# thepochynsons/MCRay-Tracing

Hardware: AMD Instinct MI355X
Metric: rays/sec (Monte-Carlo sample paths traced + accumulated into whole B-mode frames: PSF, envelope, scan conversion) (higher is better)
Workload: dtype f32; 1 GPU; 1M random triangles (8 meshes, PCG64 12345): 128x1024 rays/GPU, depth 10, 465 rows; scan_lines_total=128, triangles=1000000, parallelism=scanline-shard x1, frames_in_flight=128, last_pass_gather_and_post_exposed=False, gather=none (one GPU), slowest_repeat=0, overlap_gather_psf_with_next_trace=True, bvh_builder=sah, warmup_steps_run=5304

## Files before the change

### include/mcrt.h

```cpp
#ifndef MCRT_H
#define MCRT_H
#include <stdint.h>
#include <stddef.h>

#ifdef __cplusplus
extern "C" {
#endif

#define MCRT_VERSION 109

typedef enum {
    MCRT_OK = 0,
    MCRT_ERR_INVALID = -1,
    MCRT_ERR_HIP = -2,
    MCRT_ERR_NOMEM = -3,
    MCRT_ERR_NO_DEVICE = -4,
    MCRT_ERR_LIMIT = -5
} mcrt_status;

typedef struct mcrt_ctx mcrt_ctx;

typedef struct {
    uint32_t n_elements;
    uint32_t n_samples;
// ... 158 lines not shown
                                    uint8_t *out_dev , const mcrt_compound_opts *o );
int mcrt_compound_weights(uint32_t n_elements, uint32_t n_rows, double radius_mm, double total_angle_rad, uint32_t max_travel_us,
                          uint32_t speed_of_sound, uint32_t out_rows, uint32_t out_cols, float steer_rad, float view_weight, float feather_lines,
                          float *w );

typedef struct { uint32_t n_planes;
                 float    step_rad;
                 float    pivot_mm;
} mcrt_sweep;
typedef struct { double origin_mm[3], du_mm[3], dv_mm[3], dw_mm[3];
                 uint32_t nu, nv, nw, _pad;
} mcrt_volume_grid;
int mcrt_transducer_swept(uint32_t n_elements, double radius_cm, double separation_mm, const float position[3], const float angles_deg[3],
                          float tilt_rad, float pivot_mm, float *pos, float *dir);
int mcrt_volume_maps(uint32_t n_elements, uint32_t n_rows, double radius_mm, double total_angle_rad, uint32_t max_travel_us, uint32_t speed_of_sound,
                     const mcrt_sweep *sweep, const mcrt_volume_grid *grid, float *map_plane, float *map_row, float *map_col);
int mcrt_volume_frames(mcrt_ctx *ctx, const float *rf_dev , uint32_t n_frames, uint32_t n_elements, uint32_t n_rows,
                       double radius_mm, double total_angle_rad, const mcrt_sweep *sweep, const mcrt_volume_grid *grid,
                       float *out_dev );
int mcrt_bmode_volume_frames(mcrt_ctx *ctx, const float *rf_dev , uint32_t n_frames, uint32_t n_elements, uint32_t n_rows,
                             const mcrt_bmode_params *p, const mcrt_sweep *sweep, const mcrt_volume_grid *grid,
                             const float *tgc_db , float *peak_dev ,
                             uint8_t *out_dev );

enum { MCRT_RENDER_MIP = 0, MCRT_RENDER_MEAN = 1, MCRT_RENDER_SURFACE = 2 };
typedef struct { float origin[3], di[3], dj[3], ds[3];
                 uint32_t nx, ny, n_steps, _pad;
} mcrt_render_view;
typedef struct { uint32_t mode;
                 float lo, hi;
                 float threshold;
                 float ramp;
                 float opacity;
                 float depth_cue;
                 float t_cut;
} mcrt_render_opts;
int mcrt_default_render_opts(mcrt_render_opts *o, int in_u8);
int mcrt_render_view_for_grid(const mcrt_volume_grid *g, const double dir_mm[3], const double up_mm[3], double pixel_mm, double step_mm,
                              uint32_t nx, uint32_t ny, mcrt_render_view *out);
int mcrt_render_frames(mcrt_ctx *ctx, const void *vol_dev, int in_u8, uint32_t n_frames, uint32_t nu, uint32_t nv, uint32_t nw,
                       const mcrt_render_view *view, const mcrt_render_opts *o ,
                       float *out_dev , uint8_t *out8_dev , float *depth_dev );

typedef struct { uint32_t n_iter;
                 float q0;
                 float rho;
                 float lambda;
} mcrt_speckle_opts;
int mcrt_default_speckle_opts(mcrt_speckle_opts *o);
int mcrt_speckle_tables(const mcrt_speckle_opts *o, float *q0sq , float *kq , float *lam4 );
int mcrt_speckle_frames(mcrt_ctx *ctx, const float *in_dev, uint32_t n_frames, uint32_t height, uint32_t width,
                        const mcrt_speckle_opts *o , float *out_dev);

enum { MCRT_RECON_MEAN = 0, MCRT_RECON_MAX = 1 };
typedef struct { uint32_t mode;
                 float    value_max;
                 uint32_t fill_radius;
                 uint32_t fill_min;
                 float    empty;
} mcrt_recon_opts;
int mcrt_default_recon_opts(mcrt_recon_opts *o);
int mcrt_recon_transform(const mcrt_volume_grid *grid_world_mm, double unit_mm, float A[9], float b[3]);
int mcrt_recon_frames(mcrt_ctx *ctx, const float *stack_dev , uint32_t n_frames, uint32_t n_elements, uint32_t n_rows,
                      const float *pos , const float *dir , double row_mm, double unit_mm,
                      const mcrt_volume_grid *grid , const mcrt_recon_opts *o ,
                      float *out_dev , uint32_t *count_dev , uint32_t *stats_dev );

enum { MCRT_LABEL_TRACED = 0, MCRT_LABEL_GEOMETRIC = 1 };
#define MCRT_LABEL_NONE 255u
#define MCRT_LABEL_MAX_CROSSINGS 64u
typedef struct { uint32_t rule;
                 float    start_offset;
} mcrt_label_opts;
int mcrt_default_label_opts(mcrt_label_opts *o);
int mcrt_label_frames(mcrt_ctx *ctx, uint32_t n_frames, uint32_t e_begin, uint32_t e_end,
                      const float *pos , const float *dir ,
                      const mcrt_label_opts *o ,
                      uint8_t *tissue_dev , int32_t *interface_dev ,
                      uint32_t *crossings_dev );
int mcrt_label_scan_convert_frames(mcrt_ctx *ctx, const uint8_t *tissue_dev , uint32_t n_frames, uint32_t n_elements, uint32_t n_rows,
                                   double radius_mm, double total_angle_rad, uint8_t *out_dev , uint32_t out_rows, uint32_t out_cols);
int mcrt_label_volume_frames(mcrt_ctx *ctx, const uint8_t *tissue_dev , uint32_t n_frames, uint32_t n_elements, uint32_t n_rows,
                             double radius_mm, double total_angle_rad, const mcrt_sweep *sweep, const mcrt_volume_grid *grid,
                             uint8_t *out_dev );

typedef struct { uint32_t n_labels;
                 uint32_t fill_radius;
                 uint32_t fill_min;
} mcrt_recon_label_opts;
int mcrt_default_recon_label_opts(mcrt_recon_label_opts *o, uint32_t n_labels);
int mcrt_recon_label_frames(mcrt_ctx *ctx, const uint8_t *stack_dev , uint32_t n_frames, uint32_t n_elements, uint32_t n_rows,
                            const float *pos , const float *dir , double row_mm, double unit_mm,
                            const mcrt_volume_grid *grid , const mcrt_recon_label_opts *o,
                            uint8_t *out_dev , uint32_t *count_dev , uint32_t *votes_dev ,
                            uint32_t *stats_dev );
int mcrt_render_label_frames(mcrt_ctx *ctx, const uint8_t *label_dev , uint32_t n_frames, uint32_t nu, uint32_t nv, uint32_t nw,
                             const mcrt_render_view *view, const float *depth_dev , uint8_t *out_dev );

int mcrt_export_rf(mcrt_ctx *ctx, const float *rf_dev, uint32_t n_elements, uint32_t n_rows, float *host_rows_by_cols);

int mcrt_import_rf(mcrt_ctx *ctx, const float *host_rows_by_cols, uint32_t n_elements, uint32_t n_rows, float *rf_dev);

typedef struct mcrt_group mcrt_group;
int mcrt_group_create(const int *devices, uint32_t n_devices, mcrt_group **out);
int mcrt_group_destroy(mcrt_group *grp);
int mcrt_group_size(const mcrt_group *grp);
mcrt_ctx *mcrt_group_root(mcrt_group *grp);
mcrt_ctx *mcrt_group_member(mcrt_group *grp, uint32_t rank);
int mcrt_group_shard(uint32_t rank, uint32_t n_ranks, uint32_t n_elements, uint32_t *e_begin, uint32_t *e_end);
int mcrt_group_set_params(mcrt_group *grp, const mcrt_params *p);
int mcrt_group_set_bvh_builder(mcrt_group *grp, int builder);
int mcrt_group_upload_scene(mcrt_group *grp, const float *tri_xyz_host, const uint32_t *tri_mesh, uint32_t n_tri, const mcrt_mesh *meshes, uint32_t n_mesh,
                            const float *materials, uint32_t n_mat, uint32_t start_mat, const float spacing[3]);
int mcrt_group_update_triangles(mcrt_group *grp, const float *tri_xyz_host, uint32_t n_tri);
int mcrt_group_last_scene_seconds(mcrt_group *grp, double *build_s, double *upload_s);
int mcrt_group_refit_triangles(mcrt_group *grp, const float *tri_xyz_host, uint32_t n_tri);
int mcrt_group_upload_texture(mcrt_group *grp, const float *voxels, uint32_t n);
int mcrt_group_set_transducer(mcrt_group *grp, const float *pos, const float *dir, uint32_t n_elements);
int mcrt_group_trace_frames(mcrt_group *grp, uint32_t frame_id, uint32_t n_frames, float *rf_dev);
int mcrt_group_trace_frames_poses(mcrt_group *grp, uint32_t frame_id, uint32_t n_frames, const float *pos, const float *dir, float *rf_dev);
int mcrt_group_synchronize(mcrt_group *grp);
int mcrt_group_last_pass_ms(mcrt_group *grp, float *trace_ms, float *copy_ms);

int mcrt_alloc(mcrt_ctx *ctx, size_t bytes, void **dev);
int mcrt_free(mcrt_ctx *ctx, void *dev);
int mcrt_memcpy_d2h(mcrt_ctx *ctx, void *host, const void *dev, size_t bytes);
int mcrt_memcpy_h2d(mcrt_ctx *ctx, void *dev, const void *host, size_t bytes);

int mcrt_enable_stats(mcrt_ctx *ctx, int enable);
int mcrt_get_stats(mcrt_ctx *ctx, mcrt_stats *out, int reset);
int mcrt_enable_timing(mcrt_ctx *ctx, int enable);
int mcrt_get_kernel_time(mcrt_ctx *ctx, double *avg_ms, uint32_t *n, int reset);
int mcrt_get_kernel_times(mcrt_ctx *ctx, double avg_ms[3], uint32_t n[3], int reset);

int mcrt_build_bvh(const float *tri_xyz, const uint32_t *tri_mesh, uint32_t n_tri, mcrt_bvh *out);
void mcrt_free_bvh(mcrt_bvh *bvh);
int mcrt_get_bvh(mcrt_ctx *ctx, mcrt_bvh *out );
int mcrt_build_bvh4(const mcrt_bvh *bvh2, mcrt_bvh4 *out);
void mcrt_free_bvh4(mcrt_bvh4 *bvh4);
int mcrt_get_bvh4(mcrt_ctx *ctx, mcrt_bvh4 *out );
int mcrt_row_thresholds(double row_dt_us, uint32_t n_rows, double *thr);
int mcrt_generate_texture(float *voxels, uint32_t n);
int mcrt_psf_kernels(float freq, float var_x, float var_y, uint32_t res_um, float *axial, uint32_t n_ax, float *lateral, uint32_t n_lat);
int mcrt_transducer_elements(uint32_t n_elements, double radius_cm, double separation_mm,
                             const float position[3], const float angles_deg[3], float *pos, float *dir);

int mcrt_debug_math(mcrt_ctx *ctx, int op, const double *x, const double *y, double *out, uint32_t n);
int mcrt_debug_philox(mcrt_ctx *ctx, const uint32_t ctr[4], const uint32_t key[2], uint32_t out[4]);
int mcrt_debug_stamps(mcrt_ctx *ctx, uint64_t out[200], int reset);
int mcrt_debug_tail_histograms(mcrt_ctx *ctx, uint64_t out[2560], int reset);
int mcrt_debug_fast_paths(mcrt_ctx *ctx, uint32_t out[4]);
int mcrt_debug_beam(mcrt_ctx *ctx, uint32_t out[6]);
int mcrt_debug_beam_bounce(mcrt_ctx *ctx, uint32_t b, uint32_t out[8]);
int mcrt_debug_set_error(mcrt_ctx *ctx, uint32_t bits);

#ifdef __cplusplus
}
#endif
#endif
```

### mcray-tracing_amd/__init__.py

```python
from ._lib import load_library, build_library, McrtError, Params, MeshRec, BvhNode, Stats, BmodeParams, Focus, Compound, Sweep, VolumeGrid, CompoundOpts, LabelOpts, RenderView, RenderOpts, SpeckleOpts, ReconOpts, ReconLabelOpts, SEGMENT_DTYPE
from .api import Context, Group, shard_range, Simulator, bmode_params, Transducer, Psf, host_build_bvh, host_build_bvh4, host_row_thresholds, host_texture, host_psf, host_psf_focus, focus_struct, row_pitch_mm, host_transducer, host_scan_maps, host_elevation_axis, host_elevation_planes, host_psf_elevation, host_transducer_steered, host_compound_maps, host_transducer_swept, host_volume_maps, sweep_struct, sweep_tilts, volume_grid, cplane_grid, sagittal_grid, compound_struct, compound_opts_struct, host_compound_weights, label_opts_struct, render_view, render_opts_struct, RENDER_MODES, speckle_opts_struct, host_speckle_tables, recon_opts_struct, recon_label_opts_struct, host_recon_transform, RECON_MODES, LABEL_RULES, LABEL_NONE, LABEL_MAX_CROSSINGS, LABEL_CAPPED
from . import synth, scene_io


def __getattr__(name):
    if name == "dist":
        import importlib
        return importlib.import_module("mcray_tracing_amd.dist")
    raise AttributeError(name)

__all__ = ["load_library", "build_library", "McrtError", "Params", "BmodeParams", "bmode_params", "Context", "Group", "shard_range", "Simulator", "Transducer", "Psf",
           "synth", "scene_io", "host_build_bvh", "host_texture", "host_psf", "host_psf_focus", "host_transducer"]
```

### mcray-tracing_amd/_lib.py

```python
import ctypes as C
import os
import subprocess
import numpy as np

_HERE = os.path.dirname(os.path.abspath(__file__))
_SO = os.environ.get("MCRT_LIB") or os.path.join(_HERE, "libmcrt_hip.so")
_LIB = None


class McrtError(RuntimeError):
    def __init__(self, code, msg):
        super().__init__(f"mcrt error {code}: {msg}")
        self.code = code


class Params(C.Structure):
    _fields_ = [("n_elements", C.c_uint32), ("n_samples", C.c_uint32), ("max_depth", C.c_uint32), ("n_rows", C.c_uint32),
                ("frequency", C.c_float), ("intensity_epsilon", C.c_float), ("initial_intensity", C.c_float),
                ("ray_start_offset", C.c_float), ("speed_of_sound", C.c_uint32), ("depth_cm", C.c_double),
                ("seed", C.c_uint32), ("sanitize_tir", C.c_uint32), ("tex_n", C.c_uint32), ("tex_res", C.c_float)]


class MeshRec(C.Structure):
    _fields_ = [("mat_inside", C.c_uint32), ("mat_outside", C.c_uint32), ("vascular", C.c_uint32), ("_pad", C.c_uint32)]


class BvhNode(C.Structure):
    _fields_ = [("lo0", C.c_float * 3), ("c0", C.c_int32), ("hi0", C.c_float * 3), ("c1", C.c_int32),
                ("lo1", C.c_float * 3), ("pad0", C.c_uint32), ("hi1", C.c_float * 3), ("pad1", C.c_uint32)]


class Bvh(C.Structure):
    _fields_ = [("n_nodes", C.c_uint32), ("n_tri", C.c_uint32), ("max_depth", C.c_uint32), ("pad_abs", C.c_float),
                ("nodes", C.c_void_p), ("tri", C.c_void_p)]


class Bvh4(C.Structure):
    _fields_ = [("n_nodes", C.c_uint32), ("max_stack", C.c_uint32), ("nodes", C.c_void_p)]


class Stats(C.Structure):
    _fields_ = [(n, C.c_uint64) for n in ("queries", "nodes_visited", "tris_tested", "segments", "rf_steps", "hits")]

    def as_dict(self):
        return {n: int(getattr(self, n)) for n, _ in self._fields_}


class BmodeParams(C.Structure):
    _fields_ = [("mode", C.c_uint32), ("dynamic_range_db", C.c_float), ("gain_db", C.c_float), ("ref", C.c_float), ("persistence", C.c_float),
                ("reset_state", C.c_uint32), ("out_rows", C.c_uint32), ("out_cols", C.c_uint32), ("radius_mm", C.c_double), ("total_angle_rad", C.c_double)]


class Focus(C.Structure):
    _fields_ = [("n_focus", C.c_uint32), ("focus_mm", C.c_float * 8), ("focal_range_mm", C.c_float)]


class Compound(C.Structure):
    _fields_ = [("n_views", C.c_uint32), ("steer_rad", C.c_float * 16)]


class CompoundOpts(C.Structure):
    _fields_ = [("mode", C.c_uint32), ("feather_lines", C.c_float), ("view_weight", C.c_float * 16)]


class Sweep(C.Structure):
    _fields_ = [("n_planes", C.c_uint32), ("step_rad", C.c_float), ("pivot_mm", C.c_float)]


class VolumeGrid(C.Structure):
    _fields_ = [("origin_mm", C.c_double * 3), ("du_mm", C.c_double * 3), ("dv_mm", C.c_double * 3), ("dw_mm", C.c_double * 3),
                ("nu", C.c_uint32), ("nv", C.c_uint32), ("nw", C.c_uint32), ("_pad", C.c_uint32)]


class LabelOpts(C.Structure):
    _fields_ = [("rule", C.c_uint32), ("start_offset", C.c_float)]


class RenderView(C.Structure):
    _fields_ = [("origin", C.c_float * 3), ("di", C.c_float * 3), ("dj", C.c_float * 3), ("ds", C.c_float * 3),
                ("nx", C.c_uint32), ("ny", C.c_uint32), ("n_steps", C.c_uint32), ("_pad", C.c_uint32)]


class RenderOpts(C.Structure):
    _fields_ = [("mode", C.c_uint32), ("lo", C.c_float), ("hi", C.c_float), ("threshold", C.c_float), ("ramp", C.c_float), ("opacity", C.c_float),
                ("depth_cue", C.c_float), ("t_cut", C.c_float)]


class SpeckleOpts(C.Structure):
    _fields_ = [("n_iter", C.c_uint32), ("q0", C.c_float), ("rho", C.c_float), ("lambda_", C.c_float)]


class ReconOpts(C.Structure):
    _fields_ = [("mode", C.c_uint32), ("value_max", C.c_float), ("fill_radius", C.c_uint32), ("fill_min", C.c_uint32), ("empty", C.c_float)]


class ReconLabelOpts(C.Structure):
    _fields_ = [("n_labels", C.c_uint32), ("fill_radius", C.c_uint32), ("fill_min", C.c_uint32)]


NODE_DTYPE = np.dtype([("lo0", "<f4", 3), ("c0", "<i4"), ("hi0", "<f4", 3), ("c1", "<i4"),
                       ("lo1", "<f4", 3), ("pad0", "<u4"), ("hi1", "<f4", 3), ("pad1", "<u4")])
SEGMENT_DTYPE = np.dtype([("from", "<f4", 3), ("to", "<f4", 3), ("dir", "<f4", 3),
                          ("reflected_intensity", "<f4"), ("initial_intensity", "<f4"), ("attenuation", "<f4"),
                          ("distance_traveled", "<f8"), ("media", "<i4"), ("tri", "<i4")])
assert NODE_DTYPE.itemsize == 64 and SEGMENT_DTYPE.itemsize == 64 and C.sizeof(BvhNode) == 64 and C.sizeof(BmodeParams) == 48 and C.sizeof(Focus) == 40 and C.sizeof(Compound) == 68 and C.sizeof(CompoundOpts) == 72
assert C.sizeof(Sweep) == 12 and C.sizeof(VolumeGrid) == 112 and C.sizeof(LabelOpts) == 8 and C.sizeof(RenderView) == 64 and C.sizeof(RenderOpts) == 32 and C.sizeof(SpeckleOpts) == 16 and C.sizeof(ReconOpts) == 20
assert C.sizeof(ReconLabelOpts) == 12

SYMBOLS = ["mcrt_last_error", "mcrt_version", "mcrt_device_count", "mcrt_create", "mcrt_destroy", "mcrt_set_stream",
           "mcrt_synchronize", "mcrt_default_params", "mcrt_set_params", "mcrt_get_params", "mcrt_import_rf", "mcrt_set_bvh_builder", "mcrt_upload_scene", "mcrt_update_triangles", "mcrt_refit_triangles", "mcrt_upload_texture",
           "mcrt_set_transducer", "mcrt_trace_frame", "mcrt_trace_frames", "mcrt_trace_frames_poses", "mcrt_envelope_frames", "mcrt_scan_convert_frames", "mcrt_trace_frame_debug", "mcrt_cast_rays", "mcrt_convolve", "mcrt_convolve_frames", "mcrt_convolve_frames_depth",
           "mcrt_envelope", "mcrt_scan_convert", "mcrt_default_bmode", "mcrt_bmode_frames", "mcrt_export_rf", "mcrt_alloc", "mcrt_free", "mcrt_memcpy_d2h",
           "mcrt_memcpy_h2d", "mcrt_enable_stats", "mcrt_get_stats", "mcrt_enable_timing", "mcrt_get_kernel_time", "mcrt_get_kernel_times",
           "mcrt_build_bvh", "mcrt_free_bvh", "mcrt_get_bvh", "mcrt_build_bvh4", "mcrt_free_bvh4", "mcrt_get_bvh4", "mcrt_row_thresholds", "mcrt_generate_texture", "mcrt_psf_kernels", "mcrt_psf_focus_kernels",
           "mcrt_transducer_elements", "mcrt_transducer_elevation_axis", "mcrt_elevation_planes", "mcrt_psf_elevation_kernels", "mcrt_elevation_frames", "mcrt_debug_math", "mcrt_debug_philox", "mcrt_debug_stamps", "mcrt_debug_tail_histograms", "mcrt_debug_set_error", "mcrt_debug_fast_paths", "mcrt_debug_beam", "mcrt_debug_beam_bounce", "mcrt_scan_maps",
           "mcrt_group_create", "mcrt_group_destroy", "mcrt_group_size", "mcrt_group_root", "mcrt_group_member", "mcrt_group_shard", "mcrt_group_set_params",
           "mcrt_group_set_bvh_builder", "mcrt_group_upload_scene", "mcrt_group_update_triangles", "mcrt_group_refit_triangles", "mcrt_group_upload_texture",
           "mcrt_group_set_transducer", "mcrt_group_trace_frames", "mcrt_group_trace_frames_poses", "mcrt_group_synchronize", "mcrt_group_last_pass_ms", "mcrt_group_last_scene_seconds",
           "mcrt_transducer_steered", "mcrt_compound_maps", "mcrt_compound_frames", "mcrt_bmode_compound_frames",
           "mcrt_default_compound_opts", "mcrt_compound_weights", "mcrt_compound_frames_opts", "mcrt_bmode_compound_frames_opts",
           "mcrt_transducer_swept", "mcrt_volume_maps", "mcrt_volume_frames", "mcrt_bmode_volume_frames",
           "mcrt_default_label_opts", "mcrt_label_frames", "mcrt_label_scan_convert_frames", "mcrt_label_volume_frames",
           "mcrt_default_render_opts", "mcrt_render_view_for_grid", "mcrt_render_frames",
           "mcrt_default_speckle_opts", "mcrt_speckle_tables", "mcrt_speckle_frames",
           "mcrt_default_recon_opts", "mcrt_recon_transform", "mcrt_recon_frames",
           "mcrt_default_recon_label_opts", "mcrt_recon_label_frames", "mcrt_render_label_frames"]


def build_library(force=False):
    srcs = [os.path.join(_HERE, "csrc", f) for f in os.listdir(os.path.join(_HERE, "csrc"))]
    srcs.append(os.path.join(_HERE, "..", "include", "mcrt.h"))
    stale = (not os.path.exists(_SO)) or any(os.path.getmtime(s) > os.path.getmtime(_SO) for s in srcs)
    if force or stale:
        subprocess.check_call(["make", "-C", _HERE, "libmcrt_hip.so"] + (["-B"] if force else []))
    return _SO


def load_library():
    global _LIB
    if _LIB is not None:
        return _LIB
    if not os.path.exists(_SO):
        raise McrtError(-4, f"{_SO} is missing: run __graft_entry__.build() (make -C mcray-tracing_amd); there is no CPU fallback")
    L = C.CDLL(_SO)
    L.mcrt_last_error.restype = C.c_char_p
    vp, u32, i32 = C.c_void_p, C.c_uint32, C.c_int
    sig = {
        "mcrt_create": [i32, C.POINTER(vp)], "mcrt_destroy": [vp], "mcrt_set_stream": [vp, vp], "mcrt_synchronize": [vp],
        "mcrt_default_params": [C.POINTER(Params)], "mcrt_set_params": [vp, C.POINTER(Params)], "mcrt_get_params": [vp, C.POINTER(Params)], "mcrt_import_rf": [vp, vp, u32, u32, vp],
        "mcrt_upload_scene": [vp, vp, vp, u32, vp, u32, vp, u32, u32, vp],
        "mcrt_upload_texture": [vp, vp, u32], "mcrt_set_transducer": [vp, vp, vp, u32],
        "mcrt_trace_frame": [vp, u32, u32, u32, vp], "mcrt_trace_frames": [vp, u32, u32, u32, u32, vp], "mcrt_trace_frame_debug": [vp, u32, u32, u32, vp, vp, vp, vp],
        "mcrt_cast_rays": [vp, u32, u32, u32, vp, vp, vp],
        "mcrt_convolve": [vp, vp, u32, u32, vp, u32, vp, u32], "mcrt_envelope": [vp, vp, u32, u32],
        "mcrt_scan_convert": [vp, vp, u32, u32, C.c_double, C.c_double, vp, u32, u32],
        "mcrt_convolve_frames": [vp, vp, u32, u32, u32, vp, u32, vp, u32], "mcrt_convolve_frames_depth": [vp, vp, u32, u32, u32, vp, u32, vp, u32],
        "mcrt_trace_frames_poses": [vp, u32, u32, u32, u32, vp, vp, vp], "mcrt_envelope_frames": [vp, vp, u32, u32, u32],
        "mcrt_scan_convert_frames": [vp, vp, u32, u32, u32, C.c_double, C.c_double, vp, u32, u32],
        "mcrt_default_bmode": [C.POINTER(BmodeParams)], "mcrt_bmode_frames": [vp, vp, u32, u32, u32, C.POINTER(BmodeParams), vp, vp, vp, vp],
        "mcrt_set_bvh_builder": [vp, i32], "mcrt_update_triangles": [vp, vp, u32], "mcrt_refit_triangles": [vp, vp, u32],
        "mcrt_export_rf": [vp, vp, u32, u32, vp], "mcrt_alloc": [vp, C.c_size_t, C.POINTER(vp)], "mcrt_free": [vp, vp],
        "mcrt_memcpy_d2h": [vp, vp, vp, C.c_size_t], "mcrt_memcpy_h2d": [vp, vp, vp, C.c_size_t],
        "mcrt_enable_stats": [vp, i32], "mcrt_get_stats": [vp, C.POINTER(Stats), i32],
        "mcrt_enable_timing": [vp, i32], "mcrt_get_kernel_time": [vp, C.POINTER(C.c_double), C.POINTER(u32), i32], "mcrt_get_kernel_times": [vp, vp, vp, i32],
        "mcrt_build_bvh": [vp, vp, u32, C.POINTER(Bvh)], "mcrt_free_bvh": [C.POINTER(Bvh)], "mcrt_get_bvh": [vp, C.POINTER(Bvh)],
        "mcrt_build_bvh4": [C.POINTER(Bvh), C.POINTER(Bvh4)], "mcrt_free_bvh4": [C.POINTER(Bvh4)], "mcrt_get_bvh4": [vp, C.POINTER(Bvh4)],
        "mcrt_row_thresholds": [C.c_double, u32, vp],
        "mcrt_generate_texture": [vp, u32], "mcrt_psf_kernels": [C.c_float, C.c_float, C.c_float, u32, vp, u32, vp, u32],
        "mcrt_psf_focus_kernels": [C.c_float, u32, C.POINTER(Focus), u32, C.c_double, vp, u32],
        "mcrt_transducer_elements": [u32, C.c_double, C.c_double, vp, vp, vp, vp],
        "mcrt_transducer_elevation_axis": [vp, vp], "mcrt_elevation_planes": [vp, vp, u32, vp, u32, u32, vp, vp, vp],
        "mcrt_psf_elevation_kernels": [C.c_float, u32, C.POINTER(Focus), u32, C.c_double, i32, vp, u32],
        "mcrt_elevation_frames": [vp, vp, u32, u32, u32, u32, vp, vp],
        "mcrt_transducer_steered": [u32, C.c_double, C.c_double, vp, vp, C.c_float, vp, vp],
        "mcrt_compound_maps": [u32, u32, C.c_double, C.c_double, u32, u32, u32, u32, C.c_float, vp, vp],
        "mcrt_compound_frames": [vp, vp, u32, u32, u32, C.c_double, C.c_double, C.POINTER(Compound), vp, u32, u32],
        "mcrt_bmode_compound_frames": [vp, vp, u32, u32, u32, C.POINTER(BmodeParams), C.POINTER(Compound), vp, vp, vp, vp],
        "mcrt_default_compound_opts": [C.POINTER(CompoundOpts)],
        "mcrt_compound_weights": [u32, u32, C.c_double, C.c_double, u32, u32, u32, u32, C.c_float, C.c_float, C.c_float, vp],
        "mcrt_compound_frames_opts": [vp, vp, u32, u32, u32, C.c_double, C.c_double, C.POINTER(Compound), vp, u32, u32, C.POINTER(CompoundOpts)],
        "mcrt_bmode_compound_frames_opts": [vp, vp, u32, u32, u32, C.POINTER(BmodeParams), C.POINTER(Compound), vp, vp, vp, vp, C.POINTER(CompoundOpts)],
        "mcrt_transducer_swept": [u32, C.c_double, C.c_double, vp, vp, C.c_float, C.c_float, vp, vp],
        "mcrt_volume_maps": [u32, u32, C.c_double, C.c_double, u32, u32, C.POINTER(Sweep), C.POINTER(VolumeGrid), vp, vp, vp],
        "mcrt_volume_frames": [vp, vp, u32, u32, u32, C.c_double, C.c_double, C.POINTER(Sweep), C.POINTER(VolumeGrid), vp],
        "mcrt_bmode_volume_frames": [vp, vp, u32, u32, u32, C.POINTER(BmodeParams), C.POINTER(Sweep), C.POINTER(VolumeGrid), vp, vp, vp],
        "mcrt_default_label_opts": [C.POINTER(LabelOpts)],
        "mcrt_label_frames": [vp, u32, u32, u32, vp, vp, C.POINTER(LabelOpts), vp, vp, vp],
        "mcrt_label_scan_convert_frames": [vp, vp, u32, u32, u32, C.c_double, C.c_double, vp, u32, u32],
        "mcrt_label_volume_frames": [vp, vp, u32, u32, u32, C.c_double, C.c_double, C.POINTER(Sweep), C.POINTER(VolumeGrid), vp],
        "mcrt_default_render_opts": [C.POINTER(RenderOpts), i32],
        "mcrt_render_view_for_grid": [C.POINTER(VolumeGrid), vp, vp, C.c_double, C.c_double, u32, u32, C.POINTER(RenderView)],
        "mcrt_render_frames": [vp, vp, i32, u32, u32, u32, u32, C.POINTER(RenderView), C.POINTER(RenderOpts), vp, vp, vp],
        "mcrt_default_speckle_opts": [C.POINTER(SpeckleOpts)],
        "mcrt_speckle_tables": [C.POINTER(SpeckleOpts), vp, vp, vp],
        "mcrt_speckle_frames": [vp, vp, u32, u32, u32, C.POINTER(SpeckleOpts), vp],
        "mcrt_default_recon_opts": [C.POINTER(ReconOpts)],
        "mcrt_recon_transform": [C.POINTER(VolumeGrid), C.c_double, vp, vp],
        "mcrt_recon_frames": [vp, vp, u32, u32, u32, vp, vp, C.c_double, C.c_double, C.POINTER(VolumeGrid), C.POINTER(ReconOpts), vp, vp, vp],
        "mcrt_default_recon_label_opts": [C.POINTER(ReconLabelOpts), u32],
        "mcrt_recon_label_frames": [vp, vp, u32, u32, u32, vp, vp, C.c_double, C.c_double, C.POINTER(VolumeGrid), C.POINTER(ReconLabelOpts), vp, vp, vp, vp],
        "mcrt_render_label_frames": [vp, vp, u32, u32, u32, u32, C.POINTER(RenderView), vp, vp],
        "mcrt_debug_math": [vp, i32, vp, vp, vp, u32], "mcrt_debug_philox": [vp, vp, vp, vp], "mcrt_debug_stamps": [vp, vp, i32], "mcrt_debug_tail_histograms": [vp, vp, i32], "mcrt_debug_set_error": [vp, u32], "mcrt_debug_fast_paths": [vp, vp], "mcrt_debug_beam": [vp, vp], "mcrt_debug_beam_bounce": [vp, u32, vp],
        "mcrt_scan_maps": [u32, u32, C.c_double, C.c_double, u32, u32, u32, u32, vp, vp],
        "mcrt_group_create": [vp, u32, C.POINTER(vp)], "mcrt_group_destroy": [vp], "mcrt_group_size": [vp], "mcrt_group_root": [vp], "mcrt_group_member": [vp, u32],
        "mcrt_group_shard": [u32, u32, u32, C.POINTER(u32), C.POINTER(u32)], "mcrt_group_set_params": [vp, C.POINTER(Params)], "mcrt_group_set_bvh_builder": [vp, i32],
        "mcrt_group_upload_scene": [vp, vp, vp, u32, vp, u32, vp, u32, u32, vp], "mcrt_group_update_triangles": [vp, vp, u32], "mcrt_group_refit_triangles": [vp, vp, u32],
        "mcrt_group_upload_texture": [vp, vp, u32], "mcrt_group_set_transducer": [vp, vp, vp, u32], "mcrt_group_trace_frames": [vp, u32, u32, vp],
        "mcrt_group_trace_frames_poses": [vp, u32, u32, vp, vp, vp], "mcrt_group_synchronize": [vp], "mcrt_group_last_pass_ms": [vp, vp, vp],
        "mcrt_group_last_scene_seconds": [vp, C.POINTER(C.c_double), C.POINTER(C.c_double)],
    }
    for name, args in sig.items():
        if name in ("mcrt_debug_beam", "mcrt_debug_beam_bounce") and not hasattr(L, name):
            continue
        f = getattr(L, name)
        f.argtypes = args
        f.restype = None if name in ("mcrt_free_bvh", "mcrt_free_bvh4") else vp if name in ("mcrt_group_root", "mcrt_group_member") else C.c_int
    _LIB = L
    return L


def check(rc):
    if rc != 0:
        raise McrtError(rc, load_library().mcrt_last_error().decode())


def ptr(a):
    if a is None:
        return None
    if isinstance(a, int):
        return C.c_void_p(a)
    if isinstance(a, np.ndarray):
        return a.ctypes.data_as(C.c_void_p)
    if hasattr(a, "data_ptr"):
        return C.c_void_p(a.data_ptr())
    raise TypeError(type(a))
```

### mcray-tracing_amd/api.py

```python
import contextlib
import ctypes as C
import math
import numpy as np

from . import _lib
from ._lib import Params, MeshRec, Stats, Bvh, Bvh4, BmodeParams, Focus, Compound, Sweep, VolumeGrid, CompoundOpts, LabelOpts, RenderView, RenderOpts, SpeckleOpts, ReconOpts, ReconLabelOpts, NODE_DTYPE, SEGMENT_DTYPE, check, ptr, load_library

DEFAULT_ANGLE = 1.0471975511965976


def host_build_bvh(tri, tri_mesh):
    L = load_library()
    tri = np.ascontiguousarray(tri, np.float32).reshape(-1, 9)
    tm = np.ascontiguousarray(tri_mesh, np.uint32)
    b = Bvh()
    check(L.mcrt_build_bvh(ptr(tri), ptr(tm), tri.shape[0], C.byref(b)))
    try:
        nodes = np.frombuffer(C.string_at(b.nodes, 64 * b.n_nodes), dtype=NODE_DTYPE).copy()
        btri = np.frombuffer(C.string_at(b.tri, 48 * b.n_tri), dtype=np.float32).reshape(-1, 12).copy()
        depth = int(b.max_depth)
    finally:
        L.mcrt_free_bvh(C.byref(b))
    return nodes, btri, depth


def host_build_bvh4(tri, tri_mesh):
    L = load_library()
    tri = np.ascontiguousarray(tri, np.float32).reshape(-1, 9)
    tm = np.ascontiguousarray(tri_mesh, np.uint32)
    b = Bvh(); b4 = Bvh4()
    check(L.mcrt_build_bvh(ptr(tri), ptr(tm), tri.shape[0], C.byref(b)))
    try:
        check(L.mcrt_build_bvh4(C.byref(b), C.byref(b4)))
        nodes = np.frombuffer(C.string_at(b.nodes, 64 * b.n_nodes), dtype=NODE_DTYPE).copy()
        btri = np.frombuffer(C.string_at(b.tri, 48 * b.n_tri), dtype=np.float32).reshape(-1, 12).copy()
        n4 = np.frombuffer(C.string_at(b4.nodes, 128 * b4.n_nodes), dtype=np.uint8).reshape(-1, 128).copy()
        ms = int(b4.max_stack)
    finally:
        L.mcrt_free_bvh(C.byref(b)); L.mcrt_free_bvh4(C.byref(b4))
    return nodes, btri, n4, ms


def host_row_thresholds(row_dt_us, n_rows):
    thr = np.zeros(n_rows + 1, np.float64)
    check(load_library().mcrt_row_thresholds(row_dt_us, n_rows, ptr(thr)))
    return thr


def host_texture(n=256):
    out = np.empty((n, n, n, 2), np.float32)
    check(load_library().mcrt_generate_texture(ptr(out), n))
    return out


def host_psf(freq=4.5, var_x=0.05, var_y=0.2, res_um=145, n_ax=7, n_lat=13):
    ax = np.zeros(n_ax, np.float32); lat = np.zeros(n_lat, np.float32)
    check(load_library().mcrt_psf_kernels(freq, var_x, var_y, res_um, ptr(ax), n_ax, ptr(lat), n_lat))
    return ax, lat


def focus_struct(focus_mm=(), focal_range_mm=20.0):
    f = Focus()
    fm = [float(x) for x in (focus_mm or ())]
    f.n_focus = len(fm)
    for i, x in enumerate(fm[:8]):
        f.focus_mm[i] = x
    f.focal_range_mm = focal_range_mm
    return f


def host_psf_focus(var_y, res_um, n_rows, row_mm, focus_mm, focal_range_mm=20.0, n_lat=13):
    out = np.zeros((n_rows, n_lat), np.float32)
    f = focus_struct(focus_mm, focal_range_mm)
    check(load_library().mcrt_psf_focus_kernels(var_y, res_um, C.byref(f), n_rows, row_mm, ptr(out), n_lat))
    return out


def row_pitch_mm(frequency):
    res_f = np.float32(np.float32(1.45) / np.float32(frequency))
    return int(np.float32(res_f * np.float32(1000.0))) / 1000.0


def _element_tables(fn, n_elements, radius_cm, sep_mm, position, angles_deg, *how):
    pos = np.zeros((n_elements, 3), np.float32); d = np.zeros((n_elements, 3), np.float32)
    p = np.asarray(position, np.float32); a = np.asarray(angles_deg, np.float32)
    check(getattr(load_library(), fn)(n_elements, radius_cm, sep_mm, ptr(p), ptr(a), *how, ptr(pos), ptr(d)))
    return pos, d


def host_transducer(n_elements, radius_cm, sep_mm, position, angles_deg):
    return _element_tables("mcrt_transducer_elements", n_elements, radius_cm, sep_mm, position, angles_deg)


def host_elevation_axis(angles_deg):
    a = np.asarray(angles_deg, np.float32); out = np.zeros(3, np.float32)
    check(load_library().mcrt_transducer_elevation_axis(ptr(a), ptr(out)))
    return out


def host_elevation_planes(pos, dirs, axis, n_planes, pitch_um):
    pos = np.ascontiguousarray(pos, np.float32).reshape(-1, 3); dirs = np.ascontiguousarray(dirs, np.float32).reshape(-1, 3)
    axis = np.ascontiguousarray(axis, np.float32)
    E, K = pos.shape[0], max(int(n_planes), 0)
    po = np.zeros((K, E, 3), np.float32); do = np.zeros((K, E, 3), np.float32); z = np.zeros(K, np.float32)
    check(load_library().mcrt_elevation_planes(ptr(pos), ptr(dirs), E, ptr(axis), n_planes, pitch_um, ptr(po), ptr(do), ptr(z)))
    return po, do, z


def host_psf_elevation(var_z, pitch_um, n_rows, row_mm, focus_mm=(), focal_range_mm=20.0, n_planes=7, normalize=True):
    out = np.zeros((n_rows, max(int(n_planes), 0)), np.float32)
    f = focus_struct(focus_mm, focal_range_mm)
    check(load_library().mcrt_psf_elevation_kernels(var_z, pitch_um, C.byref(f), n_rows, row_mm, 1 if normalize else 0, ptr(out), n_planes))
    return out


def host_scan_maps(n_elements, n_rows, radius_mm=30.0, total_angle=DEFAULT_ANGLE, max_travel_us=100, speed_of_sound=1500, out_rows=400, out_cols=500):
    return _sector_maps("mcrt_scan_maps", n_elements, n_rows, radius_mm, total_angle, max_travel_us, speed_of_sound, out_rows, out_cols)


def _sector_maps(fn, n_elements, n_rows, radius_mm, total_angle, max_travel_us, speed_of_sound, out_rows, out_cols, *steer):
    mr = np.zeros((out_rows, out_cols), np.float32); mc = np.zeros((out_rows, out_cols), np.float32)
    check(getattr(load_library(), fn)(n_elements, n_rows, radius_mm, total_angle, max_travel_us, speed_of_sound, out_rows, out_cols, *steer, ptr(mr), ptr(mc)))
    return mr, mc


def host_transducer_steered(n_elements, radius_cm, sep_mm, position, angles_deg, steer_rad):
    return _element_tables("mcrt_transducer_steered", n_elements, radius_cm, sep_mm, position, angles_deg, steer_rad)


def host_compound_maps(n_elements, n_rows, steer_rad, radius_mm=30.0, total_angle=DEFAULT_ANGLE, max_travel_us=100, speed_of_sound=1500, out_rows=400,
                       out_cols=500):
    return _sector_maps("mcrt_compound_maps", n_elements, n_rows, radius_mm, total_angle, max_travel_us, speed_of_sound, out_rows, out_cols, steer_rad)


def compound_struct(steer_rad):
    st = [float(x) for x in steer_rad]
    cp = Compound()
    cp.n_views = len(st)
    for i, x in enumerate(st[:16]):
        cp.steer_rad[i] = x
    return cp


COMPOUND_MODES = {"mean": 0, "max": 1, "median": 2}


def compound_opts_struct(mode="mean", view_weights=None, feather_lines=0.0):
    o = CompoundOpts()
    check(load_library().mcrt_default_compound_opts(C.byref(o)))
    o.mode = COMPOUND_MODES[mode] if isinstance(mode, str) else int(mode)
    o.feather_lines = float(feather_lines)
    if view_weights is not None:
        w = [float(x) for x in view_weights]
        if len(w) > 16:
            raise ValueError("at most 16 view weights, got %d" % len(w))
        for i, x in enumerate(w):
            o.view_weight[i] = x
    return o


def _compound_defaults(mode, view_weights, feather_lines):
    return mode in ("mean", 0) and view_weights is None and feather_lines == 0.0


def host_compound_weights(n_elements, n_rows, steer_rad, view_weight=1.0, feather_lines=0.0, radius_mm=30.0, total_angle=DEFAULT_ANGLE,
                          max_travel_us=100, speed_of_sound=1500, out_rows=400, out_cols=500):
    w = np.zeros((out_rows, out_cols), np.float32)
    check(load_library().mcrt_compound_weights(n_elements, n_rows, radius_mm, total_angle, max_travel_us, speed_of_sound, out_rows, out_cols, steer_rad,
                                               view_weight, feather_lines, ptr(w)))
    return w


def host_transducer_swept(n_elements, radius_cm, sep_mm, position, angles_deg, tilt_rad, pivot_mm=0.0):
    return _element_tables("mcrt_transducer_swept", n_elements, radius_cm, sep_mm, position, angles_deg, tilt_rad, pivot_mm)


def sweep_struct(n_planes, step_rad, pivot_mm=0.0):
    sw = Sweep()
    sw.n_planes, sw.step_rad, sw.pivot_mm = int(n_planes), float(step_rad), float(pivot_mm)
    return sw


def _as_sweep(sweep):
    return sweep if isinstance(sweep, Sweep) else sweep_struct(*sweep)


def sweep_tilts(n_planes, step_rad):
    step = float(np.float32(step_rad))
    return np.array([(k - (n_planes - 1) / 2.0) * step for k in range(n_planes)], np.float32)


def volume_grid(origin_mm, du, dv, dw, nu, nv, nw=1):
    g = VolumeGrid()
    for dst, src in ((g.origin_mm, origin_mm), (g.du_mm, du), (g.dv_mm, dv), (g.dw_mm, dw)):
        for i in range(3):
            dst[i] = float(src[i])
    g.nu, g.nv, g.nw, g._pad = int(nu), int(nv), int(nw), 0
    return g


def cplane_grid(depth_mm, nu, nv, pitch_mm, x0_mm=None, z0_mm=None):
    x0 = -(nu - 1) * pitch_mm / 2.0 if x0_mm is None else x0_mm
    z0 = -(nv - 1) * pitch_mm / 2.0 if z0_mm is None else z0_mm
    return volume_grid((x0, depth_mm, z0), (pitch_mm, 0, 0), (0, 0, pitch_mm), (0, 0, 0), nu, nv, 1)


def sagittal_grid(x_mm, nu, nv, pitch_mm, y0_mm, z0_mm=None):
    z0 = -(nu - 1) * pitch_mm / 2.0 if z0_mm is None else z0_mm
    return volume_grid((x_mm, y0_mm, z0), (0, 0, pitch_mm), (0, pitch_mm, 0), (0, 0, 0), nu, nv, 1)


def host_volume_maps(n_elements, n_rows, sweep, grid, radius_mm=30.0, total_angle=DEFAULT_ANGLE, max_travel_us=100, speed_of_sound=1500):
    sw = _as_sweep(sweep)
    shape = (grid.nw, grid.nv, grid.nu)
    mz = np.zeros(shape, np.float32); mr = np.zeros(shape, np.float32); mc = np.zeros(shape, np.float32)
    check(load_library().mcrt_volume_maps(n_elements, n_rows, radius_mm, total_angle, max_travel_us, speed_of_sound, C.byref(sw), C.byref(grid), ptr(mz), ptr(mr), ptr(mc)))
    return mz, mr, mc


BMODE_MODES = {"db": 0, "ref_log": 1}


RENDER_MODES = {"mip": 0, "mean": 1, "surface": 2}


def render_view(grid, direction, up=(0, 0, 1), pixel_mm=0.25, step_mm=0.25, nx=500, ny=400):
    v = RenderView()
    d = (C.c_double * 3)(*[float(x) for x in direction]); u = (C.c_double * 3)(*[float(x) for x in up])
    check(load_library().mcrt_render_view_for_grid(C.byref(grid), d, u, float(pixel_mm), float(step_mm), int(nx), int(ny), C.byref(v)))
    return v


def render_opts_struct(in_u8=False, mode=None, lo=None, hi=None, threshold=None, ramp=None, opacity=None, depth_cue=None, t_cut=None):
    o = RenderOpts()
    check(load_library().mcrt_default_render_opts(C.byref(o), 1 if in_u8 else 0))
    if mode is not None:
        o.mode = RENDER_MODES[mode] if isinstance(mode, str) else int(mode)
    for name, val in (("lo", lo), ("hi", hi), ("threshold", threshold), ("ramp", ramp), ("opacity", opacity), ("depth_cue", depth_cue), ("t_cut", t_cut)):
        if val is not None:
            setattr(o, name, float(val))
    return o


def speckle_opts_struct(n_iter=None, q0=None, rho=None, lambda_=None, **kw):
    o = SpeckleOpts()
    check(load_library().mcrt_default_speckle_opts(C.byref(o)))
    for k in ("lambda", "lam"):
        if k in kw:
            lambda_ = kw.pop(k)
    if kw:
        raise TypeError("unknown speckle options: %s" % ", ".join(sorted(kw)))
    if n_iter is not None:
        o.n_iter = int(n_iter)
    for name, val in (("q0", q0), ("rho", rho), ("lambda_", lambda_)):
        if val is not None:
            setattr(o, name, float(val))
    return o


def host_speckle_tables(opts=None, **kw):
    o = opts if opts is not None else speckle_opts_struct(**kw)
    n = min(int(o.n_iter), 256)
    q0sq = np.zeros(n, np.float32); kq = np.zeros(n, np.float32); lam4 = np.zeros(1, np.float32)
    check(load_library().mcrt_speckle_tables(C.byref(o), ptr(q0sq), ptr(kq), ptr(lam4)))
    return q0sq, kq, np.float32(lam4[0])


RECON_MODES = {"mean": 0, "max": 1}
# ... 93 lines not shown
        if positions.shape != angles_deg.shape:
            raise ValueError("poses takes one position and one set of angles per frame")
        tabs = [host_transducer(self.n_elements, self.radius_cm, self.separation_mm, p, a) for p, a in zip(positions, angles_deg)]
        return np.stack([t[0] for t in tabs]), np.stack([t[1] for t in tabs])


class Psf:

    def __init__(self, freq=4.5, var_x=0.05, var_y=0.2, var_z=0.1, axial_size=7, lateral_size=13, resolution_um=145, focus_mm=None, focal_range_mm=20.0,
                 elevation_size=7, elevation_pitch_um=None, elevation_focus_mm=None, elevation_normalize=True):
        self.axial_kernel, self.lateral_kernel = host_psf(freq, var_x, var_y, resolution_um, axial_size, lateral_size)
        self.var_y, self.resolution_um = var_y, resolution_um
        self.focus_mm = tuple(float(x) for x in focus_mm) if focus_mm is not None else ()
        self.focal_range_mm = focal_range_mm
        self._rows = {}
        self.var_z, self.elevation_size = var_z, elevation_size
        self.elevation_pitch_um = resolution_um if elevation_pitch_um is None else elevation_pitch_um
        self.elevation_focus_mm = tuple(float(x) for x in elevation_focus_mm) if elevation_focus_mm is not None else ()
        self.elevation_normalize = bool(elevation_normalize)
        self.elevation_kernel = (host_psf_elevation(var_z, self.elevation_pitch_um, 1, 1.0, (), focal_range_mm, elevation_size, False)[0]
                                 if var_z > 0 and math.isfinite(var_z) else np.zeros(elevation_size, np.float32))
        self._elev_rows = {}

    def elevation_rows(self, n_rows, row_mm):
        key = (n_rows, row_mm)
        if key not in self._elev_rows:
            self._elev_rows[key] = host_psf_elevation(self.var_z, self.elevation_pitch_um, n_rows, row_mm, self.elevation_focus_mm, self.focal_range_mm,
                                                      self.elevation_size, self.elevation_normalize)
        return self._elev_rows[key]

    @property
    def has_focus(self):
        return len(self.focus_mm) > 0

    def lateral_rows(self, n_rows, row_mm):
        key = (n_rows, row_mm)
        if key not in self._rows:
            self._rows[key] = host_psf_focus(self.var_y, self.resolution_um, n_rows, row_mm, self.focus_mm, self.focal_range_mm, self.lateral_kernel.size)
        return self._rows[key]


def _scene_tables(sd):
    meshes = (MeshRec * len(sd.meshes))(*[MeshRec(a, b, c, 0) for a, b, c in sd.meshes])
    return meshes, len(sd.meshes), np.asarray(sd.spacing, np.float32)


def _tri9(tri):
    if isinstance(tri, np.ndarray):
        tri = np.ascontiguousarray(tri, np.float32).reshape(-1, 9)
        return tri, tri.shape[0]
    return tri, tri.numel() // 9


def _tgc_rows(tgc_db, n_rows):
    if tgc_db is None:
        return None
    tgc = np.ascontiguousarray(tgc_db, np.float32)
    if tgc.shape != (n_rows,):
        raise ValueError("tgc_db needs one value per RF row: %d, got shape %s" % (n_rows, tgc.shape))
    return tgc


def _pose_tables(what, pos, dirs, n_frames, n_elements):
    if isinstance(pos, np.ndarray):
        pos = np.ascontiguousarray(pos, np.float32); dirs = np.ascontiguousarray(dirs, np.float32)
    if n_frames is None:
        if not hasattr(pos, "shape"):
            raise ValueError("%s: n_frames is required with raw device pointers for pos / dirs" % what)
        n_frames = pos.shape[0]
        assert tuple(pos.shape) == (n_frames, n_elements, 3) and tuple(dirs.shape) == tuple(pos.shape)
    return pos, dirs, n_frames


class _SceneCalls:

    def _call(self, name, *args):
        check(getattr(self.L, self.PREFIX + name)(self.h, *args))

    def _assign_params(self, kw):
        for k, v in kw.items():
            if not hasattr(self.params, k):
                raise AttributeError(k)
            setattr(self.params, k, v)

    def set_bvh_builder(self, builder):
        self._call("set_bvh_builder", {"sah": 0, "lbvh": 1}[builder] if isinstance(builder, str) else int(builder))

    def upload_scene(self, sd):
        meshes, n_mesh, sp = _scene_tables(sd)
        self._call("upload_scene", ptr(sd.tri), ptr(sd.tri_mesh), sd.n_tri, C.cast(meshes, C.c_void_p), n_mesh, ptr(sd.materials), sd.materials.shape[0], sd.start_mat, ptr(sp))

    def upload_texture(self, vox=None, n=256):
        if vox is not None:
            vox = np.ascontiguousarray(vox, np.float32)
        self._call("upload_texture", ptr(vox), n)

    def set_transducer(self, pos, d):
        pos = np.ascontiguousarray(pos, np.float32); d = np.ascontiguousarray(d, np.float32)
        self._call("set_transducer", ptr(pos), ptr(d), pos.shape[0])


class Context(_SceneCalls):
    PREFIX = "mcrt_"

    def __init__(self, device=0, _borrowed=None):
        self.L = load_library()
        self.owned = _borrowed is None
        if self.owned:
            h = C.c_void_p()
            check(self.L.mcrt_create(device, C.byref(h)))
        else:
            h = C.c_void_p(_borrowed)
        self.h = h
        self.params = Params()
        check(self.L.mcrt_default_params(C.byref(self.params)))

    def close(self):
        if getattr(self, "h", None):
            if self.owned:
                self.L.mcrt_destroy(self.h)
            self.h = None

    def __del__(self):
        try:
            self.close()
        except Exception:
            pass

    def set_params(self, **kw):
        self._assign_params(kw)
        check(self.L.mcrt_set_params(self.h, C.byref(self.params)))

    def set_stream(self, stream_ptr):
        check(self.L.mcrt_set_stream(self.h, C.c_void_p(stream_ptr) if stream_ptr else None))

    def synchronize(self):
        check(self.L.mcrt_synchronize(self.h))

    def debug_fast_paths(self):
        out = (C.c_uint32 * 4)()
        check(self.L.mcrt_debug_fast_paths(self.h, out))
        return bool(out[0]), bool(out[1]), int(out[2])

    def debug_beam(self):
        out = (C.c_uint32 * 6)()
        if hasattr(self.L, "mcrt_debug_beam"):
            check(self.L.mcrt_debug_beam(self.h, out))
        return bool(out[0]), int(out[1]), int(out[2]), int(out[3]), int(out[4]), int(out[5])

    def debug_beam_bounce(self, b):
        out = (C.c_uint32 * 8)()
        if hasattr(self.L, "mcrt_debug_beam_bounce"):
            check(self.L.mcrt_debug_beam_bounce(self.h, int(b), out))
        return (bool(out[0]),) + tuple(int(v) for v in out[1:])

    def debug_set_error(self, bits):
        check(self.L.mcrt_debug_set_error(self.h, int(bits)))

    def update_triangles(self, tri):
        tri, n = _tri9(tri)
        check(self.L.mcrt_update_triangles(self.h, ptr(tri), n))

    def refit_triangles(self, tri):
        tri, n = _tri9(tri)
        check(self.L.mcrt_refit_triangles(self.h, ptr(tri), n))

    def get_bvh(self):
        b = Bvh()
        check(self.L.mcrt_get_bvh(self.h, C.byref(b)))
        nodes = np.frombuffer(C.string_at(b.nodes, 64 * b.n_nodes), dtype=NODE_DTYPE).copy() if b.n_nodes else np.zeros(0, NODE_DTYPE)
        btri = np.frombuffer(C.string_at(b.tri, 48 * b.n_tri), dtype=np.float32).reshape(-1, 12).copy()
        return nodes, btri, int(b.max_depth)

    def get_bvh4(self):
        b = Bvh4()
        check(self.L.mcrt_get_bvh4(self.h, C.byref(b)))
        return np.frombuffer(C.string_at(b.nodes, 128 * b.n_nodes), dtype=np.uint8).reshape(-1, 128).copy(), int(b.max_stack)

    def alloc(self, nbytes):
        p = C.c_void_p()
        check(self.L.mcrt_alloc(self.h, nbytes, C.byref(p)))
        return p.value

    def free(self, dev):
        check(self.L.mcrt_free(self.h, C.c_void_p(dev)))

    @contextlib.contextmanager
    def temp(self, nbytes):
        p = self.alloc(nbytes)
        try:
            yield p
        finally:
            self.free(p)

    def d2h(self, dev, shape, dtype=np.float32):
        out = np.empty(shape, dtype)
        check(self.L.mcrt_memcpy_d2h(self.h, ptr(out), ptr(dev), out.nbytes))
        return out

    def h2d(self, dev, arr):
        arr = np.ascontiguousarray(arr)
        check(self.L.mcrt_memcpy_h2d(self.h, ptr(dev), ptr(arr), arr.nbytes))

    def trace_frame(self, frame_id, rf_dev, e_begin=0, e_end=None):
        e_end = self.params.n_elements if e_end is None else e_end
        check(self.L.mcrt_trace_frame(self.h, frame_id, e_begin, e_end, ptr(rf_dev)))

    def trace_frames(self, frame_id, n_frames, rf_dev, e_begin=0, e_end=None):
        e_end = self.params.n_elements if e_end is None else e_end
        check(self.L.mcrt_trace_frames(self.h, frame_id, n_frames, e_begin, e_end, ptr(rf_dev)))

    def trace_frames_poses(self, frame_id, pos, dirs, rf_dev, e_begin=0, e_end=None, n_frames=None):
        e_end = self.params.n_elements if e_end is None else e_end
        pos, dirs, n_frames = _pose_tables("trace_frames_poses", pos, dirs, n_frames, self.params.n_elements)
        check(self.L.mcrt_trace_frames_poses(self.h, frame_id, n_frames, e_begin, e_end, ptr(pos), ptr(dirs), ptr(rf_dev)))

    def trace_frame_debug(self, frame_id, rf_dev, e_begin=0, e_end=None, want_hits=True, want_segs=False):
        e_end = self.params.n_elements if e_end is None else e_end
        ne, S, B = e_end - e_begin, self.params.n_samples, self.params.max_depth
        hits = np.full((ne, S, B), -3, np.int32) if want_hits else None
        segs = np.zeros((ne, S, B), SEGMENT_DTYPE) if want_segs else None
        cnt = np.zeros((ne, S), np.uint32) if want_segs else None
        check(self.L.mcrt_trace_frame_debug(self.h, frame_id, e_begin, e_end, ptr(rf_dev), ptr(hits), ptr(segs), ptr(cnt)))
        return hits, segs, cnt

    def cast_rays(self, frame_id, e_begin=0, e_end=None, want_hits=True):
        e_end = self.params.n_elements if e_end is None else e_end
        ne, S, B = e_end - e_begin, self.params.n_samples, self.params.max_depth
        segs = np.zeros((ne, S, B), SEGMENT_DTYPE); cnt = np.zeros((ne, S), np.uint32)
        hits = np.full((ne, S, B), -3, np.int32) if want_hits else None
        check(self.L.mcrt_cast_rays(self.h, frame_id, e_begin, e_end, ptr(segs), ptr(cnt), ptr(hits)))
        return segs, cnt, hits

    def convolve_frames(self, rf_dev, n_frames, n_elements, n_rows, axial, lateral):
        ax = np.ascontiguousarray(axial, np.float32); lat = np.ascontiguousarray(lateral, np.float32)
        check(self.L.mcrt_convolve_frames(self.h, ptr(rf_dev), n_frames, n_elements, n_rows, ptr(ax), ax.size, ptr(lat), lat.size))

    def convolve_frames_depth(self, rf_dev, n_frames, n_elements, n_rows, axial, lat_rows):
        ax = np.ascontiguousarray(axial, np.float32); lat = np.ascontiguousarray(lat_rows, np.float32)
        if lat.ndim != 2 or lat.shape[0] != n_rows:
            raise ValueError("lat_rows needs one row of taps per RF row: (%d, n_lat), got shape %s" % (n_rows, lat.shape))
        check(self.L.mcrt_convolve_frames_depth(self.h, ptr(rf_dev), n_frames, n_elements, n_rows, ptr(ax), ax.size, ptr(lat), lat.shape[1]))

    def elevation_frames(self, planes_dev, n_frames, n_planes, n_elements, n_rows, w_rows, rf_dev):
        w = np.ascontiguousarray(w_rows, np.float32)
        if w.shape != (n_rows, n_planes):
            raise ValueError("w_rows needs one row of weights per RF row: (%d, %d), got shape %s" % (n_rows, n_planes, w.shape))
        check(self.L.mcrt_elevation_frames(self.h, ptr(planes_dev), n_frames, n_planes, n_elements, n_rows, ptr(w), ptr(rf_dev)))

    def convolve(self, rf_dev, n_elements, n_rows, axial, lateral):
        ax =np.ascontiguousarray(axial, np.float32); lat = np.ascontiguousarray(lateral, np.float32)
        check(self.L.mcrt_convolve(self.h, ptr(rf_dev), n_elements, n_rows, ptr(ax), ax.size, ptr(lat), lat.size))

    def envelope(self, rf_dev, n_elements, n_rows):
        check(self.L.mcrt_envelope(self.h, ptr(rf_dev), n_elements, n_rows))

    def envelope_frames(self, rf_dev, n_frames, n_elements, n_rows):
        check(self.L.mcrt_envelope_frames(self.h, ptr(rf_dev), n_frames, n_elements, n_rows))

    def scan_convert_frames(self, rf_dev, n_frames, n_elements, n_rows, out_dev, radius_mm=30.0, total_angle=DEFAULT_ANGLE, out_rows=400, out_cols=500):
        check(self.L.mcrt_scan_convert_frames(self.h, ptr(rf_dev), n_frames, n_elements, n_rows, radius_mm, total_angle, ptr(out_dev), out_rows, out_cols))

    def scan_convert(self, rf_dev, n_elements, n_rows, out_dev, radius_mm=30.0, total_angle=DEFAULT_ANGLE, out_rows=400, out_cols=500):
        check(self.L.mcrt_scan_convert(self.h, ptr(rf_dev), n_elements, n_rows, radius_mm, total_angle, ptr(out_dev), out_rows, out_cols))

    def bmode_frames(self, rf_dev, n_frames, n_elements, n_rows, out_dev, *, mode="db", dynamic_range_db=60.0, gain_db=0.0, ref=None, tgc_db=None,
                     persistence=0.0, state_dev=None, reset_state=True, peak_dev=None, radius_mm=30.0, total_angle=DEFAULT_ANGLE,
                     out_rows=400, out_cols=500):
        p = bmode_params(mode=mode, dynamic_range_db=dynamic_range_db, gain_db=gain_db, ref=ref, persistence=persistence, reset_state=reset_state,
                         radius_mm=radius_mm, total_angle=total_angle, out_rows=out_rows, out_cols=out_cols)
        tgc = _tgc_rows(tgc_db, n_rows)
        check(self.L.mcrt_bmode_frames(self.h, ptr(rf_dev), n_frames, n_elements, n_rows, C.byref(p), ptr(tgc), ptr(state_dev), ptr(peak_dev), ptr(out_dev)))

    def compound_frames(self, rf_dev, n_frames, n_elements, n_rows, steer_rad, out_dev, radius_mm=30.0, total_angle=DEFAULT_ANGLE, out_rows=400, out_cols=500,
                        mode="mean", view_weights=None, feather_lines=0.0):
        cp = compound_struct(steer_rad)
        if _compound_defaults(mode, view_weights, feather_lines):
            check(self.L.mcrt_compound_frames(self.h, ptr(rf_dev), n_frames, n_elements, n_rows, radius_mm, total_angle, C.byref(cp), ptr(out_dev), out_rows, out_cols))
            return
        o = compound_opts_struct(mode, view_weights, feather_lines)
        check(self.L.mcrt_compound_frames_opts(self.h, ptr(rf_dev), n_frames, n_elements, n_rows, radius_mm, total_angle, C.byref(cp), ptr(out_dev), out_rows, out_cols,
                                               C.byref(o)))

    def bmode_compound_frames(self, rf_dev, n_frames, n_elements, n_rows, steer_rad, out_dev, *, mode="db", dynamic_range_db=60.0, gain_db=0.0, ref=None,
                              tgc_db=None, persistence=0.0, state_dev=None, reset_state=True, peak_dev=None, radius_mm=30.0,
                              total_angle=DEFAULT_ANGLE, out_rows=400, out_cols=500, compound_mode="mean", view_weights=None, feather_lines=0.0):
        p = bmode_params(mode=mode, dynamic_range_db=dynamic_range_db, gain_db=gain_db, ref=ref, persistence=persistence, reset_state=reset_state,
                         radius_mm=radius_mm, total_angle=total_angle, out_rows=out_rows, out_cols=out_cols)
        cp = compound_struct(steer_rad)
        tgc = _tgc_rows(tgc_db, n_rows)
        if _compound_defaults(compound_mode, view_weights, feather_lines):
            check(self.L.mcrt_bmode_compound_frames(self.h, ptr(rf_dev), n_frames, n_elements, n_rows, C.byref(p), C.byref(cp), ptr(tgc), ptr(state_dev),
                                                    ptr(peak_dev), ptr(out_dev)))
            return
        o = compound_opts_struct(compound_mode, view_weights, feather_lines)
        check(self.L.mcrt_bmode_compound_frames_opts(self.h, ptr(rf_dev), n_frames, n_elements, n_rows, C.byref(p), C.byref(cp), ptr(tgc), ptr(state_dev),
                                                     ptr(peak_dev), ptr(out_dev), C.byref(o)))

    def volume_frames(self, rf_dev, n_frames, n_elements, n_rows, sweep, grid, out_dev, radius_mm=30.0, total_angle=DEFAULT_ANGLE):
        sw = _as_sweep(sweep)
        check(self.L.mcrt_volume_frames(self.h, ptr(rf_dev), n_frames, n_elements, n_rows, radius_mm, total_angle, C.byref(sw), C.byref(grid), ptr(out_dev)))

    def bmode_volume_frames(self, rf_dev, n_frames, n_elements, n_rows, sweep, grid, out_dev, *, mode="db", dynamic_range_db=60.0, gain_db=0.0, ref=None,
                            tgc_db=None, persistence=0.0, peak_dev=None, radius_mm=30.0, total_angle=DEFAULT_ANGLE):
        p = bmode_params(mode=mode, dynamic_range_db=dynamic_range_db, gain_db=gain_db, ref=ref, persistence=persistence, radius_mm=radius_mm,
                         total_angle=total_angle, out_rows=0, out_cols=0)
# ... 398 lines not shown
```

### mcray-tracing_amd/csrc/mcrt_api.cpp

```cpp
#include "mcrt_ctx.h"
#include "mcrt_kernels.h"
#include "mcrt_lbvh.h"

#include <hip/hip_runtime.h>
#include <cmath>
#include <cstdlib>
#include <cstring>
#include <vector>
#include <algorithm>
#include <memory>
#include <utility>

using mcrt::set_error;

static Consts derive_consts(const mcrt_params &p)
{
    Consts c;
    c.axial_res_f = 1.45f / p.frequency;
    c.axial_res_mm = (double)c.axial_res_f;
    c.axial_res_um = (uint32_t)(c.axial_res_f * 1000.0f);
    c.time_step_us = (c.axial_res_mm * 1000.0) / (double)p.speed_of_sound;
    c.row_dt_us = (double)c.axial_res_um / (double)p.speed_of_sound;
    c.max_travel_us = (p.depth_cm / (double)p.speed_of_sound) * 10000.0;
    c.max_rows = (uint32_t)((p.speed_of_sound * (uint32_t)c.max_travel_us) / c.axial_res_um);
    return c;
}

static Knobs read_knobs()
{
    using mcrt::tuning_env;
    Knobs k;
    if (const char *e = tuning_env("MCRT_KSPLIT_LIMIT")) { long v = atol(e); if (v >= 0 && v <= MCRT_KSPLIT_MAX) k.ksplit_limit = (uint32_t)v; }
    if (const char *e = tuning_env("MCRT_TRACE_BLOCKS")) { int v = atoi(e); if (v >= 1) k.trace_blocks = (uint32_t)v; }
    if (const char *e = tuning_env("MCRT_TRACE_BLOCKS_WIDE")) { int v = atoi(e); if (v >= 1) k.trace_blocks_wide = (uint32_t)v; }
    if (const char *e = tuning_env("MCRT_WIDE_MAX_TREE_MB")) { long long v = atoll(e); if (v >= 0 && v <= 0xffffffffll) k.wide_max_tree_mb = (uint32_t)v; }
    if (const char *e = tuning_env("MCRT_WIDE_FROM")) { long long v = atoll(e); if (v >= 1 && v <= 0xffffffffll) k.wide_from = (uint32_t)v; }
    if (const char *e = tuning_env("MCRT_GROUPS")) { int v = atoi(e); if (v >= 1 && v <= 16) k.groups = (uint32_t)v; }
    if (const char *e = tuning_env("MCRT_PACKET_BOUNCES")) { long v = strtol(e, nullptr, 0); if (v >= 0) k.packet_mask = (uint32_t)v; }
    if (const char *e = tuning_env("MCRT_PATH_GROUPS")) { int v = atoi(e); if (v >= 1 && v <= 16) k.path_groups = (uint32_t)v; }
    if (const char *e = tuning_env("MCRT_PATH_MAX")) { long long v = atoll(e); if (v >= 0 && v <= 0xffffffffll) k.path_max = (uint32_t)v; }
    if (const char *e = tuning_env("MCRT_PACKET_FROM")) { long long v = atoll(e); if (v >= 0 && v <= 0xffffffffll) k.packet_from = (uint32_t)v; }
    if (const char *e = tuning_env("MCRT_MARCH_STREAMS")) { int v = atoi(e); if (v >= 1 && v <= MCRT_SIDE_STREAMS) k.march_streams = (uint32_t)v; }
    if (const char *e = tuning_env("MCRT_MARCH_BLOCKS")) { int v = atoi(e); if (v >= 1) k.march_blocks = (uint32_t)v; }
    k.no_overlap = tuning_env("MCRT_NO_OVERLAP") != nullptr; k.no_priority = tuning_env("MCRT_NO_PRIORITY") != nullptr;
    k.no_fast_div = tuning_env("MCRT_NO_FAST_DIV") != nullptr; k.no_lean = tuning_env("MCRT_NO_LEAN") != nullptr;
    k.test_hooks = tuning_env("MCRT_TEST_HOOKS") != nullptr;
    if (const char *e = tuning_env("MCRT_RETIRE_LATE")) k.retire_late = atoi(e) != 0;
    if (const char *e = tuning_env("MCRT_FOLD_B0")) k.fold_b0 = atoi(e) != 0;
    if (const char *e = tuning_env("MCRT_BEAM_B1")) { int v = atoi(e); if (v >= 0 && v <= 2) k.beam_b1 = (uint32_t)v; }
    if (const char *e = tuning_env("MCRT_BEAM_FROM")) { long long v = atoll(e); if (v >= 0 && v <= 0xffffffffll) k.beam_from = (uint32_t)v; }
    if (const char *e = tuning_env("MCRT_BEAM_LAST")) { int v = atoi(e); if (v >= 1 && v < MCRT_MAX_BOUNCES) k.beam_last = (uint32_t)v; }
    if (const char *e = tuning_env("MCRT_BEAM_DEEP_FROM")) { long long v = atoll(e); if (v >= 0 && v <= 0xffffffffll) k.beam_deep_from = (uint32_t)v; }
    if (const char *e = tuning_env("MCRT_BEAM_GROUPS")) { long long v = atoll(e); if (v >= 1 && v <= (1 << 20)) k.beam_groups = (uint32_t)v; }
    if (const char *e = tuning_env("MCRT_BEAM_CAP")) { int v = atoi(e); if (v >= 1 && v <= (int)MCRT_BEAM_CAP_MAX) k.beam_cap = (uint32_t)v; }
    if (const char *e = tuning_env("MCRT_BEAM_NEAR")) { int v = atoi(e); if (v >= 1) k.beam_near = (uint32_t)v; }
    if (const char *e = tuning_env("MCRT_RENDER_ROW_TILE")) k.render_row_tile = atoi(e) != 0;
    if (const char *e = tuning_env("MCRT_SPECKLE_FUSE")) { int v = atoi(e); if (v == 2 || v == 4) k.speckle_fuse = (uint32_t)v; }
    return k;
}

static int prepare_tables(mcrt_ctx *c)
{
    if (c->tab.thr_rows != c->p.n_rows || c->tab.thr_dt != c->c.row_dt_us || !c->tab.d_row_thr) {
        std::vector<double> thr((size_t)c->p.n_rows + 1);
        MCRT_TRY(mcrt_row_thresholds(c->c.row_dt_us, c->p.n_rows, thr.data()));
        HIP_TRY(hipStreamSynchronize(c->stream));
        c->tab.thr_rows = 0;
        HIP_TRY(c->tab.d_row_thr.alloc(thr.size()));
        HIP_TRY(hipMemcpy(c->tab.d_row_thr, thr.data(), thr.size() * 8, hipMemcpyHostToDevice));
        c->tab.thr_rows = c->p.n_rows; c->tab.thr_dt = c->c.row_dt_us; c->tab.thr_end = thr.back();
    }
    if (c->tab.verified_res != c->p.tex_res) {
        Buf<unsigned long long> d_bad; unsigned long long bad = 1;
        HIP_TRY(d_bad.alloc(1));
        HIP_TRY(hipMemsetAsync(d_bad, 0, 8, c->stream));
        HIP_TRY(mcrt::launch_verify_div(c->p.tex_res, 1.0f / c->p.tex_res, d_bad, c->stream));
        HIP_TRY(hipStreamSynchronize(c->stream));
        HIP_TRY(hipMemcpy(&bad, d_bad, 8, hipMemcpyDeviceToHost));
        c->tab.fast_div = (bad == 0) && !c->knobs.no_fast_div;
        c->tab.fast_div_all = c->tab.fast_div && c->p.tex_res > 1e-16f && !c->knobs.no_lean;
        c->tab.verified_res = c->p.tex_res;
    }
    if (c->scene.have && (!c->tab.mtab_valid || c->tab.mtab_key[0] != c->c.axial_res_f || c->tab.mtab_key[1] != c->p.frequency)) {
        c->tab.mtab_valid = false;
        if (c->tab.d_mtab.cap < c->scene.n_mat) {
            HIP_TRY(hipStreamSynchronize(c->stream));
            HIP_TRY(c->tab.d_mtab.alloc(c->scene.n_mat));
        }
        HIP_TRY(mcrt::launch_material_table(c->scene.d_mats, c->scene.n_mat, c->c.axial_res_f, c->p.frequency, c->tab.d_mtab, c->stream));
        c->tab.mtab_key[0] = c->c.axial_res_f; c->tab.mtab_key[1] = c->p.frequency; c->tab.mtab_valid = true;
    }
    return MCRT_OK;
}

extern "C" int mcrt_version(void) { return MCRT_VERSION; }
extern "C" int mcrt_device_count(void)
{
    int n = 0;
    if (hipGetDeviceCount(&n) != hipSuccess) return 0;
    return n;
}

extern "C" int mcrt_default_params(mcrt_params *p)
{
    if (!p) return set_error(MCRT_ERR_INVALID, "null params");
    memset(p, 0, sizeof *p);
    p->n_elements = 512; p->n_samples = 5; p->max_depth = 10; p->n_rows = 465;
    p->frequency = 4.5f; p->intensity_epsilon = 1e-10f; p->initial_intensity = 1.0f; p->ray_start_offset = 0.1f;
    p->speed_of_sound = 1500; p->depth_cm = 15.0; p->seed = 0x5EED; p->sanitize_tir = 0; p->tex_n = 256; p->tex_res = 0.145f;
    return MCRT_OK;
}

extern "C" int mcrt_create(int device, mcrt_ctx **out)
{
    if (!out) return set_error(MCRT_ERR_INVALID, "null out pointer");
    *out = nullptr;
    int n = 0;
    if (hipGetDeviceCount(&n) != hipSuccess || n <= 0)
        return set_error(MCRT_ERR_NO_DEVICE, "no HIP device visible: libmcrt_hip has no CPU fallback");
    if (device < 0 || device >= n) return set_error(MCRT_ERR_INVALID, "device %d out of range (0..%d)", device, n - 1);
    HIP_TRY(hipSetDevice(device));
    hipDeviceProp_t prop;
    HIP_TRY(hipGetDeviceProperties(&prop, device));
    if (!strstr(prop.gcnArchName, "gfx950"))
        return set_error(MCRT_ERR_NO_DEVICE, "device %d is %s; this library carries gfx950 (MI355X) code only", device, prop.gcnArchName);
    std::unique_ptr<mcrt_ctx> c(new (std::nothrow) mcrt_ctx());
    if (!c) return set_error(MCRT_ERR_NOMEM, "out of host memory");
    c->device = device;
    c->knobs = read_knobs();
    if (prop.multiProcessorCount > 0) c->n_cu = (uint32_t)prop.multiProcessorCount;
    HIP_TRY(hipStreamCreateWithFlags(&c->own_stream.h, hipStreamNonBlocking));
    c->stream = c->own_stream;
    HIP_TRY(ensure_event(c->ev_start));
    c->work.reserve(16);
    mcrt_default_params(&c->p);
    c->c = derive_consts(c->p);
    HIP_TRY(c->ins.d_stats.alloc(MCRT_STATS_WORDS));
    HIP_TRY(hipMemsetAsync(c->ins.d_stats, 0, MCRT_STATS_WORDS * sizeof(unsigned long long), c->stream));
    HIP_TRY(c->d_error.alloc(1));
    HIP_TRY(hipMemsetAsync(c->d_error, 0, 4, c->stream));
    HIP_TRY(hipStreamSynchronize(c->stream));
    MCRT_TRY(prepare_tables(c.get()));
    *out = c.release();
    return MCRT_OK;
}

static int refresh_soa(mcrt_ctx *c)
{
    c->scene.walked_stale = true;
    if (c->scene.bvh4.n_nodes == 0) { c->scene.d_nodes_walk.reset(); return MCRT_OK; }
    if (c->scene.d_nodes_walk.cap != 4 * (size_t)c->scene.bvh4.n_nodes) {
        HIP_TRY(hipStreamSynchronize(c->stream));
        HIP_TRY(c->scene.d_nodes_walk.alloc(4 * (size_t)c->scene.bvh4.n_nodes));
    }
    HIP_TRY(mcrt::launch_nodes_walk(c->scene.d_nodes, c->scene.bvh4.n_nodes, c->scene.d_nodes_walk, c->stream));
    if (c->scene.d_tris_id.cap != MCRT_TRI_PIECES * (size_t)c->scene.bvh.n_tri) {
        HIP_TRY(hipStreamSynchronize(c->stream));
        HIP_TRY(c->scene.d_tris_id.alloc(MCRT_TRI_PIECES * (size_t)c->scene.bvh.n_tri));
    }
    HIP_TRY(mcrt::launch_tris_by_id((const float4 *)c->scene.d_tris, c->scene.bvh.n_tri, c->scene.d_tris_id, c->stream));
    HIP_TRY(ensure_event(c->scene.ev_update));
    HIP_TRY(hipEventRecord(c->scene.ev_update, c->stream));
    c->scene.update_stream = c->stream; c->scene.update_pending = true;
    return MCRT_OK;
}

extern "C" int mcrt_destroy(mcrt_ctx *c)
{
    if (!c) return MCRT_OK;
    hipSetDevice(c->device);
    hipDeviceSynchronize();
    delete c;
    return MCRT_OK;
}

namespace mcrt { hipStream_t ctx_stream(mcrt_ctx *c) { return c->stream; } }
extern "C" int mcrt_set_stream(mcrt_ctx *c, void *s) { CTX_TRY(c); c->stream = s ? (hipStream_t)s : c->own_stream; return MCRT_OK; }
int mcrt::check_device_error(mcrt_ctx *c)
{
    uint32_t e = 0;
    HIP_TRY(hipMemcpy(&e, c->d_error, 4, hipMemcpyDeviceToHost));
    if (e) { HIP_TRY(hipMemsetAsync(c->d_error, 0, 4, c->stream)); HIP_TRY(hipStreamSynchronize(c->stream)); return set_error(MCRT_ERR_LIMIT, "device error flag 0x%x:%s%s", e, (e & 1u) ? " BVH traversal stack overflow" : "", (e & 2u) ? " kernel watchdog expired (a persistent kernel ran for more than its time limit and was abandoned)" : ""); }
    return MCRT_OK;
}
extern "C" int mcrt_synchronize(mcrt_ctx *c) { CTX_TRY(c); HIP_TRY(hipStreamSynchronize(c->stream)); return mcrt::check_device_error(c); }

extern "C" int mcrt_set_params(mcrt_ctx *c, const mcrt_params *p)
{
    CTX_TRY(c);
    if (!p) return set_error(MCRT_ERR_INVALID, "null params");
    if (p->n_elements == 0 || p->n_samples == 0) return set_error(MCRT_ERR_INVALID, "n_elements and n_samples must be positive");
    if (p->max_depth == 0 || p->max_depth > MCRT_MAX_BOUNCES) return set_error(MCRT_ERR_LIMIT, "max_depth must be 1..%d", MCRT_MAX_BOUNCES);
    if (p->n_rows == 0 || p->n_rows > MCRT_MAX_ROWS) return set_error(MCRT_ERR_LIMIT, "n_rows must be 1..%d", MCRT_MAX_ROWS);
    if (!(p->frequency > 0.f) || p->speed_of_sound == 0 || !(p->depth_cm > 0.0)) return set_error(MCRT_ERR_INVALID, "frequency, speed_of_sound and depth must be positive");
    if (p->tex_n == 0 || !(p->tex_res > 0.f)) return set_error(MCRT_ERR_INVALID, "texture size/resolution must be positive");
    Consts k = derive_consts(*p);
    if (k.axial_res_um == 0) return set_error(MCRT_ERR_INVALID, "axial resolution rounds to 0 um at %g MHz", (double)p->frequency);
    c->p = *p; c->c = k;
    return prepare_tables(c);
}

extern "C" int mcrt_get_params(mcrt_ctx *c, mcrt_params *out)
{
    if (!c || !out) return set_error(MCRT_ERR_INVALID, "null argument");
    *out = c->p;
    return MCRT_OK;
}

// ... 204 lines not shown
extern "C" int mcrt_get_bvh4(mcrt_ctx *c, mcrt_bvh4 *out)
{
    if (!c || !out) return set_error(MCRT_ERR_INVALID, "null argument");
    if (!c->scene.have) return set_error(MCRT_ERR_INVALID, "no scene uploaded");
    HIP_TRY(hipSetDevice(c->device));
    if (c->scene.d_nodes_walk) {
        if (c->scene.walked_stale || !c->scene.walked_nodes) {
            const size_t bytes = sizeof(mcrt_bvh4_node) * (size_t)c->scene.bvh4.n_nodes;
            Buf<float4> d_tmp;
            HIP_TRY(d_tmp.alloc(bytes / 16));
            hipError_t e = mcrt::launch_nodes_walk_decode(c->scene.d_nodes_walk, c->scene.bvh4.n_nodes, d_tmp, c->stream);
            if (e == hipSuccess) e = hipStreamSynchronize(c->stream);
            free(c->scene.walked_nodes);
            c->scene.walked_nodes = (mcrt_bvh4_node *)malloc(bytes);
            if (e == hipSuccess && c->scene.walked_nodes) e = hipMemcpy(c->scene.walked_nodes, d_tmp, bytes, hipMemcpyDeviceToHost);
            d_tmp.reset();
            if (!c->scene.walked_nodes) return set_error(MCRT_ERR_NOMEM, "out of memory");
            if (e != hipSuccess) return set_error(MCRT_ERR_HIP, "mcrt_get_bvh4: %s", hipGetErrorString(e));
            c->scene.walked_stale = false;
        }
        out->n_nodes = c->scene.bvh4.n_nodes; out->max_stack = c->scene.bvh4.max_stack; out->nodes = c->scene.walked_nodes;
        return MCRT_OK;
    }
    MCRT_TRY(download_bvh(c));
    *out = c->scene.bvh4;
    return MCRT_OK;
}

extern "C" int mcrt_upload_texture(mcrt_ctx *c, const float *vox, uint32_t n)
{
    CTX_TRY(c);
    if (n == 0) return set_error(MCRT_ERR_INVALID, "texture size 0");
    const size_t total = (size_t)n * n * n;
    std::vector<float> gen;
    bool finite = true;
    if (!vox) {
        gen.resize(total * 2);
        MCRT_TRY(mcrt_generate_texture(gen.data(), n));
        vox = gen.data();
    } else {
        for (size_t i = 0; i < total * 2; i++) if (!std::isfinite(vox[i])) { finite = false; break; }
    }
    HIP_TRY(hipStreamSynchronize(c->stream));
    c->tex_n = 0;
    HIP_TRY(c->d_tex.alloc(total));
    HIP_TRY(hipMemcpy(c->d_tex, vox, total * 8, hipMemcpyHostToDevice));
    c->tex_n = n; c->tex_finite = finite;
    return MCRT_OK;
}

extern "C" int mcrt_set_transducer(mcrt_ctx *c, const float *pos, const float *dir, uint32_t n)
{
    CTX_TRY(c);
    if (!pos || !dir || n == 0) return set_error(MCRT_ERR_INVALID, "mcrt_set_transducer: bad arguments");
    if (n != c->n_el) {
        HIP_TRY(hipStreamSynchronize(c->stream));
        c->n_el = 0;
        HIP_TRY(c->d_pos.alloc(3 * (size_t)n));
        HIP_TRY(c->d_dir.alloc(3 * (size_t)n));
        c->n_el = n;
    }
    HIP_TRY(hipMemcpyAsync(c->d_pos, pos, 12 * (size_t)n, hipMemcpyHostToDevice, c->stream));
    HIP_TRY(hipMemcpyAsync(c->d_dir, dir, 12 * (size_t)n, hipMemcpyHostToDevice, c->stream));
    HIP_TRY(hipStreamSynchronize(c->stream));
    return MCRT_OK;
}

extern "C" int mcrt_alloc(mcrt_ctx *c, size_t bytes, void **dev)
{
    CTX_TRY(c);
    if (!dev) return set_error(MCRT_ERR_INVALID, "null out pointer");
    HIP_TRY(hipMalloc(dev, bytes ? bytes : 1));
    return MCRT_OK;
}
extern "C" int mcrt_free(mcrt_ctx *c, void *dev) { CTX_TRY(c); HIP_TRY(hipStreamSynchronize(c->stream)); HIP_TRY(hipFree(dev)); return MCRT_OK; }
extern "C" int mcrt_memcpy_d2h(mcrt_ctx *c, void *host, const void *dev, size_t bytes)
{
    CTX_TRY(c);
    HIP_TRY(hipMemcpyAsync(host, dev, bytes, hipMemcpyDeviceToHost, c->stream));
    HIP_TRY(hipStreamSynchronize(c->stream));
    return MCRT_OK;
}
extern "C" int mcrt_memcpy_h2d(mcrt_ctx *c, void *dev, const void *host, size_t bytes)
{
    CTX_TRY(c);
    HIP_TRY(hipMemcpyAsync(dev, host, bytes, hipMemcpyHostToDevice, c->stream));
    HIP_TRY(hipStreamSynchronize(c->stream));
    return MCRT_OK;
}

extern "C" int mcrt_enable_stats(mcrt_ctx *c, int on) { CTX_TRY(c); c->ins.stats_on = on != 0; return MCRT_OK; }
static int read_stats(mcrt_ctx *c, size_t first, size_t n, void *out, int reset)
{
    CTX_TRY(c);
    HIP_TRY(hipStreamSynchronize(c->stream));
    HIP_TRY(hipMemcpy(out, c->ins.d_stats + first, n * 8, hipMemcpyDeviceToHost));
    if (reset) { HIP_TRY(hipMemsetAsync(c->ins.d_stats + first, 0, n * 8, c->stream)); HIP_TRY(hipStreamSynchronize(c->stream)); }
    return MCRT_OK;
}
extern "C" int mcrt_get_stats(mcrt_ctx *c, mcrt_stats *out, int reset)
{
    unsigned long long v[6];
    MCRT_TRY(read_stats(c, 0, 6, v, reset));
    if (out) { out->queries = v[0]; out->nodes_visited = v[1]; out->tris_tested = v[2]; out->segments = v[3]; out->rf_steps = v[4]; out->hits = v[5]; }
    return MCRT_OK;
}

extern "C" int mcrt_debug_stamps(mcrt_ctx *c, uint64_t out[200], int reset) { return read_stats(c, 8, 200, out, reset); }

extern "C" int mcrt_debug_tail_histograms(mcrt_ctx *c, uint64_t out[2560], int reset)
{
    CTX_TRY(c);
    if (!out) return set_error(MCRT_ERR_INVALID, "null out pointer");
    return read_stats(c, 256, 2560, out, reset);
}

extern "C" int mcrt_debug_fast_paths(mcrt_ctx *c, uint32_t out[4])
{
    CTX_TRY(c);
    if (!out) return set_error(MCRT_ERR_INVALID, "null out pointer");
    out[0] = c->tab.fast_div ? 1u : 0u; out[1] = c->ins.last_lean_bound > 0.0f ? 1u : 0u; out[2] = c->ins.last_march_rows; out[3] = 0u;
    return MCRT_OK;
}

static int debug_beam(mcrt_ctx *c, uint32_t b, uint32_t out[8])
{
    for (int k = 0; k < 8; k++) out[k] = 0u;
    if (b >= MCRT_MAX_BOUNCES || !((c->ins.last_beam_mask >> b) & 1u) || c->work.empty()) return MCRT_OK;
    const Work &w = c->work[0];
    uint32_t lc[MCRT_BEAM_COUNTERS] = {}, n = 0;
    HIP_TRY(hipStreamSynchronize(c->stream));
    HIP_TRY(hipMemcpy(lc, w.beam.lcount.p + (size_t)b * MCRT_BEAM_COUNTERS, sizeof lc, hipMemcpyDeviceToHost));
    HIP_TRY(hipMemcpy(&n, w.b.counts.p + b, 4, hipMemcpyDeviceToHost));
    const uint32_t walked = lc[c->ins.last_beam_far ? 1 : 0];
    out[0] = 1u; out[1] = n - walked; out[2] = walked; out[3] = lc[2]; out[4] = lc[3]; out[5] = lc[4]; out[6] = lc[6]; out[7] = lc[7];
    return MCRT_OK;
}
extern "C" int mcrt_debug_beam(mcrt_ctx *c, uint32_t out[6])
{
    CTX_TRY(c);
    if (!out) return set_error(MCRT_ERR_INVALID, "null out pointer");
    uint32_t o[8];
    MCRT_TRY(debug_beam(c, 1u, o));
    for (int k = 0; k < 6; k++) out[k] = o[k];
    return MCRT_OK;
}
extern "C" int mcrt_debug_beam_bounce(mcrt_ctx *c, uint32_t b, uint32_t out[8])
{
    CTX_TRY(c);
    if (!out) return set_error(MCRT_ERR_INVALID, "null out pointer");
    return debug_beam(c, b, out);
}

extern "C" int mcrt_debug_set_error(mcrt_ctx *c, uint32_t bits)
{
    CTX_TRY(c);
    if (!c->knobs.test_hooks) return set_error(MCRT_ERR_INVALID, "mcrt_debug_set_error is a test hook: create the context with MCRT_TEST_HOOKS set in the environment");
    uint32_t e = 0;
    HIP_TRY(hipStreamSynchronize(c->stream));
    HIP_TRY(hipMemcpy(&e, c->d_error, 4, hipMemcpyDeviceToHost));
    e |= bits;
    HIP_TRY(hipMemcpy(c->d_error, &e, 4, hipMemcpyHostToDevice));
    return MCRT_OK;
}

extern "C" int mcrt_enable_timing(mcrt_ctx *c, int on) { CTX_TRY(c); c->ins.timing_on = on != 0; c->ins.timing_level = on; return MCRT_OK; }
extern "C" int mcrt_get_kernel_times(mcrt_ctx *c, double avg_ms[3], uint32_t n[3], int reset)
{
    CTX_TRY(c);
    double sum[3] = { 0, 0, 0 }; uint32_t cnt[3] = { 0, 0, 0 };
    for (size_t i = 0; i < c->ins.ev_used; i++) {
        const TimedLaunch &t = c->ins.ev[i];
        float ms = 0;
        HIP_TRY(hipEventSynchronize(t.end));
        HIP_TRY(hipEventElapsedTime(&ms, t.start, t.end));
        sum[t.kind] += ms; cnt[t.kind]++;
    }
    for (int k = 0; k < 3; k++) { if (avg_ms) avg_ms[k] = cnt[k] ? sum[k] / (double)cnt[k] : 0.0; if (n) n[k] = cnt[k]; }
    if (reset) c->ins.ev_used = 0;
    return MCRT_OK;
}
extern "C" int mcrt_get_kernel_time(mcrt_ctx *c, double *avg_ms, uint32_t *n, int reset)
{
    double a[3]; uint32_t k[3];
    MCRT_TRY(mcrt_get_kernel_times(c, a, k, reset));
    if (avg_ms) *avg_ms = a[0];
    if (n) *n = k[0];
    return MCRT_OK;
}

extern "C" int mcrt_debug_math(mcrt_ctx *c, int op, const double *x, const double *y, double *out, uint32_t n)
{
    CTX_TRY(c);
    if (!x || !out || n == 0) return set_error(MCRT_ERR_INVALID, "mcrt_debug_math: bad arguments");
    Buf<double> dx, dy, dout;
    HIP_TRY(dx.alloc(n)); HIP_TRY(dout.alloc(n));
    HIP_TRY(hipMemcpy(dx, x, 8 * (size_t)n, hipMemcpyHostToDevice));
    if (y) { HIP_TRY(dy.alloc(n)); HIP_TRY(hipMemcpy(dy, y, 8 * (size_t)n, hipMemcpyHostToDevice)); }
    HIP_TRY(mcrt::launch_math_probe(op, dx, dy, dout, n, c->stream));
    HIP_TRY(hipStreamSynchronize(c->stream));
    HIP_TRY(hipMemcpy(out, dout, 8 * (size_t)n, hipMemcpyDeviceToHost));
    return MCRT_OK;
}

extern "C" int mcrt_debug_philox(mcrt_ctx *c, const uint32_t ctr[4], const uint32_t key[2], uint32_t out[4])
{
    CTX_TRY(c);
    Buf<uint32_t> d;
    HIP_TRY(d.alloc(4));
    HIP_TRY(mcrt::launch_philox_probe(ctr, key, d, c->stream));
    HIP_TRY(hipStreamSynchronize(c->stream));
    HIP_TRY(hipMemcpy(out, d, 16, hipMemcpyDeviceToHost));
    return MCRT_OK;
}
```

### mcray-tracing_amd/csrc/mcrt_beam.hip

```cpp
#include <hip/hip_fp16.h>
#include "mcrt_device.h"
#include "mcrt_walk.h"

#define BEAM_CT 256u
#define BEAM_QN 512
#define BEAM_EN 1024
#define BEAM_LN 2048

namespace mcrt {

MCRT_DEV uint32_t ford(float f) { const uint32_t b = __float_as_uint(f); return (b & 0x80000000u) ? ~b : (b | 0x80000000u); }
MCRT_DEV float funord(uint32_t u) { return __uint_as_float((u & 0x80000000u) ? (u & 0x7fffffffu) : ~u); }
MCRT_DEV float comp(f3 v, int k) { return k == 0 ? v.x : k == 1 ? v.y : v.z; }

MCRT_DEV int beam_slot(const BeamArgs &g, unsigned long long key, bool claim)
{
    uint32_t h = ((uint32_t)key ^ (uint32_t)(key >> 32) * 0x9e3779b1u) * 2654435761u;
    h ^= h >> 15;
    for (uint32_t p = 0; p < MCRT_BEAM_PROBES; p++) {
        const uint32_t s = (h + p) & (g.groups - 1u);
        unsigned long long k = claim ? __hip_atomic_load(&g.gkey[s], __ATOMIC_RELAXED, __HIP_MEMORY_SCOPE_AGENT) : g.gkey[s];
        if (k == 0ull && claim) {
            k = atomicCAS(&g.gkey[s], 0ull, key);
            if (k == 0ull) { k = key; atomicAdd(&g.lcount[7], 1u); }
        }
        if (k == key) return (int)s;
        if (k == 0ull) return -1;
    }
    return -1;
}

struct BeamRay { f3 f2, to; float u, v, cmax, dd; int dom, bid; bool neg; };
MCRT_DEV bool beam_ray(const FrameArgs &a, const BeamArgs &g, uint32_t i, bool claim, BeamRay &r)
{
    const size_t half = (size_t)(g.b & 1u) * a.ne * a.S;
    const uint32_t pid = a.queue[half + i];
    const uint32_t line = pid / a.S, scan = line - (line / a.ne_frame) * a.ne_frame;
    const float4 s0 = a.st0[half + i], s1 = a.st1[half + i];
    const Ray ry = ray_of(mk(s0.x, s0.y, s0.z), mk(s1.x, s1.y, s1.z), s0.w, a);
    r.f2 = ry.f2; r.to = ry.to;
    const f3 D = ry.to - ry.f2;
    const float ax = fabsf(D.x), ay = fabsf(D.y), az = fabsf(D.z);
    r.dom = (ax >= ay && ax >= az) ? 0 : (ay >= az ? 1 : 2);
    r.dd = comp(D, r.dom);
    const float ad = fabsf(r.dd);
    r.u = comp(D, (r.dom + 1) % 3) / ad; r.v = comp(D, (r.dom + 2) % 3) / ad;
    r.cmax = fmaxf(fmaxf(fabsf(r.f2.x), fabsf(r.f2.y)), fabsf(r.f2.z));
    r.neg = r.dd < 0.0f;
    const float sum = fabsf(r.f2.x) + fabsf(r.f2.y) + fabsf(r.f2.z) + fabsf(r.to.x) + fabsf(r.to.y) + fabsf(r.to.z);
    const bool ok = sum < 1e30f && ad > 0.0f && fabsf(r.u) <= 1.0f && fabsf(r.v) <= 1.0f;
    const uint32_t code = (uint32_t)r.dom * 2u + (r.neg ? 1u : 0u);
    if (g.groups == 0u) {
        const uint32_t hist = __float_as_int(s1.w) != (int)a.start_mat ? 1u : 0u;
        r.bid = (int)((scan * 2u + hist) * 6u + code);
    } else {
        r.bid = -1;
        if (ok) {
            const unsigned long long key = (1ull << 63) | ((unsigned long long)scan << 40) | ((unsigned long long)((uint32_t)__float_as_int(s1.w) & 0xffu) << 32)
                                           | (unsigned long long)a.from_tri[pid];
            const int slot = beam_slot(g, key, claim);
            if (slot >= 0) r.bid = slot * 6 + (int)code;
        }
    }
    return ok;
}

MCRT_DEV float wave_min(float x) { for (int o = 32; o > 0; o >>= 1) x = fminf(x, __shfl_xor(x, o, 64)); return x; }
MCRT_DEV float wave_max(float x) { for (int o = 32; o > 0; o >>= 1) x = fmaxf(x, __shfl_xor(x, o, 64)); return x; }

__global__ void __launch_bounds__(256) k_beam_clear(BeamArgs g)
{
    const uint32_t i = blockIdx.x * 256u + threadIdx.x;
    if (i < g.n_beams * MCRT_BEAM_REC) g.red[i] = (i & 8u) ? 0u : 0xffffffffu;
    if (i < g.groups) g.gkey[i] = 0ull;
    if (i < MCRT_BEAM_COUNTERS) g.lcount[i] = 0u;
    if (i <= MCRT_MAX_BOUNCES) g.l_counts[i] = 0u;
    if (i < MCRT_MAX_BOUNCES * MCRT_XCDS) g.l_cursors[(size_t)i * MCRT_CURSOR_STRIDE] = 0u;
}

__global__ void __launch_bounds__(256) k_beam_bounds(FrameArgs a, BeamArgs g)
{
    const uint32_t n = a.counts[g.b];
    const uint32_t wave = (blockIdx.x * 256u + threadIdx.x) >> 6, lane = threadIdx.x & 63u;
    const uint32_t base = (wave * g.stride + ((wave * 2654435761u) >> 16) % g.stride) * 64u;
    if (base >= n) return;
    const uint32_t i = base + lane;
    BeamRay r; r.bid = -1;
    bool live = i < n && beam_ray(a, g, i, true, r);
    if (g.groups != 0u) {
        const unsigned long long lost = __ballot(live && r.bid < 0);
        if (lost && lane == 0u) atomicAdd(&g.lcount[6], (uint32_t)__popcll(lost));
        live = live && r.bid >= 0;
    }
    unsigned long long todo = __ballot(live);
    while (todo) {
        const int cb = __builtin_amdgcn_readlane(r.bid, __ffsll((long long)todo) - 1);
        const bool mine = live && r.bid == cb;
        todo &= ~__ballot(mine);
        const float lo[5] = { r.u, r.v, r.f2.x, r.f2.y, r.f2.z }, hi[6] = { r.u, r.v, r.f2.x, r.f2.y, r.f2.z, r.cmax };
        uint32_t *w = g.red + (size_t)cb * MCRT_BEAM_REC;
#pragma unroll
        for (int k = 0; k < 5; k++) { const uint32_t m = ford(wave_min(mine ? lo[k] : INFINITY)); if ((int)lane == k && m < __hip_atomic_load(&w[k], __ATOMIC_RELAXED, __HIP_MEMORY_SCOPE_AGENT)) atomicMin(&w[k], m); }
#pragma unroll
        for (int k = 0; k < 6; k++) { const uint32_t m = ford(wave_max(mine ? hi[k] : -INFINITY)); if ((int)lane == 8 + k && m > __hip_atomic_load(&w[8 + k], __ATOMIC_RELAXED, __HIP_MEMORY_SCOPE_AGENT)) atomicMax(&w[8 + k], m); }
    }
}

struct BeamGeom { int dom; bool neg; float xref, w, m, umin, umax, vmin, vmax, alo, ahi, blo, bhi, smax; };
MCRT_DEV bool beam_box(const BeamGeom &B, f3 lo, f3 hi, float &s_begin)
{
    const float lod = comp(lo, B.dom), hid = comp(hi, B.dom);
    const float sb0 = B.neg ? B.xref - hid : lod - B.xref, sb1 = B.neg ? B.xref - lod : hid - B.xref;
    s_begin = sb0 - B.m;
    const float s0 = fmaxf(s_begin, -B.m), s1 = fminf(sb1 + B.m, B.smax);
    if (!(s0 <= s1)) return false;
    const float sa = s0 - B.w;
    const int ka = (B.dom + 1) % 3, kb = (B.dom + 2) % 3;
    {
        const float p1 = sa * B.umin, p2 = sa * B.umax, p3 = s1 * B.umin, p4 = s1 * B.umax;
        const float l = B.alo + fminf(fminf(p1, p2), fminf(p3, p4)) - B.m, h = B.ahi + fmaxf(fmaxf(p1, p2), fmaxf(p3, p4)) + B.m;
        if (!(l <= comp(hi, ka) && h >= comp(lo, ka))) return false;
    }
    {
        const float p1 = sa * B.vmin, p2 = sa * B.vmax, p3 = s1 * B.vmin, p4 = s1 * B.vmax;
        const float l = B.blo + fminf(fminf(p1, p2), fminf(p3, p4)) - B.m, h = B.bhi + fmaxf(fmaxf(p1, p2), fmaxf(p3, p4)) + B.m;
        if (!(l <= comp(hi, kb) && h >= comp(lo, kb))) return false;
    }
    return true;
}

MCRT_DEV void beam_collect(const FrameArgs &a, const BeamArgs &g, const uint32_t beam)
{
    __shared__ int q[2][BEAM_QN];
    __shared__ unsigned long long ent[BEAM_EN];
    __shared__ uint32_t leaf[BEAM_LN];
    __shared__ uint32_t nq[2], n_leaf, n_ent, overflow, list_at;
    const uint32_t lane = threadIdx.x;
    const uint32_t *w = g.red + (size_t)beam * MCRT_BEAM_REC;
    uint32_t *rec = g.rec + (size_t)beam * MCRT_BEAM_REC;
    float umin = funord(w[0]), vmin = funord(w[1]), umax = funord(w[8]), vmax = funord(w[9]);
    const bool empty = w[0] == 0xffffffffu;
    bool refused = !empty && !(umax - umin <= g.spread_cap && vmax - vmin <= g.spread_cap);
    if (!empty && lane == 0u) atomicAdd(&g.lcount[4], 1u);
    uint32_t li = beam;
    if (g.groups != 0u) {
        if (lane == 0u) list_at = (empty || refused) ? 0u : atomicAdd(&g.lcount[5], 1u);
        __syncthreads();
        li = list_at;
        if (li >= g.n_lists) refused = !empty;
    }
    if (empty || refused) {
        if (lane < MCRT_BEAM_REC) rec[lane] = lane == 0u || lane == 2u ? __float_as_uint(INFINITY) : lane == 1u || lane == 3u || lane == 13u ? __float_as_uint(-INFINITY) : 0u;
        if (refused && lane == 0u) atomicAdd(&g.lcount[3], 1u);
        return;
    }
    float cmax = funord(w[13]);
    for (int k = 0; k < 3; k++) cmax = fmaxf(cmax, fmaxf(fabsf(a.scene_lo[k]), fabsf(a.scene_hi[k])));
    cmax *= 1.0625f;
    const float m = cmax * 0x1p-18f;
    { const float pu = 0.0625f * (umax - umin) + 1e-6f, pv = 0.0625f * (vmax - vmin) + 1e-6f; umin -= pu; umax += pu; vmin -= pv; vmax += pv; }
    float flo[3], fhi[3];
    for (int k = 0; k < 3; k++) { const float l = funord(w[2 + k]), h = funord(w[10 + k]), p = 0.0625f * (h - l) + m; flo[k] = l - p; fhi[k] = h + p; }
    const uint32_t code = beam % 6u;
    BeamGeom B;
    B.dom = (int)(code >> 1); B.neg = (code & 1u) != 0u;
    const int ka = (B.dom + 1) % 3, kb = (B.dom + 2) % 3;
    B.xref = B.neg ? fhi[B.dom] : flo[B.dom]; B.w = fhi[B.dom] - flo[B.dom]; B.m = m;
    B.umin = umin; B.umax = umax; B.vmin = vmin; B.vmax = vmax; B.alo = flo[ka]; B.ahi = fhi[ka]; B.blo = flo[kb]; B.bhi = fhi[kb]; B.smax = 2.0f * cmax + m;

    if (lane == 0u) { nq[0] = 1u; nq[1] = 0u; n_leaf = 0u; n_ent = 0u; overflow = 0u; q[0][0] = 0; }
    __syncthreads();
    for (uint32_t level = 0; ; level++) {
        const uint32_t cur = level & 1u, cnt = nq[cur];
        if (cnt == 0u) break;
        if (level >= 256u) { if (lane == 0u) overflow = 1u; break; }
        for (uint32_t t = lane; t < cnt; t += BEAM_CT) {
            const uint4 *N = a.nodes_walk + 4 * (size_t)(uint32_t)q[cur][t];
            const uint4 q0 = N[0], q1 = N[1], q2 = N[2], q3 = N[3];
            const uint32_t wd[12] = { q0.x, q0.y, q0.z, q0.w, q1.x, q1.y, q1.z, q1.w, q2.x, q2.y, q2.z, q2.w };
            const int ref[4] = { (int)q3.x, (int)q3.y, (int)q3.z, (int)q3.w };
#pragma unroll
            for (int c = 0; c < 4; c++) {
                if (ref[c] == MCRT_BVH4_EMPTY) continue;
                float bx[6];
#pragma unroll
                for (int k = 0; k < 6; k++) bx[k] = __half2float(__ushort_as_half((unsigned short)((wd[2 * k + (c >> 1)] >> ((c & 1) * 16)) & 0xffffu)));
                float sb;
                if (!beam_box(B, mk(bx[0], bx[1], bx[2]), mk(bx[3], bx[4], bx[5]), sb)) continue;
                if (ref[c] >= 0) {
                    const uint32_t at = atomicAdd(&nq[cur ^ 1u], 1u);
                    if (at < BEAM_QN) q[cur ^ 1u][at] = ref[c]; else overflow = 1u;
                } else {
                    const uint32_t v = (uint32_t)~ref[c], first = v >> 3, nt = (v & 7u) + 1u;
                    const uint32_t at = atomicAdd(&n_leaf, nt);
                    if (at + nt <= BEAM_LN) { for (uint32_t k = 0; k < nt; k++) leaf[at + k] = first + k; } else overflow = 1u;
                }
            }
        }
        __syncthreads();
        if (lane == 0u) nq[cur] = 0u;
        if (nq[cur ^ 1u] > BEAM_QN) break;
        __syncthreads();
    }
    __syncthreads();
    for (uint32_t t = lane; t < (overflow ? 0u : n_leaf); t += BEAM_CT) {
        const float4 *T = a.tris + (size_t)leaf[t] * MCRT_TRI_PIECES;
        f3 plo, phi;
        float sb;
        tri_padded_bounds(xyz(T[0]), xyz(T[1]), xyz(T[2]), a.pad_abs, plo, phi);
        if (!beam_box(B, plo, phi, sb)) continue;
        const uint32_t at = atomicAdd(&n_ent, 1u);
        if (at < BEAM_EN) ent[at] = ((unsigned long long)ford(sb) << 32) | (unsigned long long)leaf[t]; else overflow = 1u;
    }
    __syncthreads();
    const bool lost = overflow != 0u;
    const uint32_t N = lost ? 0u : n_ent;
    uint32_t P = 1u; while (P < N) P <<= 1;
    for (uint32_t t = N + lane; t < P; t += BEAM_CT) ent[t] = ~0ull;
    __syncthreads();
    for (uint32_t k = 2u; k <= P; k <<= 1)
        for (uint32_t j = k >> 1; j > 0u; j >>= 1) {
            for (uint32_t t = lane; t < P; t += BEAM_CT) {
                const uint32_t l = t ^ j;
                if (l > t) {
                    const unsigned long long x = ent[t], y = ent[l];
                    if ((x > y) == ((t & k) == 0u)) { ent[t] = y; ent[l] = x; }
                }
            }
            __syncthreads();
        }
    const uint32_t keep = N < g.cap ? N : g.cap;
    for (uint32_t e = lane; e < keep; e += BEAM_CT) {
        const unsigned long long x = ent[e];
        const float4 *T = a.tris + (size_t)(uint32_t)x * MCRT_TRI_PIECES;
        const float4 t0 = T[0], t1 = T[1], t2 = T[2];
        float4 *L = (float4 *)(g.list + 4 * ((size_t)li * g.cap + e));
        L[0] = t0; L[1] = make_float4(t1.x, t1.y, t1.z, funord((uint32_t)(x >> 32))); L[2] = t2; L[3] = make_float4(0.0f, 0.0f, 0.0f, 0.0f);
    }
    const float s_end = lost ? -INFINITY : N > g.cap ? funord((uint32_t)(ent[g.cap] >> 32)) : INFINITY;
    if (lane == 0u) {
        rec[0] = __float_as_uint(umin); rec[1] = __float_as_uint(umax); rec[2] = __float_as_uint(vmin); rec[3] = __float_as_uint(vmax);
        for (int k = 0; k < 3; k++) { rec[4 + k] = __float_as_uint(flo[k]); rec[7 + k] = __float_as_uint(fhi[k]); }
        rec[10] = __float_as_uint(cmax); rec[11] = __float_as_uint(m); rec[12] = __float_as_uint(B.xref); rec[13] = __float_as_uint(s_end); rec[14] = keep; rec[15] = li;
        if (lost || N > g.cap) atomicAdd(&g.lcount[2], 1u);
    }
}

__global__ void __launch_bounds__(BEAM_CT) k_beam_collect(FrameArgs a, BeamArgs g)
{
    const uint32_t per = g.groups != 0u ? 6u : 1u;
    for (uint32_t k = 0; k < per; k++) {
        beam_collect(a, g, blockIdx.x * per + k);
        __syncthreads();
    }
}

__global__ void __launch_bounds__(256) k_beam_test(FrameArgs a, BeamArgs g, uint32_t pass)
{
    const uint32_t n = pass == 0u ? a.counts[g.b] : g.lcount[0];
    const uint32_t lane = threadIdx.x & 63u;
    const uint32_t base = (blockIdx.x * 256u + threadIdx.x) & ~63u;
    if (base >= n) return;
    const uint32_t j = base + lane;
    const bool live = j < n;
    const uint32_t ray = !live ? 0u : pass == 0u ? j : g.lq0[j];
    BeamRay r;
    bool member = beam_ray(a, g, ray, false, r) && live && r.bid >= 0;
    const uint32_t *rec = g.rec + (size_t)(member ? r.bid : 0) * MCRT_BEAM_REC;
    {
        const float4 b0 = ((const float4 *)rec)[0], b1 = ((const float4 *)rec)[1], b2 = ((const float4 *)rec)[2];
        member = member && r.u >= b0.x && r.u <= b0.y && r.v >= b0.z && r.v <= b0.w
                 && r.f2.x >= b1.x && r.f2.y >= b1.y && r.f2.z >= b1.z && r.f2.x <= b1.w && r.f2.y <= b2.x && r.f2.z <= b2.y && r.cmax <= b2.z;
    }
    const f3 f2 = r.f2, to = r.to;
    const f3 d = to - f2;
    const f3 inv = mk(rcp_dir(d.x), rcp_dir(d.y), rcp_dir(d.z));
    const f3 rc = ray_c(f2, inv);
    unsigned long long *keys = (g.b & 1u) ? a.key1 : a.key0;
    Best best; best.frac = 1.0f; best.tri = -1;
    if (pass != 0u && live) { const unsigned long long k = keys[ray]; best.frac = __uint_as_float((uint32_t)(k >> 32)); best.tri = (int)(uint32_t)k; }
    const float f2d = comp(f2, r.dom), sg = r.neg ? -1.0f : 1.0f;
    bool left = live && !member;
    unsigned long long todo = __ballot(member);
    const uint32_t first = pass == 0u ? 0u : g.near, cut = pass == 0u ? g.near : 0xffffffffu;
    while (todo) {
        const int cb = __builtin_amdgcn_readlane(r.bid, __ffsll((long long)todo) - 1);
        const bool mine = member && r.bid == cb;
        todo &= ~__ballot(mine);
        const u32x8 R = sload8(g.rec + (size_t)cb * MCRT_BEAM_REC + 8);
        const float m2 = 2.0f * __uint_as_float(R[3]), xref = __uint_as_float(R[4]);
        const uint32_t n_ent = R[6];
        float reach = best.tri >= 0 ? sg * ((f2d + best.frac * r.dd) - xref) + m2 : INFINITY;
        float limit = __uint_as_float(R[5]);
        const char *L = (const char *)(g.list + 4 * (size_t)R[7] * g.cap);
        for (uint32_t k = first; k < n_ent; k += 2u) {
            u32x8 A, A2; u32x4 C2, C22;
            const char *E = L + ((size_t)k << 6);
            asm volatile("s_load_dwordx8 %0, %4, 0x0\n\ts_load_dwordx4 %1, %4, 0x20\n\ts_load_dwordx8 %2, %4, 0x40\n\ts_load_dwordx4 %3, %4, 0x60\n\ts_waitcnt lgkmcnt(0)"
                         : "=&s"(A), "=&s"(C2), "=&s"(A2), "=&s"(C22) : "s"(E) : "memory");
            float begin = __uint_as_float(A[7]);
            if (k >= cut || !__any(mine && !(reach < begin))) { limit = begin; break; }
            int before = best.tri;
            packet_tri_test(A, C2, f2, to, inv, rc, a.pad_abs, mine, best);
            if (best.tri != before) reach = sg * ((f2d + best.frac * r.dd) - xref) + m2;
            if (k + 1u >= n_ent) break;
            begin = __uint_as_float(A2[7]);
            if (k + 1u >= cut || !__any(mine && !(reach < begin))) { limit = begin; break; }
            before = best.tri;
            packet_tri_test(A2, C22, f2, to, inv, rc, a.pad_abs, mine, best);
            if (best.tri != before) reach = sg * ((f2d + best.frac * r.dd) - xref) + m2;
        }
        left = left || (mine && !(reach < limit || limit == INFINITY));
    }
    if (live && best.tri >= 0) keys[ray] = ((unsigned long long)__float_as_uint(best.frac) << 32) | (unsigned long long)(uint32_t)best.tri;
    const unsigned long long lm = __ballot(left);
    if (lm) {
        uint32_t at = 0;
        if (lane == 0u) at = atomicAdd(&g.lcount[pass], (uint32_t)__popcll(lm));
        at = __shfl(at, 0, 64);
        if (left) (pass == 0u ? g.lq0 : g.lq1)[at + (uint32_t)__popcll(lm & ((1ull << lane) - 1ull))] = ray;
    }
}

MCRT_DEV uint32_t beam_walk_as(uint32_t b) { return (b & 1u) ? 2u : 1u; }
__global__ void __launch_bounds__(256) k_beam_gather(FrameArgs a, BeamArgs g, uint32_t which)
{
    const uint32_t n = g.lcount[which];
    const uint32_t *lq = which == 0u ? g.lq0 : g.lq1;
    const size_t np = (size_t)a.ne * a.S, in = (g.b & 1u) ? np : 0, out = np - in;
    unsigned long long *keys = (g.b & 1u) ? a.key0 : a.key1;
    if (blockIdx.x == 0u && threadIdx.x == 0u) g.l_counts[beam_walk_as(g.b)] = n;
    for (uint32_t j = blockIdx.x * 256u + threadIdx.x; j < n; j += gridDim.x * 256u) {
        const uint32_t r = lq[j];
        a.st0[out + j] = a.st0[in + r]; a.st1[out + j] = a.st1[in + r]; keys[j] = MCRT_KEY_MISS;
    }
}
__global__ void __launch_bounds__(256) k_beam_scatter(FrameArgs a, BeamArgs g, uint32_t which)
{
    const uint32_t n = g.lcount[which];
    const uint32_t *lq = which == 0u ? g.lq0 : g.lq1;
    unsigned long long *keys = (g.b & 1u) ? a.key1 : a.key0;
    const unsigned long long *walked = (g.b & 1u) ? a.key0 : a.key1;
    for (uint32_t j = blockIdx.x * 256u + threadIdx.x; j < n; j += gridDim.x * 256u) keys[lq[j]] = walked[j];
}

hipError_t launch_beam(const FrameArgs &a, const BeamArgs &g, hipStream_t st)
{
    const uint32_t np = a.ne * a.S, blocks = (np + 255u) / 256u;
    uint32_t setup = g.n_beams * MCRT_BEAM_REC;
    if (setup < MCRT_MAX_BOUNCES * MCRT_XCDS) setup = MCRT_MAX_BOUNCES * MCRT_XCDS;
    if (setup < g.groups) setup = g.groups;
    hipLaunchKernelGGL(k_beam_clear, dim3((setup + 255u) / 256u), dim3(256), 0, st, g);
    hipLaunchKernelGGL(k_beam_bounds, dim3((blocks + g.stride - 1u) / g.stride), dim3(256), 0, st, a, g);
    hipLaunchKernelGGL(k_beam_collect, dim3(g.groups != 0u ? g.groups : g.n_beams), dim3(BEAM_CT), 0, st, a, g);
    hipLaunchKernelGGL(k_beam_test, dim3(blocks), dim3(256), 0, st, a, g, 0u);
    const uint32_t which = g.near < g.cap ? 1u : 0u;
    if (which) hipLaunchKernelGGL(k_beam_test, dim3(blocks), dim3(256), 0, st, a, g, 1u);
    const uint32_t few = blocks < 2048u ? blocks : 2048u;
    hipLaunchKernelGGL(k_beam_gather, dim3(few), dim3(256), 0, st, a, g, which);
    hipError_t e = hipGetLastError();
    if (e != hipSuccess) return e;
    FrameArgs w = a;
    w.counts = g.l_counts; w.cursors = g.l_cursors; w.packet_mask = 0u;
    e = launch_trace(w, (g.b & 1u) ? 2u : 1u, false, st);
    if (e != hipSuccess) return e;
    hipLaunchKernelGGL(k_beam_scatter, dim3(few), dim3(256), 0, st, a, g, which);
    return hipGetLastError();
}

}
```

### mcray-tracing_amd/csrc/mcrt_ctx.h

```cpp
#pragma once
#include "../../include/mcrt.h"
#include "mcrt_internal.h"
#include "mcrt_hip.h"

#include <cstdlib>
#include <cstring>
#include <vector>

#define CTX_TRY(ctx) do { if (!(ctx)) return mcrt::set_error(MCRT_ERR_INVALID, "null context"); HIP_TRY(hipSetDevice((ctx)->device)); } while (0)

struct Consts {
    float axial_res_f; double axial_res_mm, time_step_us, row_dt_us, max_travel_us; uint32_t axial_res_um, max_rows;
};

struct PathBufs {
    Buf<float4> st0, st1, st2, mrec;
    Buf<unsigned long long> key0, key1;
    Buf<uint32_t> q, counts, seg_count, cursors, from_tri;
    size_t paths = 0; uint32_t depth = 0;
};
struct BeamBufs {
    Buf<uint32_t> red, rec, lcount, l_counts, l_cursors;
    Buf<uint4> list;
    Buf<unsigned long long> gkey;
    uint32_t beams = 0, lists = 0, groups = 0, cap = 0;
};
struct Work {
    Stream stream, side[MCRT_SIDE_STREAMS];
    Event ev_bounce[MCRT_MAX_BOUNCES], ev_join[MCRT_SIDE_STREAMS], ev_done;
    Buf<int> stack_ovf;
    Buf<mcrt_segment> segs;
    Buf<int32_t> hits;
    PathBufs b;
    BeamBufs beam;
};

#define MCRT_SPECKLE_FUSE_DEFAULT 2u
struct Knobs {
    uint32_t ksplit_limit = MCRT_KSPLIT_DEFAULT, trace_blocks = 0, trace_blocks_wide = 0, wide_from = 0 , wide_max_tree_mb = 128, groups = MCRT_GROUPS_DEFAULT, march_streams = MCRT_SIDE_STREAMS_DEFAULT, march_blocks = 0;
    bool no_overlap = false, no_priority = false, no_fast_div = false, no_lean = false;
    uint32_t path_groups = MCRT_PATH_GROUPS_DEFAULT;
    uint32_t path_max = MCRT_PATH_MAX_DEFAULT;
    uint32_t packet_mask = MCRT_PACKET_MASK_DEFAULT, packet_from = MCRT_PACKET_FROM;
    bool retire_late = true;
    bool fold_b0 = false;
    uint32_t beam_b1 = 1;
    uint32_t beam_from = MCRT_BEAM_FROM;
    uint32_t beam_last = MCRT_BEAM_LAST_DEFAULT;
    uint32_t beam_deep_from = MCRT_BEAM_DEEP_FROM;
    uint32_t beam_groups = 0;
    uint32_t beam_cap = MCRT_BEAM_CAP_DEFAULT, beam_near = MCRT_BEAM_NEAR_DEFAULT;
    bool render_row_tile = false;
    uint32_t speckle_fuse = MCRT_SPECKLE_FUSE_DEFAULT;
    bool test_hooks = false;
};

struct StagedTable : Staging {
    std::vector<float> on_dev; uint32_t key[2] = { 0, 0 };
    int put(const float *src, uint32_t R, uint32_t n, size_t room, hipStream_t st)
    {
        const size_t len = (size_t)n * R;
        if (key[0] == R && key[1] == n && !memcmp(src, on_dev.data(), 4 * len)) return MCRT_OK;
        float *h = nullptr;
        MCRT_TRY(begin(room, st, &h));
        on_dev.resize(room);
        for (uint32_t r = 0; r < R; r++)
            for (uint32_t k = 0; k < n; k++) h[(size_t)k * R + r] = src[(size_t)r * n + k];
        key[0] = key[1] = 0;
        MCRT_TRY(commit(len, st));
        memcpy(on_dev.data(), src, 4 * len);
        key[0] = R; key[1] = n;
        return MCRT_OK;
    }
};

struct MapCache {
    struct Key {
        std::vector<unsigned char> bytes;
        template <class T> Key &add(const T &v) { return add(&v, sizeof v); }
        Key &add(const void *p, size_t n) { bytes.insert(bytes.end(), (const unsigned char *)p, (const unsigned char *)p + n); return *this; }
    };
    struct Slot { Buf<float> d; std::vector<unsigned char> key; uint64_t used = 0; };
    std::vector<Slot> slot; uint64_t clock = 0;
    explicit MapCache(size_t slots) : slot(slots) {}
    static size_t pad(size_t n) { return (n + 255u) & ~(size_t)255u; }
    template <class Fill> int get(const Key &key, size_t n, hipStream_t st, Fill fill, const float **maps)
    {
        Slot *lru = &slot[0];
        for (Slot &s : slot) {
            if (s.used && s.key == key.bytes) { s.used = ++clock; *maps = s.d; return MCRT_OK; }
            if (s.used < lru->used) lru = &s;
        }
        std::vector<float> m(n, 0.0f);
        MCRT_TRY(fill(m));
        HIP_TRY(hipStreamSynchronize(st));
        lru->used = 0;
        HIP_TRY(lru->d.grow(n));
        HIP_TRY(hipMemcpy(lru->d, m.data(), n * 4, hipMemcpyHostToDevice));
        lru->key = key.bytes; lru->used = ++clock;
        *maps = lru->d;
        return MCRT_OK;
    }
};

struct TimedLaunch { Event start, end; int kind = 0; };

struct Scene {
    bool have = false;
    mcrt_bvh bvh{};
    mcrt_bvh4 bvh4{};
    Buf<float4> d_nodes, d_tris, d_mats;
    mcrt_bvh4_node *walked_nodes = nullptr; bool walked_stale = true;
    Buf<uint4> d_nodes_walk;
    Buf<uint4> d_meshes;
    Buf<uint32_t> d_tri_slot;
    Buf<float4> d_tris_id;
    uint32_t n_mesh = 0, n_mat = 0, start_mat = 0;
    bool start_silent = false;
    int builder = MCRT_BVH_HOST_SAH; bool host_bvh_stale = false;
    std::vector<uint32_t> tri_mesh;
    float lo[3] = { 0, 0, 0 }, hi[3] = { 0, 0, 0 };
    float spacing[3] = { 1, 1, 1 };
    Event ev_update; hipStream_t update_stream = nullptr; bool update_pending = false;
    ~Scene() { free(walked_nodes); mcrt_free_bvh(&bvh); mcrt_free_bvh4(&bvh4); }
};
struct Tables {
    Buf<double> d_row_thr; uint32_t thr_rows = 0; double thr_dt = 0.0, thr_end = 0.0;
    float verified_res = 0.0f; bool fast_div = false, fast_div_all = false;
    Buf<float4> d_mtab; float mtab_key[2] = { 0.0f, 0.0f }; bool mtab_valid = false;
};
struct Accumulators {
    Buf<long long> d_acc; Buf<uint32_t> d_flags;
    uint32_t clean_ne = 0, clean_rows = 0;
};
struct ImageStages {
    MapCache maps{ 1 }, cmaps{ 1 }, vmaps{ 4 };
    Buf<float> d_tmp;
    Buf<float> d_disp; StagedTable tgc;
    StagedTable lat_rows, elev_rows;
    Buf<unsigned long long> d_recon;
    Buf<uint32_t> d_votes;
};
struct Instrumentation {
    Buf<unsigned long long> d_stats; bool stats_on = false;
    bool timing_on = false; int timing_level = 0;
    std::vector<TimedLaunch> ev; size_t ev_used = 0;
    uint32_t last_beam_mask = 0;
    bool last_beam_far = false;
    float last_lean_bound = 0.0f; uint32_t last_march_rows = 0;
};

struct mcrt_ctx {
    int device = 0; uint32_t n_cu = 256;
    Knobs knobs;
    Stream own_stream; hipStream_t stream = nullptr;
    std::vector<Work> work;
    Event ev_start;
    mcrt_params p{};
    Consts c{};
    Buf<uint32_t> d_error;
    Scene scene;
    Buf<float2> d_tex; uint32_t tex_n = 0; bool tex_finite = false;
    Buf<float> d_pos, d_dir; uint32_t n_el = 0;
    Buf<int> label_ovf;
    Staging pose_stage[2];
    Tables tab;
    Accumulators acc;
    ImageStages img;
    Instrumentation ins;
};

namespace mcrt {
int check_device_error(mcrt_ctx *c);
int stage_poses(mcrt_ctx *c, size_t lines, const float *dev[2]);
}
```

### mcray-tracing_amd/csrc/mcrt_internal.h

```cpp
#pragma once
#include <stdint.h>

#define MCRT_BVH_MAX_DEPTH 32
#define MCRT_STACK 64
#define MCRT_KSPLIT_DEFAULT 262144
#ifndef MCRT_KSPLIT_MAX
#define MCRT_KSPLIT_MAX 1048576
#endif
#define MCRT_GROUPS_DEFAULT 1
#define MCRT_SIDE_STREAMS 4
#define MCRT_SIDE_STREAMS_DEFAULT 0
#define MCRT_SIDE_STREAMS_TWO_FROM 5242880u
#define MCRT_LBVH_LEAF 1
#define MCRT_XCDS 8
#define MCRT_CURSOR_STRIDE 64
#define MCRT_XCD_MIN_ITEMS 262144
#define MCRT_PACKET_MASK_DEFAULT 2u
#define MCRT_PACKET_FROM 262144u
#define MCRT_BEAM_FROM 2097152u
#define MCRT_BEAM_LAST_DEFAULT 2u
#define MCRT_BEAM_DEEP_FROM 6291456u
#define MCRT_BEAM_GROUPS_PER_LINE 32u
#define MCRT_BEAM_LISTS_PER_GROUP 1u
#define MCRT_BEAM_CAP_DEFAULT 512u
#define MCRT_BEAM_NEAR_DEFAULT 512u
#define MCRT_BEAM_SPREAD 0.25f
#define MCRT_BEAM_SAMPLE_FROM 4194304u
#define MCRT_BEAM_SAMPLE_STRIDE 16u
#define MCRT_PATH_MAX_DEFAULT 655360u
#define MCRT_PATH_GROUPS_DEFAULT 2u
#define MCRT_MAX_ROWS 2048
#define MCRT_MAX_BOUNCES 16
#define MCRT_STATS_WORDS (256 + 2560)

#define MCRT_TRI_PIECES 3

namespace mcrt {
int set_error(int code, const char *fmt, ...);
const char *tuning_env(const char *name);
}
#ifdef MCRT_H
namespace mcrt {
struct HostTree { const mcrt_bvh *bvh; const mcrt_bvh4 *bvh4; };
int ctx_bvh_builder(const mcrt_ctx *c);
int upload_scene_with_tree(mcrt_ctx *c, const float *tri, const uint32_t *tri_mesh, uint32_t n_tri, const mcrt_mesh *meshes, uint32_t n_mesh,
                           const float *mats, uint32_t n_mat, uint32_t start_mat, const float spacing[3], const HostTree *pre);
int update_triangles_with_tree(mcrt_ctx *c, const float *tri, uint32_t n_tri, const HostTree *pre);
int volume_check(const char *fn, const mcrt_sweep *sw, const mcrt_volume_grid *g);
}
#endif
```

### mcray-tracing_amd/csrc/mcrt_kernels.h

```cpp
#pragma once
#include <hip/hip_runtime.h>
#include <stdint.h>
#include "../../include/mcrt.h"
#include "mcrt_internal.h"

namespace mcrt {

struct FrameArgs {
    const uint4 *nodes_walk;
    int *stack_ovf;
    const float4 *tris;
    const float4 *tris_id;
    const uint4 *meshes;
    const float4 *mats;
    const float2 *tex;
    const float *el_pos;
    const float *el_dir;
    const double *row_thr;
    float4 *st0, *st1, *st2;
    uint32_t *queue;
    unsigned long long *key0, *key1;
    uint32_t *from_tri;
    const uint32_t *tri_slot;
    uint32_t *counts;
    uint32_t *cursors;
    mcrt_segment *segs;
    int32_t *hits;
    float4 *mrec;
    const float4 *mtab;
    uint32_t *seg_count;
    long long *acc;
    uint32_t *flags;
    unsigned long long *stats;
    uint32_t *error_flag;
    unsigned long long *stamps;
    uint32_t n_nodes, S, B, R, e_begin, ne, ne_frame, pose_stride, acc_stride, acc_off, trace_blocks, trace_blocks_wide, wide_from, packet_mask, march_blocks, ksplit_limit, frame, seed, start_mat, tex_n, tex_mask, sanitize, tex_finite, fast_div, want_segs, tex_shift, march_rows, n_mat, n_mesh;
    float scene_lo[3], scene_hi[3];
    float freq, eps, I0, offs, sx, sy, sz, tex_res, axial_res_f, pad_abs, tex_rcp, lean_bound;
    double axial_res_mm, time_step, row_dt, max_travel, sos_d, inv_row_dt;
    double thr_end;
    uint32_t retire_late;
    uint32_t beam_mask;
    uint32_t fold_b0;
};

#define MCRT_BEAM_SLOTS 12u
#define MCRT_BEAM_REC 16u
#define MCRT_BEAM_CAP_MAX 1024u
#define MCRT_BEAM_PROBES 4u
#define MCRT_BEAM_COUNTERS 8u
struct BeamArgs {
    uint32_t *red;
    uint32_t *rec;
    uint4 *list;
    unsigned long long *gkey;
    uint32_t *lq0, *lq1;
    uint32_t *lcount;
    uint32_t *l_counts, *l_cursors;
    uint32_t b;
    uint32_t groups;
    uint32_t n_beams, n_lists, cap, near, stride;
    float spread_cap;
};

constexpr uint32_t MCRT_ALL_BOUNCES = 0xffffffffu;

struct ConvTaps { float ax[16]; float lat[32]; uint32_t n_ax, n_lat; };

struct PixelPass { uint32_t n, n_pad, F, frames_per_chunk, vec; };

struct BmodeArgs {
    const float *grey;
    const float *map_col, *map_row;
    float *state;
    uint8_t *out;
    float alpha;
    uint32_t E, R, reset;
    PixelPass pass;
};

struct CompoundArgs {
    const float *src;
    const float *maps;
    float *state;
    void *out;
    float alpha;
    uint32_t E, R;
    PixelPass pass;
    uint32_t N, reset;
    uint32_t mode;
    float feather;
    float weight[16];
};
enum { COMPOUND_PLAIN = 0, COMPOUND_WEIGHTED = 1, COMPOUND_MAX = 2, COMPOUND_MEDIAN = 3 };

struct VolumeArgs {
    const float *src;
    const float *maps;
    void *out;
    uint32_t E, R, K;
    PixelPass pass;
};

struct ViewArgs { float origin[3], di[3], dj[3], ds[3]; uint32_t nx, ny, n_steps, F, nu, nv, nw; };

struct RenderArgs {
    const void *vol;
    float *out;
    uint8_t *out8;
    float *depth;
    ViewArgs view;
    uint32_t mode;
    uint32_t row_tile;
    float lo, inv_range, threshold, inv_ramp, opacity, depth_cue, t_cut, inv_steps;
};

#ifndef SRAD_TH
#define SRAD_TH 16
#endif
#ifndef SRAD_TW
#define SRAD_TW 64
#endif
#define SRAD_FUSE_MAX 4
struct SpeckleArgs {
    const float *src;
    float *dst;
    uint32_t H, W;
    uint32_t n;
    uint32_t first;
    uint32_t tx, ty;
    float lam4;
    float q0sq[SRAD_FUSE_MAX], kq[SRAD_FUSE_MAX];
};

#define RECON_TU 32
#define RECON_TV 8
#define RECON_TW 8
#define RECON_MAX_FILL 3
#define RECON_MAX_TILES (1u << 24)
struct ReconBlock {
    const float *pos, *dir;
    uint32_t *stats;
    uint32_t R, n_samples;
    uint32_t nu, nv, nw, fill_radius, fill_min;
    uint32_t tu, tv;
    float A[9], b[3], row_u;
};
struct ReconArgs {
    const float *stack;
    ReconBlock blk;
    unsigned long long *sum;
    uint32_t *count;
    float *out;
    uint32_t *count_out;
    uint32_t mode;
    float value_max, empty;
    double qscale;
};

struct LabelArgs {
    uint8_t *tissue;
    int32_t *interface;
    uint32_t *crossings;
    uint32_t rule;
    float Ls;
};

struct LabelGatherArgs {
    const uint8_t *src;
    const float *map_plane, *map_col, *map_row;
    uint8_t *out;
    uint32_t E, R, K;
    PixelPass pass;
};

struct ReconLabelArgs {
    const uint8_t *stack;
    ReconBlock blk;
    uint32_t *votes;
    uint8_t *out;
    uint32_t *count_out, *votes_out;
    uint32_t n_vox, n_labels;
};

struct RenderLabelArgs {
    const uint8_t *labels;
    const float *depth;
    uint8_t *out;
    ViewArgs view;
};

hipError_t launch_init(const FrameArgs &a, hipStream_t st);
hipError_t launch_trace(const FrameArgs &a, uint32_t b, bool stats, hipStream_t st);
hipError_t launch_beam(const FrameArgs &a, const BeamArgs &g, hipStream_t st);
hipError_t launch_nodes_walk(const float4 *nodes, uint32_t n_nodes, uint4 *out, hipStream_t st);
hipError_t launch_nodes_walk_decode(const uint4 *walk, uint32_t n_nodes, float4 *out, hipStream_t st);
uint32_t lane_stack_entries();
uint32_t lane_wide_from();
hipError_t launch_shade(const FrameArgs &a, uint32_t b, bool stats, hipStream_t st);
uint32_t path_blocks(size_t np);
hipError_t launch_path(const FrameArgs &a, hipStream_t st);
hipError_t launch_march(const FrameArgs &a, uint32_t b, bool stats, hipStream_t st);
hipError_t launch_finalize(long long *acc, uint32_t *flags, float *rf, uint32_t ne, uint32_t R, const uint32_t *error_flag, hipStream_t st);
hipError_t launch_convolve(float *img, float *tmp, uint32_t n_img, uint32_t E, uint32_t R, const ConvTaps &taps, hipStream_t st);
hipError_t launch_convolve_depth(float *img, float *tmp, uint32_t n_img, uint32_t E, uint32_t R, const ConvTaps &taps, const float *lat, hipStream_t st);
hipError_t launch_elevation(const float *planes, float *rf, uint32_t F, uint32_t K, uint32_t E, uint32_t R, const float *w, hipStream_t st);
hipError_t launch_envelope(float *img, uint32_t E, uint32_t R, hipStream_t st);
hipError_t launch_remap(const float *img, uint32_t n_img, uint32_t E, uint32_t R, const float *map_col, const float *map_row, float *out, uint32_t n, hipStream_t st);
hipError_t launch_bmode_peak(const float *rf, uint32_t F, uint32_t E, uint32_t R, const float *tgc, float *peak, hipStream_t st);
hipError_t launch_bmode_grey(const float *rf, uint32_t F, uint32_t E, uint32_t R, const float *tgc, const float *peak , float ref,
                             float *peak_out , uint32_t mode, float gain, float dr, float *grey, hipStream_t st);
hipError_t launch_bmode(const BmodeArgs &a, hipStream_t st);
hipError_t launch_compound(const CompoundArgs &a, bool out8, hipStream_t st);
hipError_t launch_volume(const VolumeArgs &a, bool out8, hipStream_t st);
hipError_t launch_render(const RenderArgs &a, bool in8, hipStream_t st);
// ... 21 lines not shown
```

### mcray-tracing_amd/csrc/mcrt_trace.cpp

```cpp
#include "mcrt_ctx.h"
#include "mcrt_kernels.h"

#include <hip/hip_runtime.h>
#include <cmath>
#include <cstring>
#include <vector>
#include <algorithm>
#include <utility>

using mcrt::set_error;

static int get_work(mcrt_ctx *c, size_t g, Work **out)
{
    while (c->work.size() <= g) {
        Work w;
        for (Event &e : w.ev_join) HIP_TRY(ensure_event(e));
        for (Event &e : w.ev_bounce) HIP_TRY(ensure_event(e));
        HIP_TRY(ensure_event(w.ev_done));
        c->work.push_back(std::move(w));
    }
    *out = &c->work[g];
    return MCRT_OK;
}

// ... 12 lines not shown
        HIP_TRY(hipStreamCreateWithPriority(&w.side[i].h, hipStreamNonBlocking, prio_low));
    }
    *out = w.side[i];
    return MCRT_OK;
}

static int ensure_acc(mcrt_ctx *c, uint32_t ne)
{
    const size_t need = (size_t)ne * c->p.n_rows, needf = (size_t)ne * ((c->p.n_rows + 31u) >> 5);
    if (need > c->acc.d_acc.cap || needf > c->acc.d_flags.cap) {
        HIP_TRY(hipStreamSynchronize(c->stream));
        c->acc.clean_ne = 0;
        HIP_TRY(c->acc.d_acc.grow(need)); HIP_TRY(c->acc.d_flags.grow(needf));
    }
    if (c->acc.clean_ne != ne || c->acc.clean_rows != c->p.n_rows) {
        HIP_TRY(hipMemsetAsync(c->acc.d_acc, 0, need * 8, c->stream));
        HIP_TRY(hipMemsetAsync(c->acc.d_flags, 0, needf * 4, c->stream));
    }
    c->acc.clean_ne = 0; c->acc.clean_rows = 0;
    return MCRT_OK;
}

static int check_ready(mcrt_ctx *c, uint32_t e0, uint32_t e1, const float *pose_pos = nullptr)
{
    if (!c->scene.have) return set_error(MCRT_ERR_INVALID, "no scene uploaded");
    if (!c->d_tex) return set_error(MCRT_ERR_INVALID, "no texture uploaded");
    if (c->tex_n != c->p.tex_n) return set_error(MCRT_ERR_INVALID, "texture is %u^3 but params say %u^3", c->tex_n, c->p.tex_n);
    if (!pose_pos) {
        if (!c->d_pos) return set_error(MCRT_ERR_INVALID, "no transducer set");
        if (c->n_el != c->p.n_elements) return set_error(MCRT_ERR_INVALID, "transducer has %u elements but params say %u", c->n_el, c->p.n_elements);
    }
    if (e0 >= e1 || e1 > c->p.n_elements) return set_error(MCRT_ERR_INVALID, "scan-line range [%u,%u) invalid for %u elements", e0, e1, c->p.n_elements);
    return MCRT_OK;
}

struct Plan {
    bool latency = false;
    uint32_t groups = 1;
    uint32_t trace_blocks = 0, trace_blocks_wide = 0;
    uint32_t e[17] = {};
    uint32_t sides[16] = {};
    size_t ovf[16] = {};
};

static Plan plan_pass(const mcrt_ctx *c, uint32_t e0, uint32_t e1, uint32_t n_frames, bool one_group)
{
    Plan P;
    const uint32_t ne = e1 - e0, S = c->p.n_samples;
    P.latency = !c->ins.stats_on && (uint64_t)ne * n_frames * S <= c->knobs.path_max;
    uint32_t groups = (one_group || c->ins.stats_on) ? 1u : c->knobs.groups;
    if (!one_group && groups == 1u && P.latency) groups = c->knobs.path_groups;
    P.groups = std::max(1u, std::min({ groups, ne, 16u }));
    for (uint32_t g = 0; g <= P.groups; g++) P.e[g] = e0 + (uint32_t)(((uint64_t)ne * g) / P.groups);
    P.trace_blocks = c->knobs.trace_blocks ? c->knobs.trace_blocks : c->n_cu * 4u;
    P.trace_blocks_wide = c->knobs.trace_blocks_wide ? c->knobs.trace_blocks_wide : c->n_cu * 5u;
    if ((uint64_t)c->scene.bvh4.n_nodes * 64ull > (uint64_t)c->knobs.wide_max_tree_mb * 1048576ull) P.trace_blocks_wide = 0;
    const uint32_t lds_part = mcrt::lane_stack_entries();
    const size_t deep = c->scene.bvh4.max_stack > lds_part ? c->scene.bvh4.max_stack - lds_part : 0;
    for (uint32_t g = 0; g < P.groups; g++) {
        const uint64_t np = (uint64_t)(P.e[g + 1] - P.e[g]) * n_frames * S;
        if (!P.latency) P.sides[g] = c->knobs.march_streams ? c->knobs.march_streams : (P.trace_blocks_wide != 0u && np >= (uint64_t)MCRT_SIDE_STREAMS_TWO_FROM) ? 2u : 1u;
        uint32_t blocks = std::max({ c->knobs.trace_blocks, c->knobs.trace_blocks_wide, c->n_cu * 5u });
        if (P.latency) blocks = std::max(blocks, mcrt::path_blocks(np));
        P.ovf[g] = deep * blocks * 256;
    }
    return P;
}

static int ensure_work(Work &w, size_t np, uint32_t B, size_t ovf, int out)
{
    if (out >= 2 && w.segs.cap < np * B) { HIP_TRY(hipDeviceSynchronize()); HIP_TRY(w.segs.alloc(np * B)); }
    if (out >= 1 && w.hits.cap < np * B) { HIP_TRY(hipDeviceSynchronize()); HIP_TRY(w.hits.alloc(np * B)); }
    if (ovf > w.stack_ovf.cap) { HIP_TRY(hipDeviceSynchronize()); HIP_TRY(w.stack_ovf.alloc(ovf)); }
    if (np <= w.b.paths && B <= w.b.depth) return MCRT_OK;
    HIP_TRY(hipDeviceSynchronize());
    w.b = PathBufs();
    PathBufs &b = w.b;
    HIP_TRY(b.st0.alloc(2 * np)); HIP_TRY(b.st1.alloc(2 * np)); HIP_TRY(b.st2.alloc(2 * np));
    HIP_TRY(b.key0.alloc(np)); HIP_TRY(b.key1.alloc(np)); HIP_TRY(b.from_tri.alloc(np));
    HIP_TRY(b.q.alloc(2 * np)); HIP_TRY(b.seg_count.alloc(np));
    HIP_TRY(b.counts.alloc(MCRT_MAX_BOUNCES + 1));
    HIP_TRY(b.cursors.alloc((size_t)MCRT_MAX_BOUNCES * MCRT_XCDS * MCRT_CURSOR_STRIDE));
    HIP_TRY(b.mrec.alloc(3 * np * B));
    b.paths = np; b.depth = B;
    return MCRT_OK;
}

static void fill_pass(mcrt_ctx *c, const Plan &P, mcrt::FrameArgs &a, uint32_t frame, uint32_t acc_ne, bool accumulate, int out, const float *pose_pos, const float *pose_dir)
{
    memset(&a, 0, sizeof a);
    a.nodes_walk = c->scene.d_nodes_walk; a.tris = c->scene.d_tris; a.meshes = c->scene.d_meshes; a.mats = c->scene.d_mats; a.tex = c->d_tex;
    a.el_pos = pose_pos ? pose_pos : c->d_pos; a.el_dir = pose_pos ? pose_dir : c->d_dir; a.pose_stride = pose_pos ? c->p.n_elements : 0u;
    a.row_thr = c->tab.d_row_thr;
    a.acc = c->acc.d_acc; a.flags = c->acc.d_flags; a.acc_stride = acc_ne;
    a.tri_slot = c->scene.d_tri_slot; a.tris_id = c->scene.d_tris_id; a.mtab = c->tab.d_mtab;
    a.stats = c->ins.d_stats; a.error_flag = c->d_error; a.stamps = c->ins.d_stats + 8;
    a.n_mat = c->scene.n_mat; a.n_mesh = c->scene.n_mesh; a.n_nodes = c->scene.bvh4.n_nodes; a.S = c->p.n_samples; a.B = c->p.max_depth; a.R = c->p.n_rows;
    a.ksplit_limit = c->knobs.ksplit_limit;
    if (c->ins.stats_on) a.ksplit_limit = 0;
    for (int i = 0; i < 3; i++) { a.scene_lo[i] = c->scene.lo[i]; a.scene_hi[i] = c->scene.hi[i]; }
    a.trace_blocks = P.trace_blocks; a.trace_blocks_wide = P.trace_blocks_wide;
    a.wide_from = c->knobs.wide_from ? c->knobs.wide_from : mcrt::lane_wide_from();
    a.march_blocks = c->knobs.march_blocks;
    a.want_segs = out >= 2 ? 1u : 0u;
    a.frame = frame; a.seed = c->p.seed; a.start_mat = c->scene.start_mat; a.tex_n = c->tex_n; a.tex_mask = (c->tex_n & (c->tex_n - 1u)) == 0u ? c->tex_n - 1u : 0u;
    a.sanitize = c->p.sanitize_tir; a.tex_finite = c->tex_finite ? 1u : 0u;
    a.freq = c->p.frequency; a.eps = c->p.intensity_epsilon; a.I0 = c->p.initial_intensity; a.offs = c->p.ray_start_offset;
    a.sx = c->scene.spacing[0]; a.sy = c->scene.spacing[1]; a.sz = c->scene.spacing[2]; a.tex_res = c->p.tex_res; a.axial_res_f = c->c.axial_res_f; a.pad_abs = c->scene.bvh.pad_abs; a.tex_rcp = 1.0f / c->p.tex_res; a.fast_div = c->tab.fast_div ? 1u : 0u;
    a.tex_shift = 0; while ((1u << a.tex_shift) < c->tex_n) a.tex_shift++;
    a.lean_bound = 0.0f;
    if (c->tab.fast_div_all && a.tex_mask && a.tex_shift <= 10u) {
        const float lim = 2147483648.0f * c->p.tex_res * (1.0f - 0x1p-20f);
        a.lean_bound = lim < 1e18f ? lim : 1e18f;
        if (!(a.lean_bound > 0.0f)) a.lean_bound = 0.0f;
    }
    a.axial_res_mm = c->c.axial_res_mm; a.time_step = c->c.time_step_us; a.row_dt = c->c.row_dt_us;
    a.max_travel = c->c.max_travel_us; a.sos_d = (double)c->p.speed_of_sound; a.inv_row_dt = 1.0 / c->c.row_dt_us;
    a.march_rows = 0u;
    {
        const double g = a.max_travel * a.inv_row_dt;
        if (a.lean_bound > 0.0f && c->tex_n == 256u && g >= 0.0 && g < (double)(MCRT_MAX_ROWS + 1)) {
            const uint32_t gmax = (uint32_t)g;
            a.march_rows = (gmax + 2u > c->p.n_rows + 1u) ? gmax + 2u : c->p.n_rows + 1u;
        }
    }
    c->ins.last_lean_bound = a.lean_bound; c->ins.last_march_rows = a.march_rows;
    const bool image_only = !c->ins.stats_on && out == 0;
    a.thr_end = c->tab.thr_end;
    a.retire_late = image_only && c->knobs.retire_late ? 1u : 0u;
    a.fold_b0 = image_only && c->knobs.fold_b0 && !P.latency && accumulate && c->tex_finite && c->scene.start_silent && c->p.n_samples % 256u == 0u ? 1u : 0u;
}

static void fill_group(const mcrt_ctx *c, const Work &w, mcrt::FrameArgs &a, uint32_t n_frames, uint32_t b0, uint32_t b1, uint32_t acc_e0, int out)
{
    a.stack_ovf = w.stack_ovf; a.segs = w.segs; a.hits = out >= 1 ? (int32_t *)w.hits : nullptr;
    a.st0 = w.b.st0; a.st1 = w.b.st1; a.st2 = w.b.st2; a.queue = w.b.q; a.key0 = w.b.key0; a.key1 = w.b.key1; a.from_tri = w.b.from_tri;
    a.counts = w.b.counts; a.cursors = w.b.cursors; a.mrec = w.b.mrec; a.seg_count = w.b.seg_count;
    a.acc_off = b0 - acc_e0;
    a.e_begin = b0; a.ne_frame = b1 - b0; a.ne = (b1 - b0) * n_frames;
    a.packet_mask = (c->ins.stats_on || (uint64_t)a.ne * a.S < c->knobs.packet_from) ? 0u : c->knobs.packet_mask;
}

static uint32_t beam_wanted(const mcrt_ctx *c, const Plan &P, const mcrt::FrameArgs &a)
{
    if (P.latency || c->ins.stats_on || a.pose_stride != 0u || a.B < 2u || a.n_nodes == 0u || c->knobs.beam_b1 == 0u) return 0u;
    const bool force = c->knobs.beam_b1 == 2u;
    const uint64_t np = (uint64_t)a.ne * a.S;
    uint32_t mask = 0;
    if (force || ((a.packet_mask & 2u) != 0u && np >= c->knobs.beam_from)) mask |= 2u;
    if (force || np >= c->knobs.beam_deep_from)
        for (uint32_t b = 2; b <= c->knobs.beam_last && b < a.B; b++) mask |= 1u << b;
    return mask;
}
struct BeamPlan { mcrt::BeamArgs g = {}; uint32_t mask = 0, beams_b1 = 0, groups = 0; };
static int fill_beam(const mcrt_ctx *c, Work &w, const mcrt::FrameArgs &a, uint32_t mask, BeamPlan &bp)
{
    const uint32_t cap = c->knobs.beam_cap;
    bp.mask = mask; bp.beams_b1 = a.ne_frame * MCRT_BEAM_SLOTS; bp.groups = 0;
    if (mask & ~2u) {
        const uint64_t want = c->knobs.beam_groups ? c->knobs.beam_groups : (uint64_t)a.ne_frame * MCRT_BEAM_GROUPS_PER_LINE;
        bp.groups = 1u;
        while ((uint64_t)bp.groups * 2u <= want && bp.groups < (1u << 20)) bp.groups *= 2u;
        if (!c->knobs.beam_groups && bp.groups < want) bp.groups *= 2u;
    }
    const uint32_t beams = std::max((mask & 2u) ? bp.beams_b1 : 0u, bp.groups * 6u);
    const uint32_t lists = std::max((mask & 2u) ? bp.beams_b1 : 0u, bp.groups * MCRT_BEAM_LISTS_PER_GROUP);
    BeamBufs &b = w.beam;
    if (beams > b.beams || lists > b.lists || bp.groups > b.groups || cap != b.cap) {
        HIP_TRY(hipDeviceSynchronize());
        b.beams = b.lists = b.groups = b.cap = 0;
        HIP_TRY(b.red.alloc((size_t)beams * MCRT_BEAM_REC)); HIP_TRY(b.rec.alloc((size_t)beams * MCRT_BEAM_REC)); HIP_TRY(b.list.alloc(((size_t)lists * cap + 1) * 4));
        HIP_TRY(b.gkey.alloc(std::max(bp.groups, 1u)));
        HIP_TRY(b.lcount.grow((size_t)MCRT_MAX_BOUNCES * MCRT_BEAM_COUNTERS)); HIP_TRY(b.l_counts.grow(MCRT_MAX_BOUNCES + 1)); HIP_TRY(b.l_cursors.grow((size_t)MCRT_MAX_BOUNCES * MCRT_XCDS * MCRT_CURSOR_STRIDE));
        b.beams = beams; b.lists = lists; b.groups = bp.groups; b.cap = cap;
    }
    const size_t np = (size_t)a.ne * a.S;
    mcrt::BeamArgs &g = bp.g;
    g.red = b.red; g.rec = b.rec; g.list = b.list; g.gkey = b.gkey; g.lcount = b.lcount; g.l_counts = b.l_counts; g.l_cursors = b.l_cursors;
    g.cap = cap; g.near = std::min(c->knobs.beam_near, cap);
    g.stride = np >= MCRT_BEAM_SAMPLE_FROM ? MCRT_BEAM_SAMPLE_STRIDE : 1u;
    g.spread_cap = MCRT_BEAM_SPREAD;
    return MCRT_OK;
}
static mcrt::BeamArgs beam_args(const BeamPlan &bp, const mcrt::FrameArgs &a, uint32_t b)
{
    mcrt::BeamArgs g = bp.g;
    const size_t other = (b & 1u) ? 0 : (size_t)a.ne * a.S;
    g.b = b; g.lcount = bp.g.lcount + (size_t)b * MCRT_BEAM_COUNTERS;
    g.lq0 = a.queue + other; g.lq1 = (uint32_t *)(a.st2 + other);
    g.groups = b == 1u ? 0u : bp.groups;
    g.n_beams = b == 1u ? bp.beams_b1 : bp.groups * 6u;
    g.n_lists = b == 1u ? bp.beams_b1 : bp.groups * MCRT_BEAM_LISTS_PER_GROUP;
    return g;
}

static int check_overflow(const mcrt_ctx *c, const Plan &P, const mcrt::FrameArgs &a, const Work &w)
{
    const uint32_t lds_part = mcrt::lane_stack_entries();
    if (c->scene.bvh4.max_stack <= lds_part) return MCRT_OK;
    const uint32_t blocks = P.latency ? mcrt::path_blocks((size_t)a.ne * a.S) : std::max(a.trace_blocks, a.trace_blocks_wide);
    const size_t need = (size_t)(c->scene.bvh4.max_stack - lds_part) * blocks * 256;
    if (need > w.stack_ovf.cap) return set_error(MCRT_ERR_LIMIT, "traversal-stack overflow: %zu entries needed, the work set holds %zu", need, w.stack_ovf.cap);
    return MCRT_OK;
}

template <class Launch> static int timed_launch(mcrt_ctx *c, int kind, hipStream_t st, Launch launch)
{
    if (!c->ins.timing_on || (kind != 0 && c->ins.timing_level < 2)) { HIP_TRY(launch()); return MCRT_OK; }
    if (c->ins.ev_used == c->ins.ev.size()) {
        if (c->ins.ev.size() >= 65536) return set_error(MCRT_ERR_LIMIT, "timing buffer full: call mcrt_get_kernel_time(reset=1)");
        TimedLaunch t;
        HIP_TRY(hipEventCreate(&t.start.h)); HIP_TRY(hipEventCreate(&t.end.h));
        c->ins.ev.push_back(std::move(t));
    }
    TimedLaunch &t = c->ins.ev[c->ins.ev_used];
    HIP_TRY(hipEventRecord(t.start, st));
    HIP_TRY(launch());
    HIP_TRY(hipEventRecord(t.end, st));
    t.kind = kind; c->ins.ev_used++;
    return MCRT_OK;
}

static int run_bounce(mcrt_ctx *c, Work &w, hipStream_t st, const mcrt::FrameArgs &a, const BeamPlan &beam, uint32_t b, uint32_t sides, bool accumulate, bool overlap)
{
    if ((beam.mask >> b) & 1u) MCRT_TRY(timed_launch(c, 0, st, [&] { return mcrt::launch_beam(a, beam_args(beam, a, b), st); }));
    else MCRT_TRY(timed_launch(c, 0, st, [&] { return mcrt::launch_trace(a, b, c->ins.stats_on, st); }));
    MCRT_TRY(timed_launch(c, 1, st, [&] { return mcrt::launch_shade(a, b, c->ins.stats_on, st); }));
    if (!accumulate || (a.fold_b0 && b == 0u)) return MCRT_OK;
    hipStream_t ms = st;
    if (overlap) {
        HIP_TRY(hipEventRecord(w.ev_bounce[b], st));
        MCRT_TRY(side_stream(c, w, b % sides, &ms));
        HIP_TRY(hipStreamWaitEvent(ms, w.ev_bounce[b], 0));
    }
    return timed_launch(c, 2, ms, [&] { return mcrt::launch_march(a, b, c->ins.stats_on, ms); });
}

static int enqueue_pass(mcrt_ctx *c, const Plan &P, const mcrt::FrameArgs *args, const BeamPlan *beams, Work *const *ws, bool accumulate)
{
    const bool overlap = !c->knobs.no_overlap;
    hipStream_t gst[16] = { c->stream };
    for (uint32_t g = 1; g < P.groups; g++) MCRT_TRY(work_stream(*ws[g], &gst[g]));
    if (c->scene.update_pending && c->scene.update_stream != c->stream) HIP_TRY(hipStreamWaitEvent(c->stream, c->scene.ev_update, 0));
    HIP_TRY(hipEventRecord(c->ev_start, c->stream));
    for (uint32_t g = 0; g < P.groups; g++) {
        if (gst[g] != c->stream) HIP_TRY(hipStreamWaitEvent(gst[g], c->ev_start, 0));
        HIP_TRY(mcrt::launch_init(args[g], gst[g]));
    }
    if (P.latency) {
        for (uint32_t g = 0; g < P.groups; g++) {
            MCRT_TRY(timed_launch(c, 0, gst[g], [&] { return mcrt::launch_path(args[g], gst[g]); }));
        }
        for (uint32_t g = 0; g < P.groups && accumulate; g++) {
            MCRT_TRY(timed_launch(c, 2, gst[g], [&] { return mcrt::launch_march(args[g], mcrt::MCRT_ALL_BOUNCES, false, gst[g]); }));
        }
    } else {
        for (uint32_t b = 0; b < c->p.max_depth; b++)
            for (uint32_t g = 0; g < P.groups; g++) {
                MCRT_TRY(run_bounce(c, *ws[g], gst[g], args[g], beams[g], b, P.sides[g], accumulate, overlap));
            }
    }
    for (uint32_t g = 0; g < P.groups; g++) {
        for (uint32_t i = 0; i < P.sides[g] && accumulate && overlap; i++) {
            if (!ws[g]->side[i]) continue;
            HIP_TRY(hipEventRecord(ws[g]->ev_join[i], ws[g]->side[i]));
            HIP_TRY(hipStreamWaitEvent(gst[g], ws[g]->ev_join[i], 0));
        }
        if (gst[g] != c->stream) {
            HIP_TRY(hipEventRecord(ws[g]->ev_done, gst[g]));
            HIP_TRY(hipStreamWaitEvent(c->stream, ws[g]->ev_done, 0));
        }
    }
    return MCRT_OK;
}

static int run_pass(mcrt_ctx *c, uint32_t frame, uint32_t n_frames, uint32_t e0, uint32_t e1, bool accumulate, bool one_group, int out, const float *pose_pos = nullptr, const float *pose_dir = nullptr)
{
    const Plan P = plan_pass(c, e0, e1, n_frames, one_group);
    mcrt::FrameArgs pass, args[16];
    BeamPlan beams[16];
    Work *ws[16];
    fill_pass(c, P, pass, frame, e1 - e0, accumulate, out, pose_pos, pose_dir);
    for (uint32_t g = 0; g < P.groups; g++) {
        MCRT_TRY(get_work(c, g, &ws[g]));
        MCRT_TRY(ensure_work(*ws[g], (size_t)(P.e[g + 1] - P.e[g]) * n_frames * c->p.n_samples, c->p.max_depth, P.ovf[g], out));
        args[g] = pass;
        fill_group(c, *ws[g], args[g], n_frames, P.e[g], P.e[g + 1], e0, out);
        MCRT_TRY(check_overflow(c, P, args[g], *ws[g]));
        if (const uint32_t mask = beam_wanted(c, P, args[g])) { MCRT_TRY(fill_beam(c, *ws[g], args[g], mask, beams[g])); args[g].beam_mask = mask & ~3u; }
    }
    c->ins.last_beam_mask = beams[0].mask; c->ins.last_beam_far = c->knobs.beam_near < c->knobs.beam_cap;
    return enqueue_pass(c, P, args, beams, ws, accumulate);
}

static int finalize(mcrt_ctx *c, float *rf_dev, uint32_t lines)
{
    HIP_TRY(mcrt::launch_finalize(c->acc.d_acc, c->acc.d_flags, rf_dev, lines, c->p.n_rows, c->d_error, c->stream));
    c->acc.clean_ne = lines; c->acc.clean_rows = c->p.n_rows;
    return MCRT_OK;
}

static int trace_frames(mcrt_ctx *c, uint32_t frame, uint32_t n_frames, uint32_t e0, uint32_t e1, const float *pose_pos, const float *pose_dir, float *rf_dev)
{
    CTX_TRY(c);
    MCRT_TRY(check_ready(c, e0, e1, pose_pos));
    if (!rf_dev) return set_error(MCRT_ERR_INVALID, "null rf_dev");
    if (n_frames == 0 || n_frames > 1024) return set_error(MCRT_ERR_LIMIT, "n_frames must be 1..1024");
    if ((uint64_t)(e1 - e0) * n_frames * c->p.n_samples > (1ull << 27))
        return set_error(MCRT_ERR_LIMIT, "%u frames x %u scan-lines x %u samples: more than 2^27 paths in one pass", n_frames, e1 - e0, c->p.n_samples);
    const uint32_t lines = (e1 - e0) * n_frames;
    MCRT_TRY(ensure_acc(c, lines));
    MCRT_TRY(run_pass(c, frame, n_frames, e0, e1, true, false, 0, pose_pos, pose_dir));
    return finalize(c, rf_dev, lines);
}

extern "C" int mcrt_trace_frames(mcrt_ctx *c, uint32_t frame, uint32_t n_frames, uint32_t e0, uint32_t e1, float *rf_dev)
{
    return trace_frames(c, frame, n_frames, e0, e1, nullptr, nullptr, rf_dev);
}

extern "C" int mcrt_trace_frame(mcrt_ctx *c, uint32_t frame, uint32_t e0, uint32_t e1, float *rf_dev)
{
    return mcrt_trace_frames(c, frame, 1, e0, e1, rf_dev);
}

int mcrt::stage_poses(mcrt_ctx *c, size_t lines, const float *dev[2])
{
    for (int k = 0; k < 2; k++) {
        if (is_device_pointer(dev[k])) continue;
        float *h = nullptr;
        MCRT_TRY(c->pose_stage[k].begin(3 * lines, c->stream, &h));
        memcpy(h, dev[k], 12 * lines);
        MCRT_TRY(c->pose_stage[k].commit(3 * lines, c->stream));
        dev[k] = c->pose_stage[k].dev;
    }
    return MCRT_OK;
}

extern "C" int mcrt_trace_frames_poses(mcrt_ctx *c, uint32_t frame, uint32_t n_frames, uint32_t e0, uint32_t e1,
                                       const float *pos, const float *dir, float *rf_dev)
{
    CTX_TRY(c);
    if (!pos || !dir) return set_error(MCRT_ERR_INVALID, "mcrt_trace_frames_poses: null pose tables");
    if (n_frames == 0 || n_frames > 1024) return set_error(MCRT_ERR_LIMIT, "n_frames must be 1..1024");
    const float *dev[2] = { pos, dir };
    MCRT_TRY(mcrt::stage_poses(c, (size_t)n_frames * c->p.n_elements, dev));
    return trace_frames(c, frame, n_frames, e0, e1, dev[0], dev[1], rf_dev);
}

static int copy_out(mcrt_ctx *c, uint32_t ne, int32_t *hits, mcrt_segment *segs, uint32_t *seg_count)
{
    const size_t np = (size_t)ne * c->p.n_samples, B = c->p.max_depth;
    const Work &w = c->work[0];
    HIP_TRY(hipStreamSynchronize(c->stream));
    MCRT_TRY(mcrt::check_device_error(c));
    std::vector<uint32_t> cnt;
    if (!seg_count && (hits || segs)) { cnt.resize(np); seg_count = cnt.data(); }
    if (seg_count) HIP_TRY(hipMemcpy(seg_count, w.b.seg_count, np * 4, hipMemcpyDeviceToHost));
    if (segs) {
        HIP_TRY(hipMemcpy(segs, w.segs, np * B * sizeof(mcrt_segment), hipMemcpyDeviceToHost));
        for (size_t p = 0; p < np; p++)
            for (size_t b = seg_count[p]; b < B; b++) memset(&segs[p * B + b], 0, sizeof(mcrt_segment));
    }
    if (hits) {
        HIP_TRY(hipMemcpy(hits, w.hits, np * B * 4, hipMemcpyDeviceToHost));
        for (size_t p = 0; p < np; p++)
            for (size_t b = seg_count[p]; b < B; b++) hits[p * B + b] = -2;
    }
    return MCRT_OK;
}

extern "C" int mcrt_trace_frame_debug(mcrt_ctx *c, uint32_t frame, uint32_t e0, uint32_t e1, float *rf_dev,
                                      int32_t *hits, mcrt_segment *segs, uint32_t *seg_count)
{
    CTX_TRY(c);
    MCRT_TRY(check_ready(c, e0, e1));
    if (!rf_dev) return set_error(MCRT_ERR_INVALID, "null rf_dev");
    MCRT_TRY(ensure_acc(c, e1 - e0));
    MCRT_TRY(run_pass(c, frame, 1, e0, e1, true, true, segs ? 2 : 1));
    MCRT_TRY(finalize(c, rf_dev, e1 - e0));
    return copy_out(c, e1 - e0, hits, segs, seg_count);
}

extern "C" int mcrt_cast_rays(mcrt_ctx *c, uint32_t frame, uint32_t e0, uint32_t e1, mcrt_segment *segs, uint32_t *seg_count, int32_t *hits)
{
    CTX_TRY(c);
    MCRT_TRY(check_ready(c, e0, e1));
    MCRT_TRY(run_pass(c, frame, 1, e0, e1, false, true, segs ? 2 : 1));
    return copy_out(c, e1 - e0, hits, segs, seg_count);
}

extern "C" int mcrt_default_label_opts(mcrt_label_opts *o)
{
    if (!o) return set_error(MCRT_ERR_INVALID, "mcrt_default_label_opts: null options");
    o->rule = MCRT_LABEL_TRACED; o->start_offset = -1.0f;
    return MCRT_OK;
}

extern "C" int mcrt_label_frames(mcrt_ctx *c, uint32_t n_frames, uint32_t e0, uint32_t e1, const float *pos, const float *dir, const mcrt_label_opts *o,
                                 uint8_t *tissue_dev, int32_t *interface_dev, uint32_t *crossings_dev)
{
    CTX_TRY(c);
    static const char fn[] = "mcrt_label_frames";
    mcrt_label_opts d;
    mcrt_default_label_opts(&d);
    if (!o) o = &d;
    if (!c->scene.have) return set_error(MCRT_ERR_INVALID, "%s: no scene uploaded", fn);
    if ((pos == nullptr) != (dir == nullptr)) return set_error(MCRT_ERR_INVALID, "%s: pos and dir go together (null %s)", fn, pos ? "dir" : "pos");
    if (!pos) {
        if (!c->d_pos) return set_error(MCRT_ERR_INVALID, "%s: no transducer set", fn);
        if (c->n_el != c->p.n_elements) return set_error(MCRT_ERR_INVALID, "%s: transducer has %u elements but params say %u", fn, c->n_el, c->p.n_elements);
        if (n_frames != 1) return set_error(MCRT_ERR_INVALID, "%s: the context's transducer is one pose: n_frames must be 1 (%u)", fn, n_frames);
    }
    if (e0 >= e1 || e1 > c->p.n_elements) return set_error(MCRT_ERR_INVALID, "%s: scan-line range [%u,%u) invalid for %u elements", fn, e0, e1, c->p.n_elements);
    if (!tissue_dev && !interface_dev && !crossings_dev) return set_error(MCRT_ERR_INVALID, "%s: no output asked for", fn);
    if (o->rule != MCRT_LABEL_TRACED && o->rule != MCRT_LABEL_GEOMETRIC) return set_error(MCRT_ERR_INVALID, "%s: unknown rule %u", fn, o->rule);
    if (!std::isfinite(o->start_offset) || o->start_offset == 0.0f) return set_error(MCRT_ERR_INVALID, "%s: start_offset must be finite and not 0 (%g)", fn, (double)o->start_offset);
    if (n_frames == 0) return set_error(MCRT_ERR_INVALID, "%s: n_frames must be 1..1024", fn);
    if (n_frames > 1024) return set_error(MCRT_ERR_LIMIT, "%s: n_frames must be 1..1024 (%u)", fn, n_frames);
    if (c->scene.n_mat > 254) return set_error(MCRT_ERR_LIMIT, "%s: at most 254 materials fit a tissue byte (%u)", fn, c->scene.n_mat);
    const uint32_t lines = (e1 - e0) * n_frames, blocks = mcrt::label_blocks(lines), lds_part = mcrt::label_stack_entries();
    const size_t ovf = c->scene.bvh4.max_stack > lds_part ? (size_t)(c->scene.bvh4.max_stack - lds_part) * blocks * 64 : 0;
    if (ovf > c->label_ovf.cap) { HIP_TRY(hipDeviceSynchronize()); HIP_TRY(c->label_ovf.alloc(ovf)); }
    const float *dev[2] = { pos, dir };
    if (pos) MCRT_TRY(mcrt::stage_poses(c, (size_t)n_frames * c->p.n_elements, dev));
    if (c->scene.update_pending && c->scene.update_stream != c->stream) HIP_TRY(hipStreamWaitEvent(c->stream, c->scene.ev_update, 0));
    mcrt::FrameArgs a;
    memset(&a, 0, sizeof a);
    a.nodes_walk = c->scene.d_nodes_walk; a.tris = c->scene.d_tris; a.tris_id = c->scene.d_tris_id; a.meshes = c->scene.d_meshes; a.n_nodes = c->scene.bvh4.n_nodes;
    a.n_mat = c->scene.n_mat; a.n_mesh = c->scene.n_mesh; a.start_mat = c->scene.start_mat; a.pad_abs = c->scene.bvh.pad_abs;
    a.sx = c->scene.spacing[0]; a.sy = c->scene.spacing[1]; a.sz = c->scene.spacing[2];
    a.el_pos = pos ? dev[0] : c->d_pos; a.el_dir = pos ? dev[1] : c->d_dir; a.pose_stride = pos ? c->p.n_elements : 0u;
    a.e_begin = e0; a.ne_frame = e1 - e0; a.ne = lines;
    a.row_thr = c->tab.d_row_thr; a.R = c->p.n_rows; a.thr_end = c->tab.thr_end; a.inv_row_dt = 1.0 / c->c.row_dt_us;
    a.max_travel = c->c.max_travel_us; a.sos_d = (double)c->p.speed_of_sound;
    a.offs = o->start_offset < 0.0f ? c->p.ray_start_offset : o->start_offset;
    a.stack_ovf = c->label_ovf; a.error_flag = c->d_error;
    mcrt::LabelArgs l;
    l.tissue = tissue_dev; l.interface = interface_dev; l.crossings = crossings_dev; l.rule = o->rule; l.Ls = (float)(2.0 * c->p.depth_cm);
    HIP_TRY(mcrt::launch_label(a, l, c->stream));
    return MCRT_OK;
}
```

Measured before the change: 543.5 million rays/s.

## Sort beam-test rays by beam id and extend beam path to bounce three

Adds a counting-sort pass (rank, scan, place) that groups rays by beam id into 64-aligned padded segments, so each wavefront in the first beam-test pass mostly handles one beam and runs fewer per-beam loop iterations. Ordering is enabled by default for bounce 3, and the default last beam bounce is raised from 2 to 3 so that bounce uses the beam path. This costs three extra kernel launches per ordered bounce, a single-block scan, padded lanes, and a one-time buffer allocation. It also adds debug hooks and an optional counter of beams met per wave.

```diff
diff --git a/include/mcrt.h b/include/mcrt.h
--- a/include/mcrt.h
+++ b/include/mcrt.h
@@ -334,6 +334,8 @@
 int mcrt_debug_fast_paths(mcrt_ctx *ctx, uint32_t out[4]);
 int mcrt_debug_beam(mcrt_ctx *ctx, uint32_t out[6]);
 int mcrt_debug_beam_bounce(mcrt_ctx *ctx, uint32_t b, uint32_t out[8]);
+int mcrt_debug_beam_order(mcrt_ctx *ctx, uint32_t b, uint32_t out[5]);
+int mcrt_debug_beam_layout(const uint32_t *counts, uint32_t n, uint32_t *bases, uint32_t out[4]);
 int mcrt_debug_set_error(mcrt_ctx *ctx, uint32_t bits);
 
 #ifdef __cplusplus
diff --git a/mcray-tracing_amd/__init__.py b/mcray-tracing_amd/__init__.py
--- a/mcray-tracing_amd/__init__.py
+++ b/mcray-tracing_amd/__init__.py
@@ -1,5 +1,5 @@
 from ._lib import load_library, build_library, McrtError, Params, MeshRec, BvhNode, Stats, BmodeParams, Focus, Compound, Sweep, VolumeGrid, CompoundOpts, LabelOpts, RenderView, RenderOpts, SpeckleOpts, ReconOpts, ReconLabelOpts, SEGMENT_DTYPE
-from .api import Context, Group, shard_range, Simulator, bmode_params, Transducer, Psf, host_build_bvh, host_build_bvh4, host_row_thresholds, host_texture, host_psf, host_psf_focus, focus_struct, row_pitch_mm, host_transducer, host_scan_maps, host_elevation_axis, host_elevation_planes, host_psf_elevation, host_transducer_steered, host_compound_maps, host_transducer_swept, host_volume_maps, sweep_struct, sweep_tilts, volume_grid, cplane_grid, sagittal_grid, compound_struct, compound_opts_struct, host_compound_weights, label_opts_struct, render_view, render_opts_struct, RENDER_MODES, speckle_opts_struct, host_speckle_tables, recon_opts_struct, recon_label_opts_struct, host_recon_transform, RECON_MODES, LABEL_RULES, LABEL_NONE, LABEL_MAX_CROSSINGS, LABEL_CAPPED
+from .api import Context, Group, shard_range, Simulator, bmode_params, Transducer, Psf, host_build_bvh, host_build_bvh4, host_row_thresholds, host_texture, host_psf, host_psf_focus, focus_struct, row_pitch_mm, host_transducer, host_scan_maps, host_beam_layout, host_elevation_axis, host_elevation_planes, host_psf_elevation, host_transducer_steered, host_compound_maps, host_transducer_swept, host_volume_maps, sweep_struct, sweep_tilts, volume_grid, cplane_grid, sagittal_grid, compound_struct, compound_opts_struct, host_compound_weights, label_opts_struct, render_view, render_opts_struct, RENDER_MODES, speckle_opts_struct, host_speckle_tables, recon_opts_struct, recon_label_opts_struct, host_recon_transform, RECON_MODES, LABEL_RULES, LABEL_NONE, LABEL_MAX_CROSSINGS, LABEL_CAPPED
 from . import synth, scene_io
 
 
diff --git a/mcray-tracing_amd/_lib.py b/mcray-tracing_amd/_lib.py
--- a/mcray-tracing_amd/_lib.py
+++ b/mcray-tracing_amd/_lib.py
@@ -113,7 +113,7 @@
            "mcrt_envelope", "mcrt_scan_convert", "mcrt_default_bmode", "mcrt_bmode_frames", "mcrt_export_rf", "mcrt_alloc", "mcrt_free", "mcrt_memcpy_d2h",
            "mcrt_memcpy_h2d", "mcrt_enable_stats", "mcrt_get_stats", "mcrt_enable_timing", "mcrt_get_kernel_time", "mcrt_get_kernel_times",
            "mcrt_build_bvh", "mcrt_free_bvh", "mcrt_get_bvh", "mcrt_build_bvh4", "mcrt_free_bvh4", "mcrt_get_bvh4", "mcrt_row_thresholds", "mcrt_generate_texture", "mcrt_psf_kernels", "mcrt_psf_focus_kernels",
-           "mcrt_transducer_elements", "mcrt_transducer_elevation_axis", "mcrt_elevation_planes", "mcrt_psf_elevation_kernels", "mcrt_elevation_frames", "mcrt_debug_math", "mcrt_debug_philox", "mcrt_debug_stamps", "mcrt_debug_tail_histograms", "mcrt_debug_set_error", "mcrt_debug_fast_paths", "mcrt_debug_beam", "mcrt_debug_beam_bounce", "mcrt_scan_maps",
+           "mcrt_transducer_elements", "mcrt_transducer_elevation_axis", "mcrt_elevation_planes", "mcrt_psf_elevation_kernels", "mcrt_elevation_frames", "mcrt_debug_math", "mcrt_debug_philox", "mcrt_debug_stamps", "mcrt_debug_tail_histograms", "mcrt_debug_set_error", "mcrt_debug_fast_paths", "mcrt_debug_beam", "mcrt_debug_beam_bounce", "mcrt_debug_beam_order", "mcrt_debug_beam_layout", "mcrt_scan_maps",
            "mcrt_group_create", "mcrt_group_destroy", "mcrt_group_size", "mcrt_group_root", "mcrt_group_member", "mcrt_group_shard", "mcrt_group_set_params",
            "mcrt_group_set_bvh_builder", "mcrt_group_upload_scene", "mcrt_group_update_triangles", "mcrt_group_refit_triangles", "mcrt_group_upload_texture",
            "mcrt_group_set_transducer", "mcrt_group_trace_frames", "mcrt_group_trace_frames_poses", "mcrt_group_synchronize", "mcrt_group_last_pass_ms", "mcrt_group_last_scene_seconds",
@@ -200,7 +200,7 @@
         "mcrt_default_recon_label_opts": [C.POINTER(ReconLabelOpts), u32],
         "mcrt_recon_label_frames": [vp, vp, u32, u32, u32, vp, vp, C.c_double, C.c_double, C.POINTER(VolumeGrid), C.POINTER(ReconLabelOpts), vp, vp, vp, vp],
         "mcrt_render_label_frames": [vp, vp, u32, u32, u32, u32, C.POINTER(RenderView), vp, vp],
-        "mcrt_debug_math": [vp, i32, vp, vp, vp, u32], "mcrt_debug_philox": [vp, vp, vp, vp], "mcrt_debug_stamps": [vp, vp, i32], "mcrt_debug_tail_histograms": [vp, vp, i32], "mcrt_debug_set_error": [vp, u32], "mcrt_debug_fast_paths": [vp, vp], "mcrt_debug_beam": [vp, vp], "mcrt_debug_beam_bounce": [vp, u32, vp],
+        "mcrt_debug_math": [vp, i32, vp, vp, vp, u32], "mcrt_debug_philox": [vp, vp, vp, vp], "mcrt_debug_stamps": [vp, vp, i32], "mcrt_debug_tail_histograms": [vp, vp, i32], "mcrt_debug_set_error": [vp, u32], "mcrt_debug_fast_paths": [vp, vp], "mcrt_debug_beam": [vp, vp], "mcrt_debug_beam_bounce": [vp, u32, vp], "mcrt_debug_beam_order": [vp, u32, vp], "mcrt_debug_beam_layout": [vp, u32, vp, vp],
         "mcrt_scan_maps": [u32, u32, C.c_double, C.c_double, u32, u32, u32, u32, vp, vp],
         "mcrt_group_create": [vp, u32, C.POINTER(vp)], "mcrt_group_destroy": [vp], "mcrt_group_size": [vp], "mcrt_group_root": [vp], "mcrt_group_member": [vp, u32],
         "mcrt_group_shard": [u32, u32, u32, C.POINTER(u32), C.POINTER(u32)], "mcrt_group_set_params": [vp, C.POINTER(Params)], "mcrt_group_set_bvh_builder": [vp, i32],
@@ -210,7 +210,7 @@
         "mcrt_group_last_scene_seconds": [vp, C.POINTER(C.c_double), C.POINTER(C.c_double)],
     }
     for name, args in sig.items():
-        if name in ("mcrt_debug_beam", "mcrt_debug_beam_bounce") and not hasattr(L, name):
+        if name in ("mcrt_debug_beam", "mcrt_debug_beam_bounce", "mcrt_debug_beam_order", "mcrt_debug_beam_layout") and not hasattr(L, name):
             continue
         f = getattr(L, name)
         f.argtypes = args
diff --git a/mcray-tracing_amd/api.py b/mcray-tracing_amd/api.py
--- a/mcray-tracing_amd/api.py
+++ b/mcray-tracing_amd/api.py
@@ -114,6 +114,14 @@
     return out
 
 
+def host_beam_layout(counts):
+    counts = np.ascontiguousarray(counts, np.uint32)
+    bases = np.zeros(len(counts), np.uint32)
+    out = (C.c_uint32 * 4)()
+    check(load_library().mcrt_debug_beam_layout(ptr(counts), len(counts), ptr(bases), out))
+    return bases, int(out[0]), int(out[1]), int(out[2]), int(out[3])
+
+
 def host_scan_maps(n_elements, n_rows, radius_mm=30.0, total_angle=DEFAULT_ANGLE, max_travel_us=100, speed_of_sound=1500, out_rows=400, out_cols=500):
     return _sector_maps("mcrt_scan_maps", n_elements, n_rows, radius_mm, total_angle, max_travel_us, speed_of_sound, out_rows, out_cols)
 
@@ -513,6 +521,12 @@
         out = (C.c_uint32 * 8)()
         if hasattr(self.L, "mcrt_debug_beam_bounce"):
             check(self.L.mcrt_debug_beam_bounce(self.h, int(b), out))
+        return (bool(out[0]),) + tuple(int(v) for v in out[1:])
+
+    def debug_beam_order(self, b):
+        out = (C.c_uint32 * 5)()
+        if hasattr(self.L, "mcrt_debug_beam_order"):
+            check(self.L.mcrt_debug_beam_order(self.h, int(b), out))
         return (bool(out[0]),) + tuple(int(v) for v in out[1:])
 
     def debug_set_error(self, bits):
diff --git a/mcray-tracing_amd/csrc/mcrt_api.cpp b/mcray-tracing_amd/csrc/mcrt_api.cpp
--- a/mcray-tracing_amd/csrc/mcrt_api.cpp
+++ b/mcray-tracing_amd/csrc/mcrt_api.cpp
@@ -54,6 +54,8 @@
     if (const char *e = tuning_env("MCRT_BEAM_GROUPS")) { long long v = atoll(e); if (v >= 1 && v <= (1 << 20)) k.beam_groups = (uint32_t)v; }
     if (const char *e = tuning_env("MCRT_BEAM_CAP")) { int v = atoi(e); if (v >= 1 && v <= (int)MCRT_BEAM_CAP_MAX) k.beam_cap = (uint32_t)v; }
     if (const char *e = tuning_env("MCRT_BEAM_NEAR")) { int v = atoi(e); if (v >= 1) k.beam_near = (uint32_t)v; }
+    if (const char *e = tuning_env("MCRT_BEAM_ORDER")) { long v = strtol(e, nullptr, 0); if (v >= 0 && v < (1l << MCRT_MAX_BOUNCES)) k.beam_order = (uint32_t)v; }
+    if (const char *e = tuning_env("MCRT_BEAM_PAIRS")) k.beam_pairs = atoi(e) != 0;
     if (const char *e = tuning_env("MCRT_RENDER_ROW_TILE")) k.render_row_tile = atoi(e) != 0;
     if (const char *e = tuning_env("MCRT_SPECKLE_FUSE")) { int v = atoi(e); if (v == 2 || v == 4) k.speckle_fuse = (uint32_t)v; }
     return k;
@@ -564,6 +566,35 @@
     return debug_beam(c, b, out);
 }
 
+extern "C" int mcrt_debug_beam_order(mcrt_ctx *c, uint32_t b, uint32_t out[5])
+{
+    CTX_TRY(c);
+    if (!out) return set_error(MCRT_ERR_INVALID, "null out pointer");
+    for (int k = 0; k < 5; k++) out[k] = 0u;
+    if (b >= MCRT_MAX_BOUNCES || !((c->ins.last_beam_mask >> b) & 1u) || c->work.empty()) return MCRT_OK;
+    uint32_t lc[MCRT_BEAM_COUNTERS] = {};
+    HIP_TRY(hipStreamSynchronize(c->stream));
+    HIP_TRY(hipMemcpy(lc, c->work[0].beam.lcount.p + (size_t)b * MCRT_BEAM_COUNTERS, sizeof lc, hipMemcpyDeviceToHost));
+    out[0] = (c->ins.last_beam_order >> b) & 1u; out[1] = lc[8]; out[2] = lc[9]; out[3] = lc[10]; out[4] = lc[11];
+    return MCRT_OK;
+}
+
+extern "C" int mcrt_debug_beam_layout(const uint32_t *counts, uint32_t n, uint32_t *bases, uint32_t out[4])
+{
+    if ((!counts || !bases) && n) return set_error(MCRT_ERR_INVALID, "null pointer");
+    if (!out) return set_error(MCRT_ERR_INVALID, "null out pointer");
+    uint64_t at = 0, placed = 0;
+    uint32_t segments = 0;
+    for (uint32_t k = 0; k < n; k++) {
+        if (at > 0xffffffffull) return set_error(MCRT_ERR_LIMIT, "the beam order is longer than 2^32 words");
+        bases[k] = (uint32_t)at;
+        at += mcrt::beam_segment(counts[k]); placed += counts[k]; segments += counts[k] != 0u ? 1u : 0u;
+    }
+    if (at > 0xffffffffull) return set_error(MCRT_ERR_LIMIT, "the beam order is longer than 2^32 words");
+    out[0] = (uint32_t)placed; out[1] = segments; out[2] = (uint32_t)(at - placed); out[3] = (uint32_t)at;
+    return MCRT_OK;
+}
+
 extern "C" int mcrt_debug_set_error(mcrt_ctx *c, uint32_t bits)
 {
     CTX_TRY(c);
diff --git a/mcray-tracing_amd/csrc/mcrt_beam.hip b/mcray-tracing_amd/csrc/mcrt_beam.hip
--- a/mcray-tracing_amd/csrc/mcrt_beam.hip
+++ b/mcray-tracing_amd/csrc/mcrt_beam.hip
@@ -74,6 +74,7 @@
     if (i < g.n_beams * MCRT_BEAM_REC) g.red[i] = (i & 8u) ? 0u : 0xffffffffu;
     if (i < g.groups) g.gkey[i] = 0ull;
     if (i < MCRT_BEAM_COUNTERS) g.lcount[i] = 0u;
+    if (g.ordered && i <= g.n_beams) g.ocount[i] = 0u;
     if (i <= MCRT_MAX_BOUNCES) g.l_counts[i] = 0u;
     if (i < MCRT_MAX_BOUNCES * MCRT_XCDS) g.l_cursors[(size_t)i * MCRT_CURSOR_STRIDE] = 0u;
 }
@@ -104,6 +105,70 @@
 #pragma unroll
         for (int k = 0; k < 6; k++) { const uint32_t m = ford(wave_max(mine ? hi[k] : -INFINITY)); if ((int)lane == 8 + k && m > __hip_atomic_load(&w[8 + k], __ATOMIC_RELAXED, __HIP_MEMORY_SCOPE_AGENT)) atomicMax(&w[8 + k], m); }
     }
+}
+
+#define BEAM_ST 1024u
+
+__global__ void __launch_bounds__(256) k_beam_rank(FrameArgs a, BeamArgs g)
+{
+    const uint32_t n = a.counts[g.b];
+    const uint32_t lane = threadIdx.x & 63u;
+    const uint32_t base = (blockIdx.x * 256u + threadIdx.x) & ~63u;
+    if (base >= n) return;
+    const uint32_t i = base + lane;
+    const bool live = i < n;
+    BeamRay r;
+    const bool ok = beam_ray(a, g, live ? i : 0u, false, r);
+    const int bid = ok && r.bid >= 0 ? r.bid : (int)g.n_beams;
+    uint32_t rank = 0;
+    unsigned long long todo = __ballot(live);
+    while (todo) {
+        const int first = __ffsll((long long)todo) - 1;
+        const int cb = __builtin_amdgcn_readlane(bid, first);
+        const bool mine = live && bid == cb;
+        const unsigned long long mm = __ballot(mine);
+        todo &= ~mm;
+        uint32_t at = 0;
+        if ((int)lane == first) at = atomicAdd(&g.ocount[cb], (uint32_t)__popcll(mm));
+        at = (uint32_t)__builtin_amdgcn_readlane((int)at, first);
+        if (mine) rank = at + (uint32_t)__popcll(mm & ((1ull << lane) - 1ull));
+    }
+    if (live) { g.rbeam[i] = (uint32_t)bid; g.rrank[i] = rank; }
+}
+
+__global__ void __launch_bounds__(BEAM_ST) k_beam_scan(BeamArgs g)
+{
+    __shared__ uint32_t part[BEAM_ST];
+    __shared__ uint32_t stat[2];
+    const uint32_t t = threadIdx.x, n = g.n_beams + 1u, per = (n + BEAM_ST - 1u) / BEAM_ST;
+    const uint32_t lo = t * per < n ? t * per : n, hi = lo + per < n ? lo + per : n;
+    uint32_t sum = 0, placed = 0, segs = 0;
+    for (uint32_t k = lo; k < hi; k++) { const uint32_t c = g.ocount[k]; sum += beam_segment(c); placed += c; segs += c != 0u ? 1u : 0u; }
+    part[t] = sum;
+    if (t < 2u) stat[t] = 0u;
+    __syncthreads();
+    for (uint32_t o = 1u; o < BEAM_ST; o <<= 1) {
+        const uint32_t v = t >= o ? part[t - o] : 0u;
+        __syncthreads();
+        part[t] += v;
+        __syncthreads();
+    }
+    uint32_t at = part[t] - sum;
+    for (uint32_t k = lo; k < hi; k++) {
+        const uint32_t c = g.ocount[k], w = beam_segment(c);
+        g.obase[k] = at;
+        for (uint32_t j = c; j < w; j++) g.order[at + j] = MCRT_BEAM_PAD;
+        at += w;
+    }
+    if (placed) { atomicAdd(&stat[0], placed); atomicAdd(&stat[1], segs); }
+    __syncthreads();
+    if (t == 0u) { const uint32_t total = part[BEAM_ST - 1u]; g.lcount[8] = stat[0]; g.lcount[9] = stat[1]; g.lcount[10] = total - stat[0]; g.lcount[12] = total; }
+}
+
+__global__ void __launch_bounds__(256) k_beam_place(FrameArgs a, BeamArgs g)
+{
+    const uint32_t n = a.counts[g.b], i = blockIdx.x * 256u + threadIdx.x;
+    if (i < n) g.order[g.obase[g.rbeam[i]] + g.rrank[i]] = i;
 }
 
 struct BeamGeom { int dom; bool neg; float xref, w, m, umin, umax, vmin, vmax, alo, ahi, blo, bhi, smax; };
@@ -257,13 +322,15 @@
 
 __global__ void __launch_bounds__(256) k_beam_test(FrameArgs a, BeamArgs g, uint32_t pass)
 {
-    const uint32_t n = pass == 0u ? a.counts[g.b] : g.lcount[0];
+    const bool ordered = pass == 0u && g.ordered != 0u;
+    const uint32_t n = pass != 0u ? g.lcount[0] : ordered ? g.lcount[12] : a.counts[g.b];
     const uint32_t lane = threadIdx.x & 63u;
     const uint32_t base = (blockIdx.x * 256u + threadIdx.x) & ~63u;
     if (base >= n) return;
     const uint32_t j = base + lane;
-    const bool live = j < n;
-    const uint32_t ray = !live ? 0u : pass == 0u ? j : g.lq0[j];
+    bool live = j < n;
+    uint32_t ray = !live ? 0u : ordered ? g.order[j] : pass == 0u ? j : g.lq0[j];
+    if (ordered && ray == MCRT_BEAM_PAD) { live = false; ray = 0u; }
     BeamRay r;
     bool member = beam_ray(a, g, ray, false, r) && live && r.bid >= 0;
     const uint32_t *rec = g.rec + (size_t)(member ? r.bid : 0) * MCRT_BEAM_REC;
@@ -282,11 +349,13 @@
     const float f2d = comp(f2, r.dom), sg = r.neg ? -1.0f : 1.0f;
     bool left = live && !member;
     unsigned long long todo = __ballot(member);
+    uint32_t met = 0;
     const uint32_t first = pass == 0u ? 0u : g.near, cut = pass == 0u ? g.near : 0xffffffffu;
     while (todo) {
         const int cb = __builtin_amdgcn_readlane(r.bid, __ffsll((long long)todo) - 1);
         const bool mine = member && r.bid == cb;
         todo &= ~__ballot(mine);
+        met++;
         const u32x8 R = sload8(g.rec + (size_t)cb * MCRT_BEAM_REC + 8);
         const float m2 = 2.0f * __uint_as_float(R[3]), xref = __uint_as_float(R[4]);
         const uint32_t n_ent = R[6];
@@ -312,6 +381,7 @@
         }
         left = left || (mine && !(reach < limit || limit == INFINITY));
     }
+    if (g.pairs && pass == 0u && met && lane == 0u) atomicAdd(&g.lcount[11], met);
     if (live && best.tri >= 0) keys[ray] = ((unsigned long long)__float_as_uint(best.frac) << 32) | (unsigned long long)(uint32_t)best.tri;
     const unsigned long long lm = __ballot(left);
     if (lm) {
@@ -352,8 +422,14 @@
     if (setup < g.groups) setup = g.groups;
     hipLaunchKernelGGL(k_beam_clear, dim3((setup + 255u) / 256u), dim3(256), 0, st, g);
     hipLaunchKernelGGL(k_beam_bounds, dim3((blocks + g.stride - 1u) / g.stride), dim3(256), 0, st, a, g);
+    if (g.ordered) {
+        hipLaunchKernelGGL(k_beam_rank, dim3(blocks), dim3(256), 0, st, a, g);
+        hipLaunchKernelGGL(k_beam_scan, dim3(1), dim3(BEAM_ST), 0, st, g);
+        hipLaunchKernelGGL(k_beam_place, dim3(blocks), dim3(256), 0, st, a, g);
+    }
     hipLaunchKernelGGL(k_beam_collect, dim3(g.groups != 0u ? g.groups : g.n_beams), dim3(BEAM_CT), 0, st, a, g);
-    hipLaunchKernelGGL(k_beam_test, dim3(blocks), dim3(256), 0, st, a, g, 0u);
+    const uint32_t blocks0 = g.ordered ? (uint32_t)(((size_t)np + 64u * ((size_t)g.n_beams + 1u) + 255u) / 256u) : blocks;
+    hipLaunchKernelGGL(k_beam_test, dim3(blocks0), dim3(256), 0, st, a, g, 0u);
     const uint32_t which = g.near < g.cap ? 1u : 0u;
     if (which) hipLaunchKernelGGL(k_beam_test, dim3(blocks), dim3(256), 0, st, a, g, 1u);
     const uint32_t few = blocks < 2048u ? blocks : 2048u;
diff --git a/mcray-tracing_amd/csrc/mcrt_ctx.h b/mcray-tracing_amd/csrc/mcrt_ctx.h
--- a/mcray-tracing_amd/csrc/mcrt_ctx.h
+++ b/mcray-tracing_amd/csrc/mcrt_ctx.h
@@ -23,7 +23,9 @@
     Buf<uint32_t> red, rec, lcount, l_counts, l_cursors;
     Buf<uint4> list;
     Buf<unsigned long long> gkey;
-    uint32_t beams = 0, lists = 0, groups = 0, cap = 0;
+    Buf<uint32_t> rbeam, rrank, ocount, obase, order;
+    uint32_t beams = 0, lists = 0, groups = 0, cap = 0, order_beams = 0;
+    size_t order_rays = 0;
 };
 struct Work {
     Stream stream, side[MCRT_SIDE_STREAMS];
@@ -50,6 +52,8 @@
     uint32_t beam_deep_from = MCRT_BEAM_DEEP_FROM;
     uint32_t beam_groups = 0;
     uint32_t beam_cap = MCRT_BEAM_CAP_DEFAULT, beam_near = MCRT_BEAM_NEAR_DEFAULT;
+    uint32_t beam_order = MCRT_BEAM_ORDER_DEFAULT;
+    bool beam_pairs = false;
     bool render_row_tile = false;
     uint32_t speckle_fuse = MCRT_SPECKLE_FUSE_DEFAULT;
     bool test_hooks = false;
@@ -146,6 +150,7 @@
     bool timing_on = false; int timing_level = 0;
     std::vector<TimedLaunch> ev; size_t ev_used = 0;
     uint32_t last_beam_mask = 0;
+    uint32_t last_beam_order = 0;
     bool last_beam_far = false;
     float last_lean_bound = 0.0f; uint32_t last_march_rows = 0;
 };
diff --git a/mcray-tracing_amd/csrc/mcrt_internal.h b/mcray-tracing_amd/csrc/mcrt_internal.h
--- a/mcray-tracing_amd/csrc/mcrt_internal.h
+++ b/mcray-tracing_amd/csrc/mcrt_internal.h
@@ -18,8 +18,9 @@
 #define MCRT_PACKET_MASK_DEFAULT 2u
 #define MCRT_PACKET_FROM 262144u
 #define MCRT_BEAM_FROM 2097152u
-#define MCRT_BEAM_LAST_DEFAULT 2u
+#define MCRT_BEAM_LAST_DEFAULT 3u
 #define MCRT_BEAM_DEEP_FROM 6291456u
+#define MCRT_BEAM_ORDER_DEFAULT 0x8u
 #define MCRT_BEAM_GROUPS_PER_LINE 32u
 #define MCRT_BEAM_LISTS_PER_GROUP 1u
 #define MCRT_BEAM_CAP_DEFAULT 512u
diff --git a/mcray-tracing_amd/csrc/mcrt_kernels.h b/mcray-tracing_amd/csrc/mcrt_kernels.h
--- a/mcray-tracing_amd/csrc/mcrt_kernels.h
+++ b/mcray-tracing_amd/csrc/mcrt_kernels.h
@@ -48,7 +48,9 @@
 #define MCRT_BEAM_REC 16u
 #define MCRT_BEAM_CAP_MAX 1024u
 #define MCRT_BEAM_PROBES 4u
-#define MCRT_BEAM_COUNTERS 8u
+#define MCRT_BEAM_COUNTERS 16u
+#define MCRT_BEAM_PAD 0xffffffffu
+constexpr uint32_t beam_segment(uint32_t count) { return (count + 63u) & ~63u; }
 struct BeamArgs {
     uint32_t *red;
     uint32_t *rec;
@@ -61,6 +63,11 @@
     uint32_t groups;
     uint32_t n_beams, n_lists, cap, near, stride;
     float spread_cap;
+    uint32_t ordered;
+    uint32_t pairs;
+    uint32_t *rbeam, *rrank;
+    uint32_t *ocount, *obase;
+    uint32_t *order;
 };
 
 constexpr uint32_t MCRT_ALL_BOUNCES = 0xffffffffu;
diff --git a/mcray-tracing_amd/csrc/mcrt_trace.cpp b/mcray-tracing_amd/csrc/mcrt_trace.cpp
--- a/mcray-tracing_amd/csrc/mcrt_trace.cpp
+++ b/mcray-tracing_amd/csrc/mcrt_trace.cpp
@@ -188,7 +188,7 @@
         for (uint32_t b = 2; b <= c->knobs.beam_last && b < a.B; b++) mask |= 1u << b;
     return mask;
 }
-struct BeamPlan { mcrt::BeamArgs g = {}; uint32_t mask = 0, beams_b1 = 0, groups = 0; };
+struct BeamPlan { mcrt::BeamArgs g = {}; uint32_t mask = 0, order = 0, beams_b1 = 0, groups = 0; };
 static int fill_beam(const mcrt_ctx *c, Work &w, const mcrt::FrameArgs &a, uint32_t mask, BeamPlan &bp)
 {
     const uint32_t cap = c->knobs.beam_cap;
@@ -211,7 +211,16 @@
         b.beams = beams; b.lists = lists; b.groups = bp.groups; b.cap = cap;
     }
     const size_t np = (size_t)a.ne * a.S;
+    bp.order = mask & c->knobs.beam_order;
+    if (bp.order && (np > b.order_rays || beams > b.order_beams)) {
+        HIP_TRY(hipDeviceSynchronize());
+        b.order_rays = 0; b.order_beams = 0;
+        HIP_TRY(b.rbeam.alloc(np)); HIP_TRY(b.rrank.alloc(np)); HIP_TRY(b.ocount.alloc((size_t)beams + 1)); HIP_TRY(b.obase.alloc((size_t)beams + 1));
+        HIP_TRY(b.order.alloc(np + 64 * ((size_t)beams + 1)));
+        b.order_rays = np; b.order_beams = beams;
+    }
     mcrt::BeamArgs &g = bp.g;
+    g.rbeam = b.rbeam; g.rrank = b.rrank; g.ocount = b.ocount; g.obase = b.obase; g.order = b.order; g.pairs = c->knobs.beam_pairs ? 1u : 0u;
     g.red = b.red; g.rec = b.rec; g.list = b.list; g.gkey = b.gkey; g.lcount = b.lcount; g.l_counts = b.l_counts; g.l_cursors = b.l_cursors;
     g.cap = cap; g.near = std::min(c->knobs.beam_near, cap);
     g.stride = np >= MCRT_BEAM_SAMPLE_FROM ? MCRT_BEAM_SAMPLE_STRIDE : 1u;
@@ -227,6 +236,7 @@
     g.groups = b == 1u ? 0u : bp.groups;
     g.n_beams = b == 1u ? bp.beams_b1 : bp.groups * 6u;
     g.n_lists = b == 1u ? bp.beams_b1 : bp.groups * MCRT_BEAM_LISTS_PER_GROUP;
+    g.ordered = (bp.order >> b) & 1u;
     return g;
 }
 
@@ -325,7 +335,7 @@
         MCRT_TRY(check_overflow(c, P, args[g], *ws[g]));
         if (const uint32_t mask = beam_wanted(c, P, args[g])) { MCRT_TRY(fill_beam(c, *ws[g], args[g], mask, beams[g])); args[g].beam_mask = mask & ~3u; }
     }
-    c->ins.last_beam_mask = beams[0].mask; c->ins.last_beam_far = c->knobs.beam_near < c->knobs.beam_cap;
+    c->ins.last_beam_mask = beams[0].mask; c->ins.last_beam_order = beams[0].order; c->ins.last_beam_far = c->knobs.beam_near < c->knobs.beam_cap;
     return enqueue_pass(c, P, args, beams, ws, accumulate);
 }
 
```

Result: faster. 569.9 million rays/s (median of 6 runs) (+4.8%).
